# jcribeiro98/V-GAN

Hardware: AMD Instinct MI355X
Metric: V-GAN train steps/sec (batch=1024, d=784) (higher is better)
Workload: dtype f32; MMD contractions of `value`: split-bf16 x3 on the bf16 MFMA with fp32 accumulation (centred operand); the same step with the fp32 MFMA is timed in `fp32_mode`; 1 GPU; configs[2]: MNIST-pixels-as-features stand-in, d=784, batch=1024 (VGAN_no_kl step); global_batch=1024, features=784, latent=49, rows_per_gpu=1024, parallelism=dp1 (row-sharded Gram, replicated front), hip_graph=True, generator=collapsed, chain_association=depth, mmd_precision=bf16x3, gram_tile=64

## Files before the change

include/vgan_hip.h:

```cpp
#ifndef VGAN_HIP_H
#define VGAN_HIP_H

#include <stdint.h>

#ifdef __cplusplus
extern "C" {
#endif

#define VGAN_OK 0
#define VGAN_ERR_ARG 1
#define VGAN_ERR_HIP 2

#define VGAN_ABI_VERSION 11

typedef void* vgan_stream_t;

int vgan_abi_version(void);
const char* vgan_last_error(void);

int vgan_linear_forward(const float* x, int ldx, int x_nslabs, int64_t x_slab_stride, const float* W,
                        int ldw, const float* b, float* y, int ldy, int n, int in, int out,
                        vgan_stream_t stream);
int vgan_linear_backward_input(const float* dy, int lddy, const float* W, int ldw,
                               float* dx, int lddx, int n, int in, int out, vgan_stream_t stream);
int vgan_linear_backward_params(const float* dy, int lddy, const float* x, int ldx, int x_nslabs,
                                int64_t x_slab_stride, float* dW, int lddw, float* db, int n, int in,
                                int out, int splits, int64_t slab_stride, vgan_stream_t stream);
struct vgan_xx_job;
int vgan_linear_backward_params_xx_supported(int n, int in, int out);
int vgan_linear_backward_params_xx(const float* dy, int lddy, const float* x, int ldx, float* dW, int lddw, int n, int in,
                                   int out, const struct vgan_xx_job* xx, vgan_stream_t stream);
int64_t vgan_linear_backward_params_ksplit_ws_bytes(int in, int out, int parts);
int vgan_linear_backward_params_ksplit(const float* dy, int lddy, const float* x, int ldx, float* dW, int lddw, int n, int in,
                                       int out, int parts, void* ws, int64_t ws_bytes, vgan_stream_t stream);
int vgan_reduce_slabs(const float* src, int64_t slab_stride, int nslabs, float* dst, int64_t count,
                      vgan_stream_t stream);

typedef struct vgan_logits_chain {
    const float* za;
    const float* At4;
    int32_t ldza, ldat, e0, pad;
} vgan_logits_chain;
int vgan_mask_project_forward(const float* logits, int ldl, const float* data, int ldd,
                              const int32_t* rows, const uint64_t* row_cursor, int row_batches,
                              int row_stride, int row_offset, float* S, float* U, float* Zx, float* Zy,
                              int ldz, float* sqx, float* sqy, int n, int d, const float* center,
                              int norm_split, const vgan_logits_chain* chain, vgan_stream_t stream);
int vgan_col_mean(const float* data, int ldd, int rows, int d, float* out, vgan_stream_t stream);
int vgan_gather_rows(const float* data, int ldd, const int32_t* rows, const uint64_t* row_cursor,
                     int row_batches, int row_stride, int row_offset, float* out, int ldo,
                     float* sq, int n, int d, vgan_stream_t stream);
int vgan_gather_rows_split(const float* data, int ldd, const int32_t* rows, const uint64_t* row_cursor,
                           int row_batches, int row_stride, int row_offset, const float* center, float* out,
                           int ldo, float* sq, int norm_split, uint16_t* Zh, uint16_t* Zl, int kp, int n, int d,
                           vgan_stream_t stream);
int vgan_mask_backward(const float* gU, int ldg, int nslabs, int64_t slab_stride, const float* S,
                       int lds, const uint64_t* colkey, float pen_weight, int row_offset,
                       float* dlogits, int ldo, int n, int d, vgan_stream_t stream);
int vgan_colmax_chunks(int n);
int vgan_colmax(const float* S, int lds, int from_softmax, int row_offset, uint64_t* part,
                uint64_t* colkey, int n, int d, vgan_stream_t stream);
int vgan_colmax_partial(const float* S, int lds, int from_softmax, int row_offset, uint64_t* part,
                        int n, int d, vgan_stream_t stream);
int vgan_mask_from_softmax(const float* S, int lds, float* U, int ldu, int n, int d, vgan_stream_t stream);
int vgan_upper_softmax_forward(const float* logits, int ldl, float* S, float* U, int n, int d,
                               vgan_stream_t stream);

#define VGAN_TILE 64
#define VGAN_TILE_INTS 8
#define VGAN_TF_SLOT_MASK 3
#define VGAN_TF_TWICE 4
#define VGAN_TF_STORE 8
#define VGAN_TF_MIRROR 16
#define VGAN_TF_NEG 32

int vgan_mmd_build_tiles(int n, int grad_mode, int rank, int world, int tile, int32_t* out, int cap);
int vgan_mmd_order_tiles(int32_t* tiles, int count, int tile);

int vgan_mmd_gram(const float* Z, int ldz, const float* sq, int n, int p, const float* bw,
                  const int32_t* tiles, int ntiles, int calibrate,
                  float* Wg, int ldw, int wrow0, float* partial, vgan_stream_t stream);
#define VGAN_RBF_MAX_KERNELS 8
int vgan_mmd_gram_general(const float* Z, int ldz, const float* sq, int n, int p, const float* bw,
                          const int32_t* tiles, int ntiles, const float* multipliers, int n_kernels,
                          float* Wg, int ldw, int wrow0, float* partial, vgan_stream_t stream);
int vgan_mmd_gram_colmax(const float* Z, int ldz, const float* sq, int n, int p, const float* bw,
                         const int32_t* tiles, int ntiles, float* Wg, int ldw, int wrow0, float* partial,
                         const float* S, int lds, int from_softmax, int row_offset, uint64_t* colpart,
                         int nrows, int d, vgan_stream_t stream);
int vgan_mmd_reduce(const float* partial, const int32_t* tiles, int ntiles, double* stats,
                    int zero_first, vgan_stream_t stream);
int vgan_mmd_set_bandwidth(const double* stats, int n, float* bw, vgan_stream_t stream);
int vgan_mmd_loss(const double* stats, const uint64_t* colkey, int n, int d, float weight,
                  float* loss, float* loss_accum, float accum_scale, uint64_t* step_counter,
                  vgan_stream_t stream);
int vgan_mmd_finalize(const float* partial, const int32_t* tiles, int ntiles, const uint64_t* colpart,
                      int chunks, uint64_t* colkey, int n, int d, float weight, double* stats,
                      float* loss, float* loss_accum, float accum_scale, uint64_t* step_counter,
                      vgan_stream_t stream);
typedef struct vgan_finalize_job {
    const float* partial;
    const int32_t* tiles;
    const uint64_t* colpart;
    uint64_t* colkey;
    double* stats;
    float* loss;
    float* loss_accum;
    uint64_t* step_counter;
    int32_t ntiles, chunks, n, d;
    float weight, accum_scale;
    int32_t mode, ntiles_main;
} vgan_finalize_job;
int vgan_mmd_backward(const float* Wg, int ldw, const float* Z, int ldz, int wrow0, int nr,
                      int ncols, int p, const float* mul, int ldmul, const float* mul_shift, float* out,
                      int ldo, int splits, int64_t slab_stride, const vgan_finalize_job* finalize,
                      vgan_stream_t stream);
int vgan_mmd_bf3_prepare(const float* Z, int ldz, int rows, int p, uint16_t* Zh, uint16_t* Zl, int kp,
                         uint16_t* ZTh, uint16_t* ZTl, int kn, vgan_stream_t stream);
int64_t vgan_mmd_gram_bf3_tail_ws_bytes(void);
int vgan_mmd_gram_bf3(const uint16_t* Zh, const uint16_t* Zl, int kp, const float* sq, int n, const float* bw,
                      const int32_t* tiles, int ntiles, int tile, uint16_t* Wh, uint16_t* Wl, int ldw,
                      int wrow0, float* partial, const float* S, int lds, int from_softmax, int row_offset,
                      uint64_t* colpart, int nrows, int d, void* tail_ws, int64_t tail_ws_bytes,
                      float* rs_part, int ldrs, vgan_stream_t stream);
int vgan_mmd_backward_bf3_tile(int nr, int p, int splits, int tile);
int vgan_mmd_backward_bf3(const uint16_t* Wh, const uint16_t* Wl, int ldw, const uint16_t* ZTh,
                          const uint16_t* ZTl, int kn, int kp, const float* Z, int ldz, int wrow0, int nr,
                          int p, const float* mul, int ldmul, const float* mul_shift, float* out, int ldo,
                          int splits, int64_t slab_stride, int tile, const vgan_finalize_job* finalize,
                          vgan_stream_t stream);
int vgan_mmd_backward_bf3_rm(const uint16_t* Wh, const uint16_t* Wl, int ldw, int kn, const uint16_t* Zh,
                             const uint16_t* Zl, int kp, int zrows, const float* Z, int ldz, int wrow0, int nr,
                             int p, const float* mul, int ldmul, const float* mul_shift, float* out, int ldo,
                             int splits, int64_t slab_stride, int tile, const vgan_finalize_job* finalize,
                             const float* rs_part, int ldrs, vgan_stream_t stream);
int vgan_mmd_backward_bf3_rm_xx(const uint16_t* Wh, const uint16_t* Wl, int ldw, int kn, const uint16_t* Zh,
                                const uint16_t* Zl, int kp, int zrows, const float* Z, int ldz, int wrow0, int nr,
                                int p, const float* mul, int ldmul, const float* mul_shift, float* out, int ldo,
                                int splits, int64_t slab_stride, const vgan_finalize_job* finalize,
                                const struct vgan_xx_job* xx, vgan_stream_t stream);
typedef struct vgan_bwd_rebuild {
    const float* data;
    const int32_t* xrow;
    const float* S;
    const float* center;
    int32_t ldd, lds;
} vgan_bwd_rebuild;
int vgan_mmd_backward_bf3_rm_rebuild(const uint16_t* Wh, const uint16_t* Wl, int ldw, int kn, const uint16_t* Zh,
                                     const uint16_t* Zl, int kp, int zrows, int nr, int p,
                                     const vgan_bwd_rebuild* rebuild, float* out, int ldo, int splits,
                                     int64_t slab_stride, const vgan_finalize_job* finalize,
                                     const struct vgan_xx_job* xx, vgan_stream_t stream);
#define VGAN_GEMM_MAX_GROUP 4
#define VGAN_GEMM_NN 0
#define VGAN_GEMM_NT 1
#define VGAN_GEMM_TN 2
#define VGAN_GEMM_NT_NT 3
typedef struct vgan_gemm_problem {
    const float* a;
    const float* b;
    float* c;
    int32_t kind, m, n, k, lda, ldb, ldc, splitk;
    const float* d;
    float* scratch;
    int32_t ldd, k2;
} vgan_gemm_problem;
int vgan_gemm_grouped(const vgan_gemm_problem* problems, int count, vgan_stream_t stream);
typedef struct vgan_adadelta_layer {
    float* w_packed;
    int64_t off_w, off_b;
    int32_t ldp, out, in, pad;
} vgan_adadelta_layer;
typedef struct vgan_grouped_extras {
    const float* copy_src;
    float* copy_dst;
    int64_t copy_count;
    int32_t adadelta, pad;
    float* p;
    float* sq_avg;
    float* acc_delta;
    float lr, rho, eps, weight_decay, grad_scale;
    int32_t ld_extra;
    vgan_adadelta_layer layer[VGAN_GEMM_MAX_GROUP + 1];
    const float* g_extra;
    float* next_noise;
    int32_t noise_rows, noise_cols, noise_ld, noise_ones_col;
    uint64_t seed;
    const uint64_t* step_counter;
    const vgan_finalize_job* fold;
} vgan_grouped_extras;
int vgan_gemm_grouped_ex(const vgan_gemm_problem* problems, int count, const vgan_grouped_extras* extras,
                         vgan_stream_t stream);
int64_t vgan_gemm_grouped_ksplit_ws_bytes(const vgan_gemm_problem* problems, int count, const int32_t* kparts);
int vgan_gemm_grouped_ksplit(const vgan_gemm_problem* problems, int count, const vgan_grouped_extras* extras,
                             const int32_t* kparts, void* ws, int64_t ws_bytes, vgan_stream_t stream);

typedef struct vgan_xx_job {
    const uint16_t* Dh;
    const uint16_t* Dl;
    const float* dsq;
    const int32_t* tiles;
    const float* bw;
    float* partial;
    int32_t ldd, ntiles;
} vgan_xx_job;
int vgan_mask_project_forward_bf3(const float* logits, int ldl, const float* data, int ldd, const int32_t* rows,
                                  const uint64_t* row_cursor, int row_batches, int row_stride, float* S, float* Z,
                                  int ldz, float* sq, uint16_t* Zh, uint16_t* Zl, int kp, uint16_t* ZTh,
                                  uint16_t* ZTl, int kn, int n, int d, const float* center, int write_x,
                                  const vgan_xx_job* xx, const vgan_logits_chain* chain, vgan_stream_t stream);
int vgan_mask_project_forward_bf3_ex(const float* logits, int ldl, const float* data, int ldd, const int32_t* rows,
                                     const uint64_t* row_cursor, int row_batches, int row_stride, float* S, float* Z,
                                     int ldz, float* sq, uint16_t* Zh, uint16_t* Zl, int kp, uint16_t* ZTh,
                                     uint16_t* ZTl, int kn, int n, int d, const float* center, int write_x,
                                     const vgan_xx_job* xx, const vgan_logits_chain* chain, int write_z, int32_t* xrow,
                                     vgan_stream_t stream);
int vgan_row_sqnorm(const float* Z, int ldz, float* sq, int rows, int p, vgan_stream_t stream);

int vgan_adadelta_step(float* p, const float* g, int nslabs, int64_t slab_stride, float* sq_avg,
                       float* acc_delta, int64_t count, float lr, float rho, float eps,
                       float weight_decay, float grad_scale, vgan_stream_t stream);

int vgan_noise_normal(float* z, int rows, int cols, int ld, int ones_col, uint64_t seed,
                      const uint64_t* step_counter, uint64_t stream_id, vgan_stream_t stream);

int vgan_homogeneous_pack(const int64_t* desc, int count, int max_elems, int unpack, vgan_stream_t stream);
int vgan_adadelta_step_packed(float* p, const int32_t* pmap, const float* g_packed, float* w_packed,
                              float* sq_avg, float* acc_delta, int64_t count, float lr, float rho,
                              float eps, float weight_decay, float grad_scale, float* next_noise,
                              int noise_rows, int noise_cols, int noise_ld, int noise_ones_col,
                              uint64_t seed, const uint64_t* step_counter, vgan_stream_t stream);

int vgan_mse(const float* a, int lda, const float* b, int ldb, int n, int d, float scale,
             float* out, int accumulate, vgan_stream_t stream);

int vgan_mse_grad(const float* target, int ldt, const float* pred, int ldp, int n, int d, float gscale,
                  double* part, float* g, int ldg, vgan_stream_t stream);
int vgan_sum_f64(const double* in, int count, double scale, float* out, int accumulate, vgan_stream_t stream);

#define VGAN_DP_ID_BYTES 128
typedef struct vgan_dp_comm vgan_dp_comm;
int vgan_dp_unique_id(uint8_t* id );
int vgan_dp_comm_create(vgan_dp_comm** comm, int nranks, const uint8_t* id, int rank);
int vgan_dp_allreduce_sum(vgan_dp_comm* comm, float* buf, int64_t count, vgan_stream_t stream);
int vgan_dp_allgather(vgan_dp_comm* comm, void* buf, int64_t bytes_per_rank, vgan_stream_t stream);
int vgan_dp_comm_destroy(vgan_dp_comm* comm);

int vgan_shuffle_epoch(int32_t* perm, int64_t count, int64_t train_size, uint64_t seed, uint64_t epoch,
                       vgan_stream_t stream);
int64_t vgan_shuffle_index(int64_t i, int64_t train_size, uint64_t seed, uint64_t epoch);
int vgan_mask_unique(const uint8_t* masks, int ldm, int n, int d, uint64_t* keys, int32_t* work,
                     int32_t* out_row, int32_t* out_count, vgan_stream_t stream);

int vgan_rbf_kernel_matrix(const float* Z, int ldz, int m, int p, const float* sq, float alpha, float* K, int ldk,
                           vgan_stream_t stream);
int vgan_rbf_multi_kernel_matrix(const float* Z, int ldz, int m, int p, const float* sq, const float* bw,
                                 const float* multipliers, int n_kernels, float* K, int ldk, float* dK, int lddk,
                                 vgan_stream_t stream);
int vgan_rows_dot(const float* A, int lda, const float* B, int ldb, double* out, int rows, int cols,
                  vgan_stream_t stream);

#define VGAN_OUTLIER_MAX_K 32
#define VGAN_OUTLIER_ENGINE_EXACT 0
#define VGAN_OUTLIER_ENGINE_GRAM 1
#define VGAN_OUTLIER_KNN_LARGEST 0
#define VGAN_OUTLIER_KNN_MEAN 1
#define VGAN_OUTLIER_KNN_MEDIAN 2
#define VGAN_OUTLIER_LRD 3
#define VGAN_OUTLIER_LOF 4
#define VGAN_OUTLIER_KDE_MAX_ROWS 8388607
int vgan_outlier_pack(const float* X, int ldx, int n, int d, const float* center, const int32_t* feat,
                      const int32_t* feat_off, const int64_t* col_off, int first, int count, float* packed, float* sq,
                      vgan_stream_t stream);
int vgan_outlier_knn(const float* Pq, const float* sq_q, int nq, const float* Pr, const float* sq_r, int nr,
                     const int32_t* feat_off, const int64_t* col_off, int first, int count, int k, int exclude_self,
                     int engine, int splits, float* part_d, int32_t* part_i, int32_t* nbr, vgan_stream_t stream);
int vgan_outlier_refine(const float* Xq, int ldq, int nq, const float* Xr, int ldr, int nr, int d, const int32_t* feat,
                        const int32_t* feat_off, int first, int count, const int32_t* nbr, int k, int32_t* out_idx,
                        float* out_dist, float* kdist, vgan_stream_t stream);
int vgan_outlier_score(const int32_t* idx, const float* dist, int nq, int k, int count, int method, const float* kdist_ref,
                       const double* lrd_ref, int nr, float* score, const int32_t* score_row, int ld_score, double* lrd_out,
                       vgan_stream_t stream);
int vgan_outlier_kde(const float* Pq, const float* sq_q, int nq, const float* Pr, const float* sq_r, int nr,
                     const int32_t* feat_off, const int64_t* col_off, int first, int count, const double* bandwidth,
                     int exclude_self, int engine, int splits, uint32_t* pivot, uint64_t* acc, float* score,
                     const int32_t* score_row, int ld_score, vgan_stream_t stream);
int vgan_outlier_combine(const float* score, int ld, int S, int n, const double* weights, double* out,
                         vgan_stream_t stream);
int vgan_outlier_abod(const float* Xq, int ldq, int nq, const float* Xr, int ldr, int nr, int d, const int32_t* feat,
                      const int32_t* feat_off, int first, int count, const int32_t* idx, int k, float* score,
                      const int32_t* score_row, int ld_score, vgan_stream_t stream);
int vgan_outlier_abod_floor(float* score, int ld, int S, int n, int fit, double* score_floor, int32_t* n_degenerate,
                            vgan_stream_t stream);
#define VGAN_OUTLIER_NORM_ZSCORE 1
#define VGAN_OUTLIER_NORM_ROBUST 2
#define VGAN_OUTLIER_NORM_MINMAX 3
#define VGAN_OUTLIER_COMBINE_SUM 0
#define VGAN_OUTLIER_COMBINE_MAX 1
int64_t vgan_outlier_score_stats_ws_bytes(int S, int n, int mode);
int vgan_outlier_score_stats(const float* score, int ld, int S, int n, int mode, double* center, double* scale,
                             void* workspace, int64_t workspace_bytes, vgan_stream_t stream);
int vgan_outlier_combine_normalized(const float* score, int ld, int S, int n, const double* center, const double* scale,
                                    const double* weights, int combination, double* out, vgan_stream_t stream);

#define VGAN_CLUSTER_MAX_CLUSTERS 64
// ... 101 lines not shown
```

v-gan_amd/csrc/gemm_bf3.hpp:

```cpp
#pragma once
#include <type_traits>

#include "gemm_core.hpp"

namespace vgan {

typedef __bf16 bf16x8 __attribute__((ext_vector_type(8)));
typedef unsigned u32x4 __attribute__((ext_vector_type(4)));
typedef __attribute__((address_space(3))) u32x4 lds_u4;
typedef __attribute__((address_space(3))) unsigned short lds_u16;
typedef short s16x4 __attribute__((ext_vector_type(4)));
typedef short s16x8 __attribute__((ext_vector_type(8)));
typedef __attribute__((address_space(3))) s16x4 lds_s4;

__device__ __forceinline__ bf16x8 tr_read_k8(const char __attribute__((address_space(3)))* p0, int rows4) {
    const s16x4 a = __builtin_amdgcn_ds_read_tr16_b64_v4i16((lds_s4*)p0);
    const s16x4 b = __builtin_amdgcn_ds_read_tr16_b64_v4i16((lds_s4*)(p0 + rows4));
    const s16x8 v = {a[0], a[1], a[2], a[3], b[0], b[1], b[2], b[3]};
    return __builtin_bit_cast(bf16x8, v);
}


template <int BK_>
struct GemmBF3 {
// ... 130 lines not shown
            for (int r = 0; r < NR; ++r) {
                float s = rsum[r];
#pragma unroll
                for (int o = 1; o < QPR; o <<= 1) s += __shfl_xor(s, o, 64);
                const int f = tid + kBlock * r;
                if (f % QPR == 0) rs_lds[f / QPR] = s;
            }
            __syncthreads();
        }
    }
    __device__ static __forceinline__ int sub_row(int r) {
        const int lane = threadIdx.x & 63, wave = (threadIdx.x >> 6) & 3;
        return (wave >> 1) * 32 + (r & 3) + 8 * (r >> 2) + 4 * (lane >> 5);
    }
    __device__ static __forceinline__ int sub_col() {
        const int lane = threadIdx.x & 63, wave = (threadIdx.x >> 6) & 3;
        return (wave & 1) * 32 + (lane & 31);
    }

    static_assert(BK == 64, "row-major B path: K tile of 64");
    static constexpr int PARTB = 64 * 128;
    static constexpr int BUFT = 2 * PART + 2 * PARTB;
    static constexpr int kLdsBytesT = 2 * BUFT;

    struct StageT {
        u32x4 v[4][NR];
        const char* srcA[2][NR];
        const unsigned short *Bh, *Bl;
        long ldb;
        int lofsA[NR], lofsB[NR], rowB[NR], colB[NR], zrows;
        __device__ __forceinline__ void init(const unsigned short* Ah, const unsigned short* Al, long lda, int m0, int M,
                                             const unsigned short* Bh_, const unsigned short* Bl_, long ldb_, int n0, int zrows_, int tid) {
            Bh = Bh_; Bl = Bl_; ldb = ldb_; zrows = zrows_;
#pragma unroll
            for (int r = 0; r < NR; ++r) {
                const int f = tid + kBlock * r, row = f / QPR, q = f % QPR;
                const long ra = (long)min(m0 + row, M - 1) * lda + 8 * q;
                srcA[0][r] = reinterpret_cast<const char*>(Ah + ra);
                srcA[1][r] = reinterpret_cast<const char*>(Al + ra);
                lofsA[r] = row * ROWB + q * 16;
                rowB[r] = row;
                colB[r] = n0 + 8 * q;
                lofsB[r] = row * 128 + ((q ^ (((row >> 1) & 1) << 2)) << 4);
            }
        }
        __device__ __forceinline__ void load(int k0) {
#pragma unroll
            for (int r = 0; r < NR; ++r) {
                v[0][r] = *reinterpret_cast<const u32x4*>(srcA[0][r] + 2 * (long)k0);
                v[1][r] = *reinterpret_cast<const u32x4*>(srcA[1][r] + 2 * (long)k0);
                const long ob = (long)min(k0 + rowB[r], zrows - 1) * ldb + colB[r];
                v[2][r] = *reinterpret_cast<const u32x4*>(Bh + ob);
                v[3][r] = *reinterpret_cast<const u32x4*>(Bl + ob);
            }
        }
        __device__ __forceinline__ void store(char __attribute__((address_space(3)))* buf) const {
#pragma unroll
            for (int r = 0; r < NR; ++r) {
                *(lds_u4*)(buf + lofsA[r]) = v[0][r];
                *(lds_u4*)(buf + PART + lofsA[r]) = v[1][r];
                *(lds_u4*)(buf + 2 * PART + lofsB[r]) = v[2][r];
                *(lds_u4*)(buf + 2 * PART + PARTB + lofsB[r]) = v[3][r];
            }
        }
        __device__ __forceinline__ float a_rowpart(int r) const {
            float s = 0.f;
            const unsigned* h = reinterpret_cast<const unsigned*>(&v[0][r]);
            const unsigned* l = reinterpret_cast<const unsigned*>(&v[1][r]);
#pragma unroll
            for (int e = 0; e < 4; ++e) {
                s += __uint_as_float(h[e] << 16) + __uint_as_float(h[e] & 0xFFFF0000u);
                s += __uint_as_float(l[e] << 16) + __uint_as_float(l[e] & 0xFFFF0000u);
            }
            return s;
        }
    };

    template <bool SIDE_A>
    __device__ static __forceinline__ void run_bt(const unsigned short* Ah, const unsigned short* Al, long lda, const unsigned short* Bh,
                                                  const unsigned short* Bl, long ldb, int zrows, int m0, int n0, int M, int K,
                                                  char* lds_generic, float* rs_generic, f32x16& acc) {
        typedef char __attribute__((address_space(3))) lds_c;
        lds_c* lds = (lds_c*)lds_generic;
        lds_f* rs_lds = (lds_f*)rs_generic;
        const int tid = threadIdx.x, lane = tid & 63, wave = tid >> 6;
        const int wm0 = (wave >> 1) * 32, wn0 = (wave & 1) * 32;
        const int fi = lane & 31, fh = lane >> 5;
        const int g = lane >> 4, li = lane & 15, qq = li >> 2, pp = li & 3;
        const int chunk = (wn0 >> 3) + 2 * (g & 1) + (pp >> 1);
        const int offB0 = (8 * (g >> 1) + qq) * 128 + ((chunk ^ (((qq >> 1) & 1) << 2)) << 4) + (pp & 1) * 8;
        StageT st;
        st.init(Ah, Al, lda, m0, M, Bh, Bl, ldb, n0, zrows, tid);
        float rsum[NR];
#pragma unroll
        for (int r = 0; r < NR; ++r) rsum[r] = 0.f;
        auto side = [&]() {
#pragma unroll
            for (int r = 0; r < NR; ++r) rsum[r] += st.a_rowpart(r);
        };
        const int nk = K / BK;
        st.load(0);
        st.store(lds);
        if constexpr (SIDE_A) side();
        if (nk > 1) st.load(BK);
        __syncthreads();
        auto body = [&](int kt, auto store_next, auto load_next2) {
            const lds_c* buf = lds + (kt & 1) * BUFT;
            const lds_c* pa = buf + (wm0 + fi) * ROWB + fh * 16;
            const lds_c* pb = buf + 2 * PART + offB0;
            u32x4 ah[KS], al[KS];
            bf16x8 yh[KS], yl[KS];
#pragma unroll
            for (int s = 0; s < KS; ++s) {
                ah[s] = *(const lds_u4*)(pa + s * 32);
                al[s] = *(const lds_u4*)(pa + PART + s * 32);
                yh[s] = tr_read_k8(pb + s * 2048, 512);
                yl[s] = tr_read_k8(pb + PARTB + s * 2048, 512);
            }
            if constexpr (decltype(store_next)::value) {
                st.store(lds + ((kt & 1) ^ 1) * BUFT);
                if constexpr (SIDE_A) side();
            }
            if constexpr (decltype(load_next2)::value) st.load((kt + 2) * BK);
#pragma unroll
            for (int s = 0; s < KS; ++s) {
                const bf16x8 xh = __builtin_bit_cast(bf16x8, ah[s]), xl = __builtin_bit_cast(bf16x8, al[s]);
                acc = __builtin_amdgcn_mfma_f32_32x32x16_bf16(xl, yh[s], acc, 0, 0, 0);
                acc = __builtin_amdgcn_mfma_f32_32x32x16_bf16(xh, yl[s], acc, 0, 0, 0);
                acc = __builtin_amdgcn_mfma_f32_32x32x16_bf16(xh, yh[s], acc, 0, 0, 0);
            }
            __builtin_amdgcn_iglp_opt(0);
            __syncthreads();
        };
        using T = std::true_type;
        using F = std::false_type;
        int kt = 0;
        for (; kt + 2 < nk; ++kt) body(kt, T{}, T{});
        if (kt + 1 < nk) {
            body(kt, T{}, F{});
            ++kt;
        }
        body(kt, F{}, F{});
        if constexpr (SIDE_A) {
#pragma unroll
            for (int r = 0; r < NR; ++r) {
                float s = rsum[r];
#pragma unroll
                for (int o = 1; o < QPR; o <<= 1) s += __shfl_xor(s, o, 64);
                const int f = tid + kBlock * r;
                if (f % QPR == 0) rs_lds[f / QPR] = s;
            }
            __syncthreads();
        }
    }
};


struct GemmBF3Big {
    static constexpr int BM = 128, BN = 128, BK = 64, NTH = 512;
    static constexpr int PART = 128 * 128;
    static constexpr int PARTB = 64 * 256;
    static constexpr int BUF = 4 * PART;
    static constexpr int BUFT = 2 * PART + 2 * PARTB;
    static constexpr int kLdsBytes = 2 * BUF;
    static constexpr int kLdsBytesT = 2 * BUFT;
    typedef char __attribute__((address_space(3))) lds_c;

    struct Quad {
        f32x16 a[2][2];
        __device__ __forceinline__ void zero() {
#pragma unroll
            for (int i = 0; i < 2; ++i)
#pragma unroll
                for (int j = 0; j < 2; ++j)
#pragma unroll
                    for (int r = 0; r < 16; ++r) a[i][j][r] = 0.f;
        }
        __device__ __forceinline__ void mac(const bf16x8 (&xh)[2], const bf16x8 (&xl)[2], const bf16x8 (&yh)[2], const bf16x8 (&yl)[2]) {
#pragma unroll
            for (int i = 0; i < 2; ++i)
#pragma unroll
                for (int j = 0; j < 2; ++j) a[i][j] = __builtin_amdgcn_mfma_f32_32x32x16_bf16(xl[i], yh[j], a[i][j], 0, 0, 0);
#pragma unroll
            for (int i = 0; i < 2; ++i)
#pragma unroll
                for (int j = 0; j < 2; ++j) a[i][j] = __builtin_amdgcn_mfma_f32_32x32x16_bf16(xh[i], yl[j], a[i][j], 0, 0, 0);
#pragma unroll
            for (int i = 0; i < 2; ++i)
#pragma unroll
                for (int j = 0; j < 2; ++j) a[i][j] = __builtin_amdgcn_mfma_f32_32x32x16_bf16(xh[i], yh[j], a[i][j], 0, 0, 0);
        }
        __device__ __forceinline__ void exchange(lds_c* lds, f32x16 (&acc)[2]) const {
            lds_f* xch = (lds_f*)lds;
            const int lane = threadIdx.x & 63, wave = threadIdx.x >> 6, grp = wave >> 2;
#pragma unroll
            for (int i = 0; i < 2; ++i)
#pragma unroll
                for (int r = 0; r < 16; ++r) xch[((wave * 2 + i) * 16 + r) * 64 + lane] = grp ? a[i][0][r] : a[i][1][r];
            __syncthreads();
            const int partner = wave ^ 4;
#pragma unroll
            for (int i = 0; i < 2; ++i)
#pragma unroll
                for (int r = 0; r < 16; ++r) acc[i][r] += (grp ? a[i][1][r] : a[i][0][r]) + xch[((partner * 2 + i) * 16 + r) * 64 + lane];
            __syncthreads();
        }
    };

    struct FillRows {
        const char* src[8];
        int dst0;
        __device__ __forceinline__ void init(const unsigned short* base, long ld, int r0, int lim, int part, int half, int lane) {
#pragma unroll
            for (int e = 0; e < 8; ++e) {
                const int row = half * 64 + 8 * e + (lane >> 3);
                const int c = (lane & 7) ^ ((row >> 1) & 7);
                src[e] = reinterpret_cast<const char*>(base + (long)min(r0 + row, lim - 1) * ld) + 16 * c;
            }
            dst0 = part * PART + half * 8192;
        }
        __device__ __forceinline__ void issue(lds_c* buf, int kt) const {
#pragma unroll
            for (int e = 0; e < 8; ++e)
                __builtin_amdgcn_global_load_lds((const void __attribute__((address_space(1)))*)(src[e] + 2 * (long)kt * BK),
                                                 (void __attribute__((address_space(3)))*)(buf + dst0 + e * 1024), 16, 0, 0);
        }
    };
    struct FillRM {
        const char* src[8];
        long ldb2;
        int krow0, zrows, dst0;
        __device__ __forceinline__ void init(const unsigned short* base, long ld, int n0, int ncols, int zrows_, int bpart, int half, int lane) {
            ldb2 = 2 * ld;
            zrows = zrows_;
            krow0 = half * 32 + (lane >> 4);
#pragma unroll
            for (int e = 0; e < 8; ++e) {
                const int row = krow0 + 4 * e;
                const int c = (lane & 15) ^ ((row & 3) << 2);
                src[e] = reinterpret_cast<const char*>(base + min(n0 + 8 * c, ncols - 8));
            }
            dst0 = 2 * PART + bpart * PARTB + half * 8192;
        }
        __device__ __forceinline__ void issue(lds_c* buf, int kt) const {
#pragma unroll
            for (int e = 0; e < 8; ++e) {
                const char* g = src[e] + (long)min(kt * BK + krow0 + 4 * e, zrows - 1) * ldb2;
                __builtin_amdgcn_global_load_lds((const void __attribute__((address_space(1)))*)g,
                                                 (void __attribute__((address_space(3)))*)(buf + dst0 + e * 1024), 16, 0, 0);
            }
        }
    };

    template <class Fill0, class Fill1, class FragF, class MfmaF>
    __device__ static __forceinline__ void pingpong(int grp, int nk, Fill0 fill0, Fill1 fill1, FragF frags, MfmaF mfmas) {
        auto bar = [&]() {
            __builtin_amdgcn_sched_barrier(0);
            __builtin_amdgcn_s_barrier();
            __builtin_amdgcn_sched_barrier(0);
        };
        auto drain = [&]() { __builtin_amdgcn_s_waitcnt(0x0070); };
        if (grp == 0) {
            for (int kt = 0; kt < nk; ++kt) {
                if (kt + 1 < nk) fill0(kt + 1);
                frags(kt);
                bar();
                mfmas();
                drain();
                bar();
            }
            bar();
        } else {
            if (1 < nk) fill1(1);
            bar();
            for (int kt = 0; kt < nk; ++kt) {
                frags(kt);
                drain();
                bar();
                if (kt + 2 < nk) fill1(kt + 2);
                mfmas();
                bar();
            }
        }
        __syncthreads();
    }

    __device__ static __forceinline__ float frag_sum(const u32x4& h, const u32x4& l, float s) {
#pragma unroll
        for (int e = 0; e < 4; ++e) {
            s += __uint_as_float(h[e] << 16) + __uint_as_float(h[e] & 0xFFFF0000u);
            s += __uint_as_float(l[e] << 16) + __uint_as_float(l[e] & 0xFFFF0000u);
        }
        return s;
    }
    template <class Frag>
    __device__ static __forceinline__ void rowsum_step(const Frag (&ah)[2][2], const Frag (&al)[2][2], int C, float (&rsum)[2]) {
        if (C == 0) {
            rsum[0] = frag_sum(ah[0][0], al[0][0], rsum[0]);
            rsum[1] = frag_sum(ah[0][1], al[0][1], rsum[1]);
        } else {
            rsum[0] = frag_sum(ah[1][0], al[1][0], rsum[0]);
            rsum[1] = frag_sum(ah[1][1], al[1][1], rsum[1]);
        }
    }
    __device__ static __forceinline__ void rowsum_publish(const float (&rsum)[2], lds_f* tmp, int grp, int R, int C, int fi, int fh) {
#pragma unroll
// ... 146 lines not shown
```

v-gan_amd/csrc/mmd_bf16.hip:

```cpp
#include "gemm_bf3.hpp"
#include "gemm_bf3w.hpp"
#include "mmd_common.hpp"
#include "mmd_xx.hpp"

namespace vgan {


__global__ __launch_bounds__(kBlock) void bf3_prepare_kernel(const float* __restrict__ Z, int ldz, int rows, int p,
                                                            unsigned short* __restrict__ Zh, unsigned short* __restrict__ Zl, int kp,
                                                            unsigned short* __restrict__ ZTh, unsigned short* __restrict__ ZTl, int kn,
                                                            int vec) {
    __shared__ unsigned short th[64][68], tl[64][68];
    const int j0 = blockIdx.x * 64, k0 = blockIdx.y * 64;
    const int tj = 4 * (threadIdx.x & 15), tk = 4 * (threadIdx.x >> 4);
    unsigned short hi[4][4], lo[4][4];
#pragma unroll
    for (int a = 0; a < 4; ++a) {
        const int k = k0 + tk + a;
        float v[4] = {0.f, 0.f, 0.f, 0.f};
        if (k < rows) {
            if (vec && j0 + tj + 3 < p) {
                const float4 q = *reinterpret_cast<const float4*>(Z + (long)k * ldz + j0 + tj);
                v[0] = q.x; v[1] = q.y; v[2] = q.z; v[3] = q.w;
            } else {
// ... 385 lines not shown
        };
        float w[16];
        if (cons) {
#pragma unroll
            for (int i = 0; i < 4; ++i)
#pragma unroll
                for (int j = 0; j < 4; ++j)
#pragma unroll
                    for (int r = 0; r < 4; ++r) Wt[G::sub_row(i, r) * LDT + G::sub_col(j)] = acc[i][j][r];
        }
        __syncthreads();
        for (int t = threadIdx.x; t < 256 * 8; t += G::NTH) {
            const int line = t >> 3, q16 = 16 * (t & 7);
            float cs = 0.f;
            if (td.r0 + line < td.rlim && td.c0 + q16 < td.clim) {
#pragma unroll
                for (int e = 0; e < 4; ++e) {
                    const f32x4 v = *(const lds_f4*)(Wt + line * LDT + q16 + 4 * e);
                    w[4 * e] = v[0]; w[4 * e + 1] = v[1]; w[4 * e + 2] = v[2]; w[4 * e + 3] = v[3];
                }
                cs = emit(w, (long)(td.r0 + line - wrow0) * ldw, td.c0 + q16, td.clim);
            }
            if (rs_part != nullptr) {
                cs = slot_sum(cs);
                if ((t & 7) == 0 && td.r0 + line < td.rlim) rs_part[(long)(td.c0 >> 7) * ldrs + (td.r0 + line - wrow0)] = cs;
            }
        }
        if (mirror) {
            __syncthreads();
            if (cons) {
#pragma unroll
                for (int i = 0; i < 4; ++i)
#pragma unroll
                    for (int j = 0; j < 4; ++j)
                        *(lds_f4*)(Wt + G::sub_col(j) * LDM + G::sub_row(i, 0)) = f32x4{acc[i][j][0], acc[i][j][1], acc[i][j][2], acc[i][j][3]};
            }
            __syncthreads();
            for (int t = threadIdx.x; t < 128 * 16; t += G::NTH) {
                const int line = t >> 4, q16 = 16 * (t & 15);
                float cs = 0.f;
                if (td.c0 + line < td.clim && td.r0 + q16 < td.rlim) {
#pragma unroll
                    for (int e = 0; e < 4; ++e) {
                        const f32x4 v = *(const lds_f4*)(Wt + line * LDM + q16 + 4 * e);
                        w[4 * e] = v[0]; w[4 * e + 1] = v[1]; w[4 * e + 2] = v[2]; w[4 * e + 3] = v[3];
                    }
                    cs = emit(w, (long)(td.c0 + line - wrow0) * ldw, td.r0 + q16, td.rlim);
                }
                if (rs_part != nullptr) {
                    cs = slot_sum(cs);
                    if ((t & 7) == 0 && td.c0 + line < td.clim && td.r0 + q16 < td.rlim)
                        rs_part[(long)((td.r0 + q16) >> 7) * ldrs + (td.c0 + line - wrow0)] = cs;
                }
            }
        }
    }
    ksum = wave_sum(ksum);
    if (lane == 0) red[wave] = ksum;
    __syncthreads();
    if (threadIdx.x == 0)
        reinterpret_cast<float4*>(partial)[ti] =
            make_float4(((red[0] + red[1]) + (red[2] + red[3])) + ((red[4] + red[5]) + (red[6] + red[7])), 0.f, 0.f, 0.f);
}

struct BwdRebuild {
    const float* data;
    const int* xrow;
    const float* S;
    const float* center;
    int ldd, lds;
};

template <int BK, bool RM, bool REBUILD>
__global__ __launch_bounds__(kBlock, BK == 64 ? 2 : 3) void mmd_backward_bf3_kernel(const unsigned short* __restrict__ Wh, const unsigned short* __restrict__ Wl,
                                                                    int ldw, const unsigned short* __restrict__ ZTh,
                                                                    const unsigned short* __restrict__ ZTl, int kn, int ldb, int brows,
                                                                    const float* __restrict__ Z, int ldz, int wrow0, int nr, int p,
                                                                    int ptiles, const float* __restrict__ mul, int ldmul,
                                                                    const float* __restrict__ mul_shift, float* __restrict__ out, int ldo,
                                                                    int kchunk, long slab_stride, vgan_finalize_job job, int nfin,
                                                                    XXJob xx, BwdRebuild rb) {
    using G = GemmBF3<BK>;
    constexpr int kBytes = (RM ? G::kLdsBytesT : G::kLdsBytes) > G::kLdsBytes ? (RM ? G::kLdsBytesT : G::kLdsBytes) : G::kLdsBytes;
    __shared__ __attribute__((aligned(16))) char lds[kBytes];
    __shared__ float rs[64];
    const int gx = ptiles, gy = (nr + 63) / 64, total = gx * gy;
    if ((int)blockIdx.x >= total) {
        if (blockIdx.y != 0) return;
        const int extra = (int)blockIdx.x - total;
        if (extra < nfin)
            finalize_body(job);
        else if constexpr (BK == 64)
            xx_tile_body(xx, extra - nfin, lds, rs);
        return;
    }
    const int xcd = blockIdx.x % 8, kidx = blockIdx.x / 8;
    const int q = total / 8, r8 = total % 8;
    const int t = (xcd < r8 ? xcd * (q + 1) : r8 * (q + 1) + (xcd - r8) * q) + kidx;
    const int band = t / (4 * gx), rem = t - band * 4 * gx;
    const int rows_in_band = min(4, gy - band * 4);
    const int m0 = (band * 4 + rem % rows_in_band) * 64, n0 = (rem / rows_in_band) * 64;
    f32x16 acc;
#pragma unroll
    for (int r = 0; r < 16; ++r) acc[r] = 0.f;
    const int k0 = blockIdx.y * kchunk, klen = min(kchunk, kn - k0);
    out += blockIdx.y * slab_stride;
    const int col = n0 + G::sub_col(), colc = min(col, p - 1);
    float z_pre[16], m_pre[16];
    float mshift;
    if constexpr (REBUILD) {
        mshift = rb.center[colc];
#pragma unroll
        for (int r = 0; r < 16; ++r) {
            const int rowc = min(m0 + G::sub_row(r), nr - 1);
            z_pre[r] = rb.S[(long)rowc * rb.lds + colc];
            m_pre[r] = rb.data[(long)rb.xrow[rowc] * rb.ldd + colc];
        }
    } else {
        mshift = mul_shift != nullptr ? mul_shift[colc] : 0.f;
#pragma unroll
        for (int r = 0; r < 16; ++r) {
            const int rowc = min(m0 + G::sub_row(r), nr - 1);
            z_pre[r] = Z[(long)(wrow0 + rowc) * ldz + colc];
            m_pre[r] = mul != nullptr ? mul[(long)rowc * ldmul + colc] + mshift : 1.f;
        }
    }
    if (klen > 0) {
        if constexpr (RM)
            G::template run_bt<true>(Wh + k0, Wl + k0, ldw, ZTh + (long)k0 * ldb, ZTl + (long)k0 * ldb, ldb, brows - k0, m0, n0, nr, klen, lds,
                                     rs, acc);
        else
            G::template run<true>(Wh + k0, Wl + k0, ldw, ZTh + k0, ZTl + k0, ldb, m0, n0, nr, gx * 64, klen, lds, rs, acc);
    }
    if (col >= p) return;
    if constexpr (REBUILD) {
        const float tau = 1.0f / (float)p;
#pragma unroll
        for (int r = 0; r < 16; ++r) {
            const float x = m_pre[r];
            z_pre[r] = project_centred(upper_mask(z_pre[r], tau), x, mshift);
            m_pre[r] = uncentred_x(centred_x(x, mshift), mshift);
        }
    }
#pragma unroll
    for (int r = 0; r < 16; ++r) {
        const int lrow = G::sub_row(r), row = m0 + lrow;
        if (row < nr) {
            const float v = klen > 0 ? 2.f * (rs[lrow] * z_pre[r] - acc[r]) : 0.f;
            out[(long)row * ldo + col] = v * m_pre[r];
        }
    }
}

template <bool RM>
__global__ __launch_bounds__(512, 2) void mmd_backward_bf3_big_kernel(const unsigned short* __restrict__ Wh, const unsigned short* __restrict__ Wl,
                                                                      int ldw, const unsigned short* __restrict__ ZTh,
                                                                      const unsigned short* __restrict__ ZTl, int kn, int ldb, int brows,
                                                                      const float* __restrict__ Z, int ldz, int wrow0, int nr, int p,
                                                                      int ptiles, const float* __restrict__ mul, int ldmul,
                                                                      const float* __restrict__ mul_shift, float* __restrict__ out, int ldo,
                                                                      int kchunk, long slab_stride, int nb_rows, vgan_finalize_job job) {
    using G = GemmBF3Big;
    __shared__ __attribute__((aligned(16))) char lds[RM ? G::kLdsBytesT : G::kLdsBytes];
    __shared__ float rs[128];
    const int gx = ptiles, gy = (nr + 127) / 128, total = gx * gy;
    if ((int)blockIdx.x >= total) {
        if (blockIdx.y == 0) finalize_body(job);
        return;
    }
    const int xcd = blockIdx.x % 8, kidx = blockIdx.x / 8;
    const int q = total / 8, r8 = total % 8;
    const int t = (xcd < r8 ? xcd * (q + 1) : r8 * (q + 1) + (xcd - r8) * q) + kidx;
    const int band = t / (4 * gx), rem = t - band * 4 * gx;
    const int rows_in_band = min(4, gy - band * 4);
    const int m0 = (band * 4 + rem % rows_in_band) * 128, n0 = (rem / rows_in_band) * 128;
    const int k0 = blockIdx.y * kchunk, klen = min(kchunk, kn - k0);
    out += blockIdx.y * slab_stride;
    const int col = n0 + G::sub_col(), colc = min(col, p - 1);
    const float mshift = mul_shift != nullptr ? mul_shift[colc] : 0.f;
    f32x16 acc[2];
#pragma unroll
    for (int i2 = 0; i2 < 2; ++i2)
#pragma unroll
        for (int r = 0; r < 16; ++r) acc[i2][r] = 0.f;
    if (klen > 0) {
        if constexpr (RM)
            G::template run_bt<true>(Wh + k0, Wl + k0, ldw, ZTh + (long)k0 * ldb, ZTl + (long)k0 * ldb, ldb, nb_rows, brows - k0, m0, n0, nr, klen,
                                     lds, acc, rs);
        else
            G::template run<true>(Wh + k0, Wl + k0, ldw, ZTh + k0, ZTl + k0, ldb, m0, n0, nr, nb_rows, klen, lds, acc, rs);
    }
    if (col >= p) return;
#pragma unroll
    for (int i2 = 0; i2 < 2; ++i2) {
        float z_pre[16], m_pre[16];
#pragma unroll
        for (int r = 0; r < 16; ++r) {
            const int rowc = min(m0 + G::sub_row(i2, r), nr - 1);
            z_pre[r] = Z[(long)(wrow0 + rowc) * ldz + colc];
            m_pre[r] = mul != nullptr ? mul[(long)rowc * ldmul + colc] + mshift : 1.f;
        }
#pragma unroll
        for (int r = 0; r < 16; ++r) {
            const int lrow = G::sub_row(i2, r), row = m0 + lrow;
            if (row < nr) {
                const float v = klen > 0 ? 2.f * (rs[lrow] * z_pre[r] - acc[i2][r]) : 0.f;
                out[(long)row * ldo + col] = v * m_pre[r];
            }
        }
    }
}


__global__ __launch_bounds__(768, 3) void mmd_backward_bf3_wide_kernel(const unsigned short* __restrict__ Wh, const unsigned short* __restrict__ Wl,
                                                                       int ldw, const unsigned short* __restrict__ Bh,
                                                                       const unsigned short* __restrict__ Bl, int kn, int ldb, int brows,
                                                                       const float* __restrict__ Z, int ldz, int wrow0, int nr, int p,
                                                                       int ptiles, const float* __restrict__ mul, int ldmul,
                                                                       const float* __restrict__ mul_shift, float* __restrict__ out, int ldo,
                                                                       int kchunk, long slab_stride, int nb_cols, vgan_finalize_job job,
                                                                       const float* __restrict__ rs_part, int ldrs) {
    using G = GemmBF3Wide;
    extern __shared__ __attribute__((aligned(16))) char lds[];
    __shared__ float rs[256];
    const int gx = ptiles, gy = (nr + 255) / 256, total = gx * gy;
    if ((int)blockIdx.x >= total) {
        if (blockIdx.y == 0) finalize_body(job);
        return;
    }
    const int xcd = blockIdx.x % 8, kidx = blockIdx.x / 8;
    const int q = total / 8, r8 = total % 8;
    const int t = (xcd < r8 ? xcd * (q + 1) : r8 * (q + 1) + (xcd - r8) * q) + kidx;
    const int band = t / (4 * gx), rem = t - band * 4 * gx;
    const int rows_in_band = min(4, gy - band * 4);
    const int m0 = (band * 4 + rem % rows_in_band) * 256, n0 = (rem / rows_in_band) * 128;
    const int k0 = blockIdx.y * kchunk, klen = min(kchunk, kn - k0);
    out += blockIdx.y * slab_stride;
    f32x4w acc[4][4];
#pragma unroll
    for (int i = 0; i < 4; ++i)
#pragma unroll
        for (int j = 0; j < 4; ++j) acc[i][j] = f32x4w{0.f, 0.f, 0.f, 0.f};
    if (klen > 0 && rs_part != nullptr) {
        if (threadIdx.x < 256) {
            const float* src = rs_part + min(m0 + (int)threadIdx.x, nr - 1);
            const int s0 = k0 >> 7, s1 = (k0 + klen + 127) >> 7;
            float a0 = 0.f, a1 = 0.f, a2 = 0.f, a3 = 0.f;
            int sl = s0;
            for (; sl + 4 <= s1; sl += 4) {
                a0 += src[(long)sl * ldrs];
                a1 += src[(long)(sl + 1) * ldrs];
                a2 += src[(long)(sl + 2) * ldrs];
                a3 += src[(long)(sl + 3) * ldrs];
            }
            for (; sl < s1; ++sl) a0 += src[(long)sl * ldrs];
            rs[threadIdx.x] = (a0 + a1) + (a2 + a3);
        }
        G::run_bt<false>(Wh + k0, Wl + k0, ldw, Bh + (long)k0 * ldb, Bl + (long)k0 * ldb, ldb, nb_cols, brows - k0, m0, n0, nr, klen, lds, acc);
    } else if (klen > 0)
        G::run_bt<true>(Wh + k0, Wl + k0, ldw, Bh + (long)k0 * ldb, Bl + (long)k0 * ldb, ldb, nb_cols, brows - k0, m0, n0, nr, klen, lds, acc, rs);
    if (G::is_loader()) return;
#pragma unroll
    for (int j = 0; j < 4; ++j) {
        const int col = n0 + G::sub_col(j);
        if (col >= p) continue;
        const float mshift = mul_shift != nullptr ? mul_shift[col] : 0.f;
#pragma unroll
        for (int i = 0; i < 4; ++i) {
            float z_pre[4], m_pre[4];
#pragma unroll
            for (int r = 0; r < 4; ++r) {
                const int rowc = min(m0 + G::sub_row(i, r), nr - 1);
                z_pre[r] = Z[(long)(wrow0 + rowc) * ldz + col];
                m_pre[r] = mul != nullptr ? mul[(long)rowc * ldmul + col] + mshift : 1.f;
            }
#pragma unroll
            for (int r = 0; r < 4; ++r) {
                const int lrow = G::sub_row(i, r), row = m0 + lrow;
                if (row < nr) {
                    const float v = klen > 0 ? 2.f * (rs[lrow] * z_pre[r] - acc[i][j][r]) : 0.f;
                    out[(long)row * ldo + col] = v * m_pre[r];
                }
            }
        }
    }
}

}

using namespace vgan;

extern "C" int vgan_mmd_bf3_prepare(const float* Z, int ldz, int rows, int p, uint16_t* Zh, uint16_t* Zl, int kp, uint16_t* ZTh,
                                    uint16_t* ZTl, int kn, vgan_stream_t stream) {
    VGAN_CHECK_ARG(Z && Zh && Zl && rows > 0 && p > 0 && ldz >= p && kp >= p && kp % 64 == 0 && aligned16(Zh) && aligned16(Zl));
    VGAN_CHECK_ARG((ZTh == nullptr) == (ZTl == nullptr) && (ZTh == nullptr || (kn >= rows && kn % 64 == 0)));
    dim3 grid(kp / 64, (rows + 63) / 64);
    if (ZTh != nullptr) grid.y = kn / 64;
    const int vec = (ldz % 4 == 0) && aligned16(Z);
    hipLaunchKernelGGL(bf3_prepare_kernel, grid, dim3(kBlock), 0, (hipStream_t)stream, Z, ldz, rows, p, Zh, Zl, kp, ZTh, ZTl, kn, vec);
    VGAN_CHECK_LAUNCH();
    return VGAN_OK;
}

#ifndef VGAN_TAIL_MAX_PARTS
#define VGAN_TAIL_MAX_PARTS 4
#endif
extern "C" int64_t vgan_mmd_gram_bf3_tail_ws_bytes(void) { return kTailSlabs * kTailSlabBytes + kTailTicketBytes; }

extern "C" int vgan_mmd_gram_bf3(const uint16_t* Zh, const uint16_t* Zl, int kp, const float* sq, int n, const float* bw,
                                 const int32_t* tiles, int ntiles, int tile, uint16_t* Wh, uint16_t* Wl, int ldw, int wrow0,
                                 float* partial, const float* S, int lds, int from_softmax, int row_offset, uint64_t* colpart,
                                 int nrows, int d, void* tail_ws, int64_t tail_ws_bytes, float* rs_part, int ldrs,
                                 vgan_stream_t stream) {
    VGAN_CHECK_ARG(Zh && Zl && sq && bw && tiles && partial && n > 0 && ntiles > 0 && kp > 0 && kp % 64 == 0);
    VGAN_CHECK_ARG((Wh == nullptr) == (Wl == nullptr) && (reinterpret_cast<uintptr_t>(partial) & 15) == 0);
    VGAN_CHECK_ARG(aligned16(Zh) && aligned16(Zl) && (Wh == nullptr || (aligned16(Wh) && aligned16(Wl) && ldw % 8 == 0)));
    ColmaxJob cj{};
    int extra = 0;
    if (S != nullptr) {
        VGAN_CHECK_ARG(colpart && nrows > 0 && d > 0 && lds >= d);
        cj = ColmaxJob{S, reinterpret_cast<unsigned long long*>(colpart), lds, row_offset, nrows, d, from_softmax, (d + 63) / 64};
        extra = cj.nbx * ((nrows + kColChunkRows - 1) / kColChunkRows);
    }
    VGAN_CHECK_ARG(tile == 64 || tile == 128 || tile == 256);
    VGAN_CHECK_ARG(rs_part == nullptr || (tile == 256 && Wh != nullptr && ldrs > 0 && wrow0 >= 0 && n % 128 == 0));
    if (tile == 256) {
        static const hipError_t attr = hipFuncSetAttribute(reinterpret_cast<const void*>(&mmd_gram_bf3_wide_kernel),
                                                           hipFuncAttributeMaxDynamicSharedMemorySize, GemmBF3Wide::kLdsBytes);
        VGAN_CHECK_ARG(attr == hipSuccess);
        TailSplit ts{nullptr, nullptr, ntiles, 1, kp};
        if (tail_ws != nullptr) {
            VGAN_CHECK_ARG(tail_ws_bytes >= vgan_mmd_gram_bf3_tail_ws_bytes() && aligned16(tail_ws));
            static const int cus = [] {
                int dev = 0, v = 0;
                if (hipGetDevice(&dev) != hipSuccess || hipDeviceGetAttribute(&v, hipDeviceAttributeMultiprocessorCount, dev) != hipSuccess) v = 0;
                return v;
            }();
            const int slots = cus < kTailSlabs ? cus : kTailSlabs;
            const int r = slots > 0 ? ntiles % slots : 0, nst = kp / GemmBF3Wide::BK;
            int parts = 1;
            while (r > 0 && parts < VGAN_TAIL_MAX_PARTS && 2 * parts * r <= slots && nst / (2 * parts) >= 8) parts *= 2;
            if (parts > 1) {
                const int kchunk = ((nst + parts - 1) / parts) * GemmBF3Wide::BK;
                ts = TailSplit{static_cast<float*>(tail_ws), reinterpret_cast<int*>(static_cast<char*>(tail_ws) + kTailSlabs * kTailSlabBytes),
                               ntiles - r, (kp + kchunk - 1) / kchunk, kchunk};
            }
        }
        const int nblk = ts.first + (ntiles - ts.first) * ts.parts;
        hipLaunchKernelGGL(mmd_gram_bf3_wide_kernel, dim3(nblk + extra), dim3(GemmBF3Wide::NTH), GemmBF3Wide::kLdsBytes, (hipStream_t)stream, Zh,
                           Zl, kp, sq, n, bw, reinterpret_cast<const TileDesc*>(tiles), ntiles, Wh, Wl, ldw, wrow0, partial, cj, ts, rs_part, ldrs);
    } else if (tile == 128)
        hipLaunchKernelGGL(mmd_gram_bf3_big_kernel, dim3(ntiles + extra), dim3(512), 0, (hipStream_t)stream, Zh, Zl, kp, sq, n, bw,
                           reinterpret_cast<const TileDesc*>(tiles), ntiles, Wh, Wl, ldw, wrow0, partial, cj);
    else
        hipLaunchKernelGGL(mmd_gram_bf3_kernel<64>, dim3(ntiles + extra), dim3(kBlock), 0, (hipStream_t)stream, Zh, Zl, kp, sq, n, bw,
                           reinterpret_cast<const TileDesc*>(tiles), ntiles, Wh, Wl, ldw, wrow0, partial, cj);
    VGAN_CHECK_LAUNCH();
    return VGAN_OK;
}

extern "C" int vgan_mmd_backward_bf3_tile(int nr, int p, int splits, int tile) {
    if (tile == 64 || tile == 128 || tile == 256) return tile;
    const int wide_tiles = ((p + 127) / 128) * ((nr + 255) / 256);
    if (nr >= 256 && wide_tiles * splits >= 256) return 256;
    const int big_tiles = ((p + 127) / 128) * ((nr + 127) / 128);
    return big_tiles * splits >= 512 ? 128 : 64;
}

static int launch_backward_bf3(int rm, const uint16_t* Wh, const uint16_t* Wl, int ldw, const uint16_t* Bh, const uint16_t* Bl, int kn, int kp,
                               int zrows, const float* Z, int ldz, int wrow0, int nr, int p, const float* mul, int ldmul,
                               const float* mul_shift, float* out, int ldo, int splits, int64_t slab_stride, int tile,
                               const vgan_finalize_job* finalize, vgan_stream_t stream, const vgan_xx_job* xxjob = nullptr,
                               const float* rs_part = nullptr, int ldrs = 0, const vgan_bwd_rebuild* rebuild = nullptr) {
    VGAN_CHECK_ARG(Wh && Wl && Bh && Bl && (Z || rebuild) && out && nr > 0 && p > 0 && kn > 0 && kn % 64 == 0 && kp >= p && kp % 64 == 0);
    VGAN_CHECK_ARG(ldw >= kn && (rebuild || ldz >= p) && ldo >= p && (mul == nullptr || ldmul >= p) && wrow0 >= 0);
    BwdRebuild rb{};
    if (rebuild != nullptr) {
        const vgan_bwd_rebuild& q = *rebuild;
        VGAN_CHECK_ARG(rm && tile == 64 && q.data && q.xrow && q.S && q.center && q.ldd >= p && q.lds >= p && Z == nullptr && mul == nullptr &&
                       mul_shift == nullptr);
        rb = BwdRebuild{q.data, q.xrow, q.S, q.center, q.ldd, q.lds};
    }
    VGAN_CHECK_ARG(aligned16(Wh) && aligned16(Wl) && aligned16(Bh) && aligned16(Bl) && ldw % 8 == 0);
    VGAN_CHECK_ARG(splits >= 1 && splits <= 64 && (splits == 1 || slab_stride >= (int64_t)nr * ldo));
    VGAN_CHECK_ARG((tile == 0 || tile == 64 || tile == 128 || tile == 256) && (mul_shift == nullptr || mul != nullptr) && (!rm || zrows > 0));
    const int kchunk = ((kn / 64 + splits - 1) / splits) * 64;
    const int ldb = rm ? kp : kn;
    vgan_finalize_job job{};
    if (finalize != nullptr) {
        VGAN_CHECK_ARG(finalize_job_ok(*finalize));
        job = *finalize;
    }
    hipStream_t st = (hipStream_t)stream;
    XXJob xx{};
    if (xxjob != nullptr) {
        const vgan_xx_job& j = *xxjob;
        VGAN_CHECK_ARG(rm && tile == 64 && j.Dh && j.Dl && j.dsq && j.tiles && j.bw && j.partial && j.ntiles > 0 && j.ldd % 64 == 0 &&
                       aligned16(j.Dh) && aligned16(j.Dl) && (reinterpret_cast<uintptr_t>(j.partial) & 15) == 0);
        xx = XXJob{j.Dh, j.Dl, j.dsq, nullptr, nullptr, reinterpret_cast<const TileDesc*>(j.tiles), j.bw, j.partial, j.ldd, 1, 0, j.ntiles, 0};
    }
    const int nfin = finalize != nullptr ? 1 : 0;
    int edge = vgan_mmd_backward_bf3_tile(nr, p, splits, tile);
    if (edge == 256 && !rm) edge = 128;
    if (edge == 256) {
        static const hipError_t attr = hipFuncSetAttribute(reinterpret_cast<const void*>(&mmd_backward_bf3_wide_kernel),
                                                           hipFuncAttributeMaxDynamicSharedMemorySize, GemmBF3Wide::kLdsBytes);
        VGAN_CHECK_ARG(attr == hipSuccess);
        const int pt = (p + 127) / 128;
        dim3 grid(pt * ((nr + 255) / 256) + nfin, splits);
        if (rs_part != nullptr && !(ldrs >= nr && (splits == 1 || kchunk % 128 == 0))) rs_part = nullptr;
        hipLaunchKernelGGL(mmd_backward_bf3_wide_kernel, grid, dim3(GemmBF3Wide::NTH), GemmBF3Wide::kLdsBytes, st, Wh, Wl, ldw, Bh, Bl, kn, ldb,
                           zrows, Z, ldz, wrow0, nr, p, pt, mul, ldmul, mul_shift, out, ldo, kchunk, (long)slab_stride, kp, job, rs_part, ldrs);
        VGAN_CHECK_LAUNCH();
        return VGAN_OK;
    }
    if (edge == 128) {
        const int pt = (p + 127) / 128;
        dim3 grid(pt * ((nr + 127) / 128) + (finalize != nullptr ? 1 : 0), splits);
        if (rm)
            hipLaunchKernelGGL(mmd_backward_bf3_big_kernel<true>, grid, dim3(512), 0, st, Wh, Wl, ldw, Bh, Bl, kn, ldb, zrows, Z, ldz, wrow0, nr,
                               p, pt, mul, ldmul, mul_shift, out, ldo, kchunk, (long)slab_stride, kp, job);
        else
            hipLaunchKernelGGL(mmd_backward_bf3_big_kernel<false>, grid, dim3(512), 0, st, Wh, Wl, ldw, Bh, Bl, kn, ldb, 0, Z, ldz, wrow0, nr, p,
                               pt, mul, ldmul, mul_shift, out, ldo, kchunk, (long)slab_stride, kp, job);
        VGAN_CHECK_LAUNCH();
        return VGAN_OK;
    }
    const int ptiles = (p + 63) / 64;
    dim3 grid(ptiles * ((nr + 63) / 64) + nfin + xx.ntiles, splits);
    if (rebuild != nullptr)
        hipLaunchKernelGGL((mmd_backward_bf3_kernel<64, true, true>), grid, dim3(kBlock), 0, st, Wh, Wl, ldw, Bh, Bl, kn, ldb, zrows, Z, ldz, wrow0,
                           nr, p, ptiles, mul, ldmul, mul_shift, out, ldo, kchunk, (long)slab_stride, job, nfin, xx, rb);
    else if (rm)
        hipLaunchKernelGGL((mmd_backward_bf3_kernel<64, true, false>), grid, dim3(kBlock), 0, st, Wh, Wl, ldw, Bh, Bl, kn, ldb, zrows, Z, ldz, wrow0,
                           nr, p, ptiles, mul, ldmul, mul_shift, out, ldo, kchunk, (long)slab_stride, job, nfin, xx, rb);
    else
        hipLaunchKernelGGL((mmd_backward_bf3_kernel<64, false, false>), grid, dim3(kBlock), 0, st, Wh, Wl, ldw, Bh, Bl, kn, ldb, 0, Z, ldz, wrow0, nr,
                           p, ptiles, mul, ldmul, mul_shift, out, ldo, kchunk, (long)slab_stride, job, nfin, xx, rb);
    VGAN_CHECK_LAUNCH();
    return VGAN_OK;
}

extern "C" int vgan_mmd_backward_bf3(const uint16_t* Wh, const uint16_t* Wl, int ldw, const uint16_t* ZTh, const uint16_t* ZTl, int kn,
                                     int kp, const float* Z, int ldz, int wrow0, int nr, int p, const float* mul, int ldmul,
                                     const float* mul_shift, float* out, int ldo, int splits, int64_t slab_stride, int tile,
                                     const vgan_finalize_job* finalize, vgan_stream_t stream) {
    return launch_backward_bf3(0, Wh, Wl, ldw, ZTh, ZTl, kn, kp, 0, Z, ldz, wrow0, nr, p, mul, ldmul, mul_shift, out, ldo, splits, slab_stride,
                               tile, finalize, stream);
}

extern "C" int vgan_mmd_backward_bf3_rm_xx(const uint16_t* Wh, const uint16_t* Wl, int ldw, int kn, const uint16_t* Zh, const uint16_t* Zl,
                                           int kp, int zrows, const float* Z, int ldz, int wrow0, int nr, int p, const float* mul, int ldmul,
                                           const float* mul_shift, float* out, int ldo, int splits, int64_t slab_stride,
                                           const vgan_finalize_job* finalize, const vgan_xx_job* xx, vgan_stream_t stream) {
    VGAN_CHECK_ARG(xx != nullptr);
    return launch_backward_bf3(1, Wh, Wl, ldw, Zh, Zl, kn, kp, zrows, Z, ldz, wrow0, nr, p, mul, ldmul, mul_shift, out, ldo, splits,
                               slab_stride, 64, finalize, stream, xx);
}

extern "C" int vgan_mmd_backward_bf3_rm(const uint16_t* Wh, const uint16_t* Wl, int ldw, int kn, const uint16_t* Zh, const uint16_t* Zl,
                                        int kp, int zrows, const float* Z, int ldz, int wrow0, int nr, int p, const float* mul, int ldmul,
                                        const float* mul_shift, float* out, int ldo, int splits, int64_t slab_stride, int tile,
                                        const vgan_finalize_job* finalize, const float* rs_part, int ldrs, vgan_stream_t stream) {
    return launch_backward_bf3(1, Wh, Wl, ldw, Zh, Zl, kn, kp, zrows, Z, ldz, wrow0, nr, p, mul, ldmul, mul_shift, out, ldo, splits,
                               slab_stride, tile, finalize, stream, nullptr, rs_part, ldrs);
}

extern "C" int vgan_mmd_backward_bf3_rm_rebuild(const uint16_t* Wh, const uint16_t* Wl, int ldw, int kn, const uint16_t* Zh, const uint16_t* Zl,
                                                int kp, int zrows, int nr, int p, const vgan_bwd_rebuild* rebuild, float* out, int ldo,
                                                int splits, int64_t slab_stride, const vgan_finalize_job* finalize, const vgan_xx_job* xx,
                                                vgan_stream_t stream) {
    VGAN_CHECK_ARG(rebuild != nullptr);
    return launch_backward_bf3(1, Wh, Wl, ldw, Zh, Zl, kn, kp, zrows, nullptr, 0, 0, nr, p, nullptr, 0, nullptr, out, ldo, splits, slab_stride, 64,
                               finalize, stream, xx, nullptr, 0, rebuild);
}
```

v-gan_amd/lib.py:

```python
import ctypes
import os

_HERE = os.path.dirname(os.path.abspath(__file__))
LIB_PATH = os.path.join(_HERE, "libvgan_hip.so")

_p = ctypes.c_void_p
_i = ctypes.c_int
_f = ctypes.c_float
_i64 = ctypes.c_int64
_u64 = ctypes.c_uint64

class FinalizeJob(ctypes.Structure):
    _fields_ = [("partial", _p), ("tiles", _p), ("colpart", _p), ("colkey", _p), ("stats", _p), ("loss", _p), ("loss_accum", _p),
                ("step_counter", _p), ("ntiles", ctypes.c_int32), ("chunks", ctypes.c_int32), ("n", ctypes.c_int32),
                ("d", ctypes.c_int32), ("weight", _f), ("accum_scale", _f), ("mode", ctypes.c_int32), ("ntiles_main", ctypes.c_int32)]


class GemmProblem(ctypes.Structure):
    _fields_ = [("a", _p), ("b", _p), ("c", _p), ("kind", ctypes.c_int32), ("m", ctypes.c_int32), ("n", ctypes.c_int32),
                ("k", ctypes.c_int32), ("lda", ctypes.c_int32), ("ldb", ctypes.c_int32), ("ldc", ctypes.c_int32), ("splitk", ctypes.c_int32),
                ("d", _p), ("scratch", _p), ("ldd", ctypes.c_int32), ("k2", ctypes.c_int32)]


class LogitsChain(ctypes.Structure):
    _fields_ = [("za", _p), ("At4", _p), ("ldza", ctypes.c_int32), ("ldat", ctypes.c_int32), ("e0", ctypes.c_int32), ("pad", ctypes.c_int32)]


class XXJob(ctypes.Structure):
    _fields_ = [("Dh", _p), ("Dl", _p), ("dsq", _p), ("tiles", _p), ("bw", _p), ("partial", _p), ("ldd", ctypes.c_int32),
                ("ntiles", ctypes.c_int32)]


class BwdRebuild(ctypes.Structure):
    _fields_ = [("data", _p), ("xrow", _p), ("S", _p), ("center", _p), ("ldd", ctypes.c_int32), ("lds", ctypes.c_int32)]


class AdadeltaLayer(ctypes.Structure):
    _fields_ = [("w_packed", _p), ("off_w", _i64), ("off_b", _i64), ("ldp", ctypes.c_int32), ("out", ctypes.c_int32),
                ("inp", ctypes.c_int32), ("pad", ctypes.c_int32)]


class GroupedExtras(ctypes.Structure):
    _fields_ = [("copy_src", _p), ("copy_dst", _p), ("copy_count", _i64), ("adadelta", ctypes.c_int32), ("pad", ctypes.c_int32),
                ("p", _p), ("sq_avg", _p), ("acc_delta", _p), ("lr", _f), ("rho", _f), ("eps", _f), ("weight_decay", _f),
                ("grad_scale", _f), ("ld_extra", ctypes.c_int32), ("layer", AdadeltaLayer * 5), ("g_extra", _p), ("next_noise", _p),
                ("noise_rows", ctypes.c_int32), ("noise_cols", ctypes.c_int32), ("noise_ld", ctypes.c_int32),
                ("noise_ones_col", ctypes.c_int32), ("seed", _u64), ("step_counter", _p), ("fold", _p)]


GEMM_NN, GEMM_NT, GEMM_TN, GEMM_NT_NT = 0, 1, 2, 3
GEMM_MAX_GROUP = 4

SIGNATURES = {
    "vgan_abi_version": (_i, []),
    "vgan_last_error": (ctypes.c_char_p, []),
    "vgan_linear_forward": (_i, [_p, _i, _i, _i64, _p, _i, _p, _p, _i, _i, _i, _i, _p]),
    "vgan_linear_backward_input": (_i, [_p, _i, _p, _i, _p, _i, _i, _i, _i, _p]),
    "vgan_linear_backward_params": (_i, [_p, _i, _p, _i, _i, _i64, _p, _i, _p, _i, _i, _i, _i, _i64, _p]),
    "vgan_linear_backward_params_ksplit_ws_bytes": (_i64, [_i, _i, _i]),
    "vgan_linear_backward_params_ksplit": (_i, [_p, _i, _p, _i, _p, _i, _i, _i, _i, _i, _p, _i64, _p]),
    "vgan_linear_backward_params_xx_supported": (_i, [_i, _i, _i]),
    "vgan_linear_backward_params_xx": (_i, [_p, _i, _p, _i, _p, _i, _i, _i, _i, _p, _p]),
    "vgan_reduce_slabs": (_i, [_p, _i64, _i, _p, _i64, _p]),
    "vgan_mask_project_forward": (_i, [_p, _i, _p, _i, _p, _p, _i, _i, _i, _p, _p, _p, _p, _i, _p, _p, _i, _i, _p, _i, _p, _p]),
    "vgan_col_mean": (_i, [_p, _i, _i, _i, _p, _p]),
    "vgan_gather_rows": (_i, [_p, _i, _p, _p, _i, _i, _i, _p, _i, _p, _i, _i, _p]),
    "vgan_gather_rows_split": (_i, [_p, _i, _p, _p, _i, _i, _i, _p, _p, _i, _p, _i, _p, _p, _i, _i, _i, _p]),
    "vgan_mask_backward": (_i, [_p, _i, _i, _i64, _p, _i, _p, _f, _i, _p, _i, _i, _i, _p]),
    "vgan_colmax_partial": (_i, [_p, _i, _i, _i, _p, _i, _i, _p]),
    "vgan_mmd_finalize": (_i, [_p, _p, _i, _p, _i, _p, _i, _i, _f, _p, _p, _p, _f, _p, _p]),
    "vgan_colmax_chunks": (_i, [_i]),
    "vgan_colmax": (_i, [_p, _i, _i, _i, _p, _p, _i, _i, _p]),
    "vgan_mask_from_softmax": (_i, [_p, _i, _p, _i, _i, _i, _p]),
    "vgan_upper_softmax_forward": (_i, [_p, _i, _p, _p, _i, _i, _p]),
    "vgan_mmd_build_tiles": (_i, [_i, _i, _i, _i, _i, _p, _i]),
    "vgan_mmd_order_tiles": (_i, [_p, _i, _i]),
    "vgan_mmd_gram": (_i, [_p, _i, _p, _i, _i, _p, _p, _i, _i, _p, _i, _i, _p, _p]),
    "vgan_mmd_gram_general": (_i, [_p, _i, _p, _i, _i, _p, _p, _i, _p, _i, _p, _i, _i, _p, _p]),
    "vgan_mmd_gram_colmax": (_i, [_p, _i, _p, _i, _i, _p, _p, _i, _p, _i, _i, _p, _p, _i, _i, _i, _p, _i, _i, _p]),
    "vgan_mmd_reduce": (_i, [_p, _p, _i, _p, _i, _p]),
    "vgan_mmd_set_bandwidth": (_i, [_p, _i, _p, _p]),
    "vgan_mmd_loss": (_i, [_p, _p, _i, _i, _f, _p, _p, _f, _p, _p]),
    "vgan_mmd_backward": (_i, [_p, _i, _p, _i, _i, _i, _i, _i, _p, _i, _p, _p, _i, _i, _i64, _p, _p]),
    "vgan_mmd_bf3_prepare": (_i, [_p, _i, _i, _i, _p, _p, _i, _p, _p, _i, _p]),
    "vgan_mmd_gram_bf3": (_i, [_p, _p, _i, _p, _i, _p, _p, _i, _i, _p, _p, _i, _i, _p, _p, _i, _i, _i, _p, _i, _i, _p, _i64, _p, _i, _p]),
    "vgan_mmd_gram_bf3_tail_ws_bytes": (_i64, []),
    "vgan_mmd_backward_bf3": (_i, [_p, _p, _i, _p, _p, _i, _i, _p, _i, _i, _i, _i, _p, _i, _p, _p, _i, _i, _i64, _i, _p, _p]),
    "vgan_mmd_backward_bf3_tile": (_i, [_i, _i, _i, _i]),
    "vgan_mmd_backward_bf3_rm": (_i, [_p, _p, _i, _i, _p, _p, _i, _i, _p, _i, _i, _i, _i, _p, _i, _p, _p, _i, _i, _i64, _i, _p, _p, _i, _p]),
    "vgan_mmd_backward_bf3_rm_xx": (_i, [_p, _p, _i, _i, _p, _p, _i, _i, _p, _i, _i, _i, _i, _p, _i, _p, _p, _i, _i, _i64, _p, _p, _p]),
    "vgan_mmd_backward_bf3_rm_rebuild": (_i, [_p, _p, _i, _i, _p, _p, _i, _i, _i, _i, _p, _p, _i, _i, _i64, _p, _p, _p]),
    "vgan_row_sqnorm": (_i, [_p, _i, _p, _i, _i, _p]),
    "vgan_adadelta_step": (_i, [_p, _p, _i, _i64, _p, _p, _i64, _f, _f, _f, _f, _f, _p]),
    "vgan_noise_normal": (_i, [_p, _i, _i, _i, _i, _u64, _p, _u64, _p]),
    "vgan_homogeneous_pack": (_i, [_p, _i, _i, _i, _p]),
    "vgan_adadelta_step_packed": (_i, [_p, _p, _p, _p, _p, _p, _i64, _f, _f, _f, _f, _f, _p, _i, _i, _i, _i, _u64, _p, _p]),
    "vgan_gemm_grouped": (_i, [_p, _i, _p]),
    "vgan_gemm_grouped_ex": (_i, [_p, _i, _p, _p]),
    "vgan_gemm_grouped_ksplit_ws_bytes": (_i64, [_p, _i, _p]),
    "vgan_gemm_grouped_ksplit": (_i, [_p, _i, _p, _p, _p, _i64, _p]),
    "vgan_mask_project_forward_bf3": (_i, [_p, _i, _p, _i, _p, _p, _i, _i, _p, _p, _i, _p, _p, _p, _i, _p, _p, _i, _i, _i, _p, _i, _p, _p, _p]),
    "vgan_mask_project_forward_bf3_ex": (_i, [_p, _i, _p, _i, _p, _p, _i, _i, _p, _p, _i, _p, _p, _p, _i, _p, _p, _i, _i, _i, _p, _i, _p, _p, _i, _p,
                                              _p]),
    "vgan_mse_grad": (_i, [_p, _i, _p, _i, _i, _i, _f, _p, _p, _i, _p]),
    "vgan_sum_f64": (_i, [_p, _i, ctypes.c_double, _p, _i, _p]),
    "vgan_rbf_kernel_matrix": (_i, [_p, _i, _i, _i, _p, _f, _p, _i, _p]),
    "vgan_rbf_multi_kernel_matrix": (_i, [_p, _i, _i, _i, _p, _p, _p, _i, _p, _i, _p, _i, _p]),
    "vgan_rows_dot": (_i, [_p, _i, _p, _i, _p, _i, _i, _p]),
    "vgan_shuffle_epoch": (_i, [_p, _i64, _i64, _u64, _u64, _p]),
    "vgan_shuffle_index": (_i64, [_i64, _i64, _u64, _u64]),
    "vgan_mask_unique": (_i, [_p, _i, _i, _i, _p, _p, _p, _p, _p]),
    "vgan_dp_unique_id": (_i, [_p]),
    "vgan_dp_comm_create": (_i, [_p, _i, _p, _i]),
    "vgan_dp_allreduce_sum": (_i, [_p, _p, _i64, _p]),
    "vgan_dp_allgather": (_i, [_p, _p, _i64, _p]),
    "vgan_dp_comm_destroy": (_i, [_p]),
    "vgan_mse": (_i, [_p, _i, _p, _i, _i, _i, _f, _p, _i, _p]),
    "vgan_outlier_pack": (_i, [_p, _i, _i, _i, _p, _p, _p, _p, _i, _i, _p, _p, _p]),
    "vgan_outlier_knn": (_i, [_p, _p, _i, _p, _p, _i, _p, _p, _i, _i, _i, _i, _i, _i, _p, _p, _p, _p]),
    "vgan_outlier_refine": (_i, [_p, _i, _i, _p, _i, _i, _i, _p, _p, _i, _i, _p, _i, _p, _p, _p, _p]),
    "vgan_outlier_score": (_i, [_p, _p, _i, _i, _i, _i, _p, _p, _i, _p, _p, _i, _p, _p]),
    "vgan_outlier_kde": (_i, [_p, _p, _i, _p, _p, _i, _p, _p, _i, _i, _p, _i, _i, _i, _p, _p, _p, _p, _i, _p]),
    "vgan_outlier_combine": (_i, [_p, _i, _i, _i, _p, _p, _p]),
    "vgan_outlier_abod": (_i, [_p, _i, _i, _p, _i, _i, _i, _p, _p, _i, _i, _p, _i, _p, _p, _i, _p]),
    "vgan_outlier_abod_floor": (_i, [_p, _i, _i, _i, _i, _p, _p, _p]),
    "vgan_outlier_score_stats_ws_bytes": (_i64, [_i, _i, _i]),
    "vgan_outlier_score_stats": (_i, [_p, _i, _i, _i, _i, _p, _p, _p, _i64, _p]),
    "vgan_outlier_combine_normalized": (_i, [_p, _i, _i, _i, _p, _p, _p, _i, _p, _p]),
    "vgan_cluster_lloyd_ws_bytes": (_i64, [_i, _i, _i, _i]),
    "vgan_cluster_image": (_i, [_p, _i, _p, _p, _p, _i, _i, _p, _p, _p, _p]),
    "vgan_cluster_lloyd": (_i, [_p, _p, _p, _i, _i, _i, _p, _p, _p, _i, _i, _i, _i, _i, _i, _p, _p, _p, _p, _p, _p, _p, _p, _p,
                                _p, _i64, _i, _p]),
    "vgan_cluster_final": (_i, [_p, _i, _i, _i, _p, _p, _i, _i, _p, _p, _p, _i, _p, _p, _p, _p, _p, _i, _p]),
    "vgan_ecod_sort_columns": (_i, [_p, _i, _i, _i, _p, _i64, _p]),
    "vgan_ecod_skew_sign": (_i, [_p, _i64, _i, _i, _p, _p]),
    "vgan_ecod_tail_counts": (_i, [_p, _i, _i, _i, _p, _i64, _i, _p, _p, _p]),
    "vgan_ecod_scores": (_i, [_p, _p, _i, _i, _p, _i, _i, _i, _p, _i, _i, _p, _p, _i64, _p]),
    "vgan_hist_column_range": (_i, [_p, _i, _i, _i, _p, _p]),
    "vgan_hist_edges": (_i, [_p, _i64, _i, _p, _p]),
    "vgan_hist_column_counts": (_i, [_p, _i, _i, _i, _p, _i, _p, _p]),
    "vgan_hbos_scores": (_i, [_p, _i, _i, _i, _p, _i, _p, _p, _p, _i, _i, _p, _p, _i64, _p]),
    "vgan_hist_reset": (_i, [_p, _i64, _p, _i64, _p]),
    "vgan_loda_range": (_i, [_p, _i, _p, _p, _i, _i, _i, _p, _p, _p, _i, _p, _p]),
    "vgan_loda_counts": (_i, [_p, _i, _p, _p, _i, _i, _i, _p, _p, _p, _i, _p, _i, _p, _p]),
    "vgan_loda_scores": (_i, [_p, _i, _p, _p, _i, _i, _i, _p, _p, _p, _i, _p, _i, _p, _p, _i64, _p]),
    "vgan_iforest_build": (_i, [_p, _i, _i64, _i, _p, _p, _i, _i, _i, _i, _i, _i, _u64, _p, _p]),
    "vgan_iforest_path_sums": (_i, [_p, _i, _i, _i, _p, _i, _i, _i, _i, _i, _p, _p, _i64, _p]),
    "vgan_iforest_scores": (_i, [_p, _i64, _i, _i, _i64, _p, _i64, _p]),
    "vgan_maha_moments": (_i, [_p, _i, _i, _i, _p, _p, _p, _i, _i, _i, _i, _p, _i, _p, _i64, _p, _p, _p, _p, _i64, _p]),
    "vgan_maha_factor": (_i, [_p, _p, _p, _i, _i, _i, _p, ctypes.c_double, _p, _p, _p, _p, _p]),
    "vgan_maha_scores": (_i, [_p, _i, _i, _i, _p, _p, _p, _i, _i, _i, _p, _p, _p, _i64, _p]),
    "vgan_maha_select": (_i, [_p, _i64, _i, _i, _i, _p, _p, _i64, _p, _p]),
    "vgan_gmm_moments": (_i, [_p, _i, _i, _i, _p, _p, _p, _i, _i, _i, _i, _i, _p, _i, _p, _p, ctypes.c_double, _p, _p, _p, _p, _p, _p,
                              _i64, _p]),
    "vgan_gmm_logdet": (_i, [_p, _p, _p, _i, _i, _i, _p, _p]),
    "vgan_gmm_estep": (_i, [_p, _i, _i, _i, _p, _p, _p, _i, _i, _i, _i, _p, _p, _p, _p, _p, _p, _p, _p, _i64, _p]),
    "vgan_gmm_converge": (_i, [_p, _i, _i, _i, _i, _p, ctypes.c_double, _i, _p, _p, _p, _p, _p]),
}

ABI_VERSION = 11
_lib = None


class VganHipError(RuntimeError):
    pass


def load():
    global _lib
    if _lib is not None:
        return _lib
    if not os.path.exists(LIB_PATH):
        raise VganHipError(
            f"{LIB_PATH} is missing: build it with `python -c 'import __graft_entry__ as g; g.build()'` "
            "(or `make -C v-gan_amd/csrc`).  vgan_amd has no CPU fallback.")
    lib = ctypes.CDLL(LIB_PATH)
    for name, (res, args) in SIGNATURES.items():
        fn = getattr(lib, name)
        fn.restype = res
        fn.argtypes = args
    if lib.vgan_abi_version() != ABI_VERSION:
        raise VganHipError(f"ABI mismatch: library {lib.vgan_abi_version()} vs binding {ABI_VERSION}")
    _lib = lib
    return lib


def check(rc, what=""):
    if rc != 0:
        msg = load().vgan_last_error().decode(errors="replace")
        raise VganHipError(f"{what} failed (code {rc}): {msg}")


def build_tiles(n, grad_mode, rank=0, world=1, tile=64):
    lib = load()
    cnt = lib.vgan_mmd_build_tiles(n, grad_mode, rank, world, tile, None, 0)
    if cnt < 0:
        raise VganHipError("vgan_mmd_build_tiles: " + lib.vgan_last_error().decode())
    buf = (ctypes.c_int32 * (cnt * 8))()
    got = lib.vgan_mmd_build_tiles(n, grad_mode, rank, world, tile, ctypes.cast(buf, ctypes.c_void_p), cnt)
    if got != cnt:
        raise VganHipError("vgan_mmd_build_tiles: inconsistent tile count")
    return list(buf), cnt


def split_tiles(table, tile=64, yy_last=False):
    import torch
    lib = load()
    slot = table[:, 4] & 3
    first = (slot != 2) if yy_last else (slot != 0)
    parts = []
    for keep in (first, ~first):
        sub = table[keep].contiguous()
        if sub.shape[0] > 1:
            buf = (ctypes.c_int32 * sub.numel())(*sub.reshape(-1).tolist())
            if lib.vgan_mmd_order_tiles(ctypes.cast(buf, ctypes.c_void_p), sub.shape[0], tile) != 0:
                raise VganHipError("vgan_mmd_order_tiles: " + lib.vgan_last_error().decode())
            sub = torch.tensor(list(buf), dtype=torch.int32).view(-1, 8)
        parts.append(sub)
    return parts
```

v-gan_amd/ops.py:

```python
import ctypes

import torch

from . import lib as _lib

_f32 = torch.float32


def _round4(v):
    return (int(v) + 3) // 4 * 4


def _ptr(t):
    return ctypes.c_void_p(t.data_ptr()) if t is not None else None


def _mat(t, name):
    if not (t.is_cuda and t.dtype == _f32 and t.dim() == 2 and t.stride(1) == 1):
        raise ValueError(f"{name}: need a float32 HIP matrix with unit inner stride, got "
                         f"{t.dtype} {tuple(t.shape)} strides {t.stride()} on {t.device}")
    return t


def _vec(t, name, dtype=_f32):
    if not (t.is_cuda and t.dtype == dtype and t.is_contiguous()):
        raise ValueError(f"{name}: need a contiguous {dtype} HIP tensor, got {t.dtype} on {t.device}")
    return t


class HipOps:

    name = "hip"

    def __init__(self):
        self.lib = _lib.load()
        if not torch.cuda.is_available():
            raise _lib.VganHipError("vgan_amd needs a HIP device (torch.cuda.is_available() is False); "
                                    "there is no CPU fallback")

    @staticmethod
    def _stream():
        return ctypes.c_void_p(torch.cuda.current_stream().cuda_stream)

    def build_tiles(self, n, grad_mode, rank=0, world=1, device=None, tile=64, split_xx=False, split=None):
        flat, cnt = _lib.build_tiles(n, grad_mode, rank, world, tile)
        table = torch.tensor(flat, dtype=torch.int32).view(cnt, 8)
        if split_xx or split:
            first, second = _lib.split_tiles(table, tile, yy_last=(split == "yy_last"))
            return torch.cat([first, second]).to(device or "cuda"), first.shape[0]
        return table.to(device or "cuda")

    def colmax_chunks(self, n):
        return self.lib.vgan_colmax_chunks(n)

    def linear_forward(self, x, W, b, y, x_nslabs=1, x_slab_stride=0):
        _mat(x, "x"), _mat(W, "W"), _mat(y, "y")
        n, kin = x.shape
        out = W.shape[0]
        assert W.shape[1] == kin and y.shape == (n, out)
        _lib.check(self.lib.vgan_linear_forward(_ptr(x), x.stride(0), int(x_nslabs), int(x_slab_stride), _ptr(W), W.stride(0),
                                                _ptr(b), _ptr(y), y.stride(0), n, kin, out, self._stream()), "vgan_linear_forward")

    def linear_backward_input(self, dy, W, dx):
        _mat(dy, "dy"), _mat(W, "W"), _mat(dx, "dx")
        n, out = dy.shape
        kin = W.shape[1]
        assert W.shape[0] == out and dx.shape == (n, kin)
        _lib.check(self.lib.vgan_linear_backward_input(_ptr(dy), dy.stride(0), _ptr(W), W.stride(0), _ptr(dx), dx.stride(0),
                                                       n, kin, out, self._stream()), "vgan_linear_backward_input")

    def linear_backward_params(self, dy, x, dW, db, splits=1, slab_stride=0, x_nslabs=1, x_slab_stride=0):
        _mat(dy, "dy"), _mat(x, "x"), _mat(dW, "dW")
        n, out = dy.shape
        kin = x.shape[1]
        assert x.shape[0] == n and dW.shape == (out, kin)
        _lib.check(self.lib.vgan_linear_backward_params(_ptr(dy), dy.stride(0), _ptr(x), x.stride(0), int(x_nslabs), int(x_slab_stride),
                                                        _ptr(dW), dW.stride(0), _ptr(db), n, kin, out, int(splits), int(slab_stride),
                                                        self._stream()), "vgan_linear_backward_params")

    def linear_backward_params_ksplit_ws_bytes(self, kin, out, parts):
        return int(self.lib.vgan_linear_backward_params_ksplit_ws_bytes(int(kin), int(out), int(parts)))

    def ksplit_workspace(self, nbytes, device=None):
        return torch.zeros(max(int(nbytes), 16) // 4 + 4, dtype=torch.int32, device=device or "cuda")

    def linear_backward_params_ksplit(self, dy, x, dW, parts, ws):
        _mat(dy, "dy"), _mat(x, "x"), _mat(dW, "dW")
        n, out = dy.shape
        kin = x.shape[1]
        assert x.shape[0] == n and dW.shape == (out, kin)
        _lib.check(self.lib.vgan_linear_backward_params_ksplit(_ptr(dy), dy.stride(0), _ptr(x), x.stride(0), _ptr(dW), dW.stride(0), n, kin, out,
                                                               int(parts), _ptr(ws), 0 if ws is None else ws.numel() * ws.element_size(),
                                                               self._stream()), "vgan_linear_backward_params_ksplit")

    def linear_backward_params_xx_supported(self, n, kin, out):
        return bool(self.lib.vgan_linear_backward_params_xx_supported(int(n), int(kin), int(out)))

    def linear_backward_params_xx(self, dy, x, dW, xx):
        _mat(dy, "dy"), _mat(x, "x"), _mat(dW, "dW")
        n, out = dy.shape
        kin = x.shape[1]
        assert x.shape[0] == n and dW.shape == (out, kin)
        _lib.check(self.lib.vgan_linear_backward_params_xx(_ptr(dy), dy.stride(0), _ptr(x), x.stride(0), _ptr(dW), dW.stride(0), n, kin, out,
                                                           ctypes.byref(xx), self._stream()), "vgan_linear_backward_params_xx")

    def reduce_slabs(self, src, slab_stride, nslabs, dst):
        _vec(dst, "dst")
        _lib.check(self.lib.vgan_reduce_slabs(_ptr(src), int(slab_stride), int(nslabs), _ptr(dst), dst.numel(), self._stream()),
                   "vgan_reduce_slabs")

    def col_mean(self, data, out):
        _mat(data, "data"), _vec(out, "out")
        rows, d = data.shape
        assert out.numel() >= d
        _lib.check(self.lib.vgan_col_mean(_ptr(data), data.stride(0), rows, d, _ptr(out), self._stream()), "vgan_col_mean")

    @staticmethod
    def logits_chain(za, At4):
        _mat(za, "za"), _mat(At4, "At4")
        assert za.shape[1] == At4.shape[1]
        return _lib.LogitsChain(_ptr(za), _ptr(At4), za.stride(0), At4.stride(0), za.shape[1], 0)

    @staticmethod
    def chain_fusable(n, d, *lds):
        return d % 4 == 0 and d <= 1024 and all(int(v) % 4 == 0 for v in lds)

    def mask_project_forward(self, logits, data, rows, S, U, Zx, Zy, sqx, sqy, row_cursor=None, row_batches=1, row_stride=0,
                             row_offset=0, center=None, norm_split=False, chain=None):
        _mat(data, "data"), _mat(Zy, "Zy"), _mat(S, "S")
        n, d = S.shape
        if logits is not None:
            _mat(logits, "logits")
            assert tuple(logits.shape) == (n, d)
        assert S.is_contiguous() and S.shape == (n, d) and (U is None or (U.is_contiguous() and U.shape == (n, d)))
        assert Zx is None or Zx.stride(0) == Zy.stride(0)
        if rows is not None:
            _vec(rows, "rows", torch.int32)
        _lib.check(self.lib.vgan_mask_project_forward(_ptr(logits), logits.stride(0) if logits is not None else 0, _ptr(data), data.stride(0), _ptr(rows),
                                                      _ptr(row_cursor), int(row_batches), int(row_stride), int(row_offset), _ptr(S), _ptr(U), _ptr(Zx), _ptr(Zy), Zy.stride(0), _ptr(sqx), _ptr(sqy),
                                                      n, d, _ptr(center), int(bool(norm_split)),
                                                      ctypes.byref(chain) if chain is not None else None, self._stream()), "vgan_mask_project_forward")

    bf3_rebuild = True
    chain_ksplit = True

    def xx_job(self, Dh, Dl, dsq, tiles, bw, partial):
        assert tiles.is_contiguous() and partial.is_contiguous() and Dh.stride(0) == Dl.stride(0)
        return _lib.XXJob(_ptr(Dh), _ptr(Dl), _ptr(dsq), _ptr(tiles), _ptr(bw), _ptr(partial), Dh.stride(0), tiles.shape[0])

    def bwd_rebuild(self, data, xrow, S, center):
        _mat(data, "data"), _mat(S, "S")
        assert xrow.dtype == torch.int32 and xrow.is_contiguous() and center.is_contiguous()
        return _lib.BwdRebuild(_ptr(data), _ptr(xrow), _ptr(S), _ptr(center), data.stride(0), S.stride(0))

    def mask_project_forward_bf3(self, logits, data, rows, S, Z, sq, Zh, Zl, ZTh, ZTl, row_cursor=None, row_batches=1, row_stride=0,
                                 center=None, write_x=True, xx=None, chain=None, write_z=True, xrow=None):
        _mat(data, "data"), _mat(Z, "Z"), _mat(S, "S")
# ... 45 lines not shown
        _mat(logits, "logits")
        n, d = logits.shape
        assert S.is_contiguous() and (U is None or U.is_contiguous())
        _lib.check(self.lib.vgan_upper_softmax_forward(_ptr(logits), logits.stride(0), _ptr(S), _ptr(U), n, d, self._stream()),
                   "vgan_upper_softmax_forward")

    def mask_backward(self, gU, S, colkey, pen_weight, row_offset, dlogits, nslabs=1, slab_stride=0):
        _mat(gU, "gU"), _mat(S, "S"), _mat(dlogits, "dlogits")
        n, d = S.shape
        _lib.check(self.lib.vgan_mask_backward(_ptr(gU), gU.stride(0), int(nslabs), int(slab_stride), _ptr(S), S.stride(0),
                                               _ptr(colkey), float(pen_weight),
                                               int(row_offset), _ptr(dlogits), dlogits.stride(0), n, d, self._stream()),
                   "vgan_mask_backward")

    def colmax(self, S, row_offset, part, colkey, from_softmax=True):
        _mat(S, "S")
        n, d = S.shape
        assert part.dtype == torch.int64 and colkey.dtype == torch.int64 and part.numel() >= self.colmax_chunks(n) * d
        _lib.check(self.lib.vgan_colmax(_ptr(S), S.stride(0), int(bool(from_softmax)), int(row_offset), _ptr(part), _ptr(colkey), n, d, self._stream()),
                   "vgan_colmax")

    def colmax_partial(self, S, row_offset, part, from_softmax=True):
        _mat(S, "S")
        n, d = S.shape
        assert part.dtype == torch.int64 and part.numel() >= self.colmax_chunks(n) * d
        _lib.check(self.lib.vgan_colmax_partial(_ptr(S), S.stride(0), int(bool(from_softmax)), int(row_offset), _ptr(part), n, d,
                                                self._stream()), "vgan_colmax_partial")

    def mmd_finalize(self, partial, tiles, colpart, chunks, colkey, n, d, weight, stats, loss, loss_accum=None, accum_scale=1.0,
                     step_counter=None):
        _lib.check(self.lib.vgan_mmd_finalize(_ptr(partial), _ptr(tiles), tiles.shape[0], _ptr(colpart), int(chunks), _ptr(colkey),
                                              int(n), int(d), float(weight), _ptr(stats), _ptr(loss), _ptr(loss_accum),
                                              float(accum_scale), _ptr(step_counter), self._stream()), "vgan_mmd_finalize")

    def finalize_job(self, partial, tiles, colpart, chunks, colkey, n, d, weight, stats, loss, loss_accum=None, accum_scale=1.0,
                     step_counter=None, mode=0, ntiles_main=0):
        return _lib.FinalizeJob(_ptr(partial), _ptr(tiles), _ptr(colpart), _ptr(colkey), _ptr(stats), _ptr(loss), _ptr(loss_accum),
                                _ptr(step_counter), tiles.shape[0], int(chunks), int(n), int(d), float(weight), float(accum_scale),
                                int(mode), int(ntiles_main))

    def mask_from_softmax(self, S, U):
        _mat(S, "S"), _mat(U, "U")
        n, d = S.shape
        _lib.check(self.lib.vgan_mask_from_softmax(_ptr(S), S.stride(0), _ptr(U), U.stride(0), n, d, self._stream()),
                   "vgan_mask_from_softmax")

    def row_sqnorm(self, Z, sq, p):
        _mat(Z, "Z")
        _lib.check(self.lib.vgan_row_sqnorm(_ptr(Z), Z.stride(0), _ptr(sq), Z.shape[0], int(p), self._stream()), "vgan_row_sqnorm")

    def mmd_gram(self, Z, sq, n, p, bw, tiles, calibrate, Wg, wrow0, partial):
        _mat(Z, "Z")
        assert (calibrate or Z.shape[0] >= 2 * n) and tiles.dtype == torch.int32 and tiles.is_contiguous()
        ntiles = tiles.shape[0]
        assert partial.numel() >= 4 * ntiles
        ldw = Wg.stride(0) if Wg is not None else 0
        _lib.check(self.lib.vgan_mmd_gram(_ptr(Z), Z.stride(0), _ptr(sq), int(n), int(p), _ptr(bw), _ptr(tiles), ntiles,
                                          int(bool(calibrate)), _ptr(Wg), ldw, int(wrow0), _ptr(partial), self._stream()),
                   "vgan_mmd_gram")

    @staticmethod
    def _mults(multipliers):
        vals = [float(v) for v in multipliers]
        return (ctypes.c_float * len(vals))(*vals), len(vals)

    def mmd_gram_general(self, Z, sq, n, p, bw, tiles, multipliers, Wg, wrow0, partial):
        _mat(Z, "Z")
        ntiles = tiles.shape[0]
        assert partial.numel() >= 4 * ntiles
        arr, nk = self._mults(multipliers)
        ldw = Wg.stride(0) if Wg is not None else 0
        _lib.check(self.lib.vgan_mmd_gram_general(_ptr(Z), Z.stride(0), _ptr(sq), int(n), int(p), _ptr(bw), _ptr(tiles), ntiles, arr, nk,
                                                  _ptr(Wg), ldw, int(wrow0), _ptr(partial), self._stream()), "vgan_mmd_gram_general")

    def rbf_multi_kernel_matrix(self, Z, sq, bw, multipliers, K, dK=None):
        _mat(Z, "Z"), _mat(K, "K")
        m, p = Z.shape
        arr, nk = self._mults(multipliers)
        _lib.check(self.lib.vgan_rbf_multi_kernel_matrix(_ptr(Z), Z.stride(0), m, p, _ptr(sq), _ptr(bw), arr, nk, _ptr(K), K.stride(0),
                                                         _ptr(dK), dK.stride(0) if dK is not None else 0, self._stream()),
                   "vgan_rbf_multi_kernel_matrix")

    def mmd_gram_colmax(self, Z, sq, n, p, bw, tiles, Wg, wrow0, partial, S, row_offset, colpart, from_softmax=True):
        _mat(Z, "Z"), _mat(S, "S")
        ntiles = tiles.shape[0]
        nrows, d = S.shape
        assert partial.numel() >= 4 * ntiles and colpart.dtype == torch.int64 and colpart.numel() >= self.colmax_chunks(nrows) * d
        ldw = Wg.stride(0) if Wg is not None else 0
        _lib.check(self.lib.vgan_mmd_gram_colmax(_ptr(Z), Z.stride(0), _ptr(sq), int(n), int(p), _ptr(bw), _ptr(tiles), ntiles,
                                                 _ptr(Wg), ldw, int(wrow0), _ptr(partial), _ptr(S), S.stride(0),
                                                 int(bool(from_softmax)), int(row_offset), _ptr(colpart), nrows, d, self._stream()),
                   "vgan_mmd_gram_colmax")

    def mmd_reduce(self, partial, tiles, stats, zero_first=True):
        assert stats.dtype == torch.float64 and stats.numel() >= 4
        _lib.check(self.lib.vgan_mmd_reduce(_ptr(partial), _ptr(tiles), tiles.shape[0], _ptr(stats), int(bool(zero_first)),
                                            self._stream()), "vgan_mmd_reduce")

    def mmd_set_bandwidth(self, stats, n, bw):
        _lib.check(self.lib.vgan_mmd_set_bandwidth(_ptr(stats), int(n), _ptr(bw), self._stream()), "vgan_mmd_set_bandwidth")

    def mmd_loss(self, stats, colkey, n, d, weight, loss, loss_accum=None, accum_scale=1.0, step_counter=None):
        _lib.check(self.lib.vgan_mmd_loss(_ptr(stats), _ptr(colkey), int(n), int(d), float(weight), _ptr(loss), _ptr(loss_accum),
                                          float(accum_scale), _ptr(step_counter), self._stream()), "vgan_mmd_loss")

    def mmd_backward(self, Wg, Z, wrow0, nr, ncols, p, mul, out, splits=1, slab_stride=0, finalize=None, mul_shift=None):
        _mat(Wg, "Wg"), _mat(Z, "Z"), _mat(out, "out")
        ldmul = mul.stride(0) if mul is not None else 0
        _lib.check(self.lib.vgan_mmd_backward(_ptr(Wg), Wg.stride(0), _ptr(Z), Z.stride(0), int(wrow0), int(nr), int(ncols), int(p),
                                              _ptr(mul), ldmul, _ptr(mul_shift), _ptr(out), out.stride(0), int(splits), int(slab_stride),
                                              ctypes.byref(finalize) if finalize is not None else None, self._stream()),
                   "vgan_mmd_backward")

    def mmd_bf3_prepare(self, Z, rows, p, Zh, Zl, ZTh=None, ZTl=None):
        _mat(Z, "Z")
        for t in (Zh, Zl, ZTh, ZTl):
            assert t is None or (t.dtype == torch.int16 and t.is_cuda and t.stride(1) == 1)
        kn = ZTh.stride(0) if ZTh is not None else 0
        _lib.check(self.lib.vgan_mmd_bf3_prepare(_ptr(Z), Z.stride(0), int(rows), int(p), _ptr(Zh), _ptr(Zl), Zh.stride(0),
                                                 _ptr(ZTh), _ptr(ZTl), kn, self._stream()), "vgan_mmd_bf3_prepare")

    def gram_tail_workspace(self, device):
        return torch.zeros(int(self.lib.vgan_mmd_gram_bf3_tail_ws_bytes()) // 4, dtype=torch.int32, device=device)

    def mmd_gram_bf3(self, Zh, Zl, sq, n, bw, tiles, Wh, Wl, wrow0, partial, S=None, row_offset=0, colpart=None, from_softmax=True,
                     tile=64, tail_ws=None, rs_part=None):
        ntiles = tiles.shape[0]
        nrows, d = (S.shape if S is not None else (0, 0))
        ldw = Wh.stride(0) if Wh is not None else 0
        _lib.check(self.lib.vgan_mmd_gram_bf3(_ptr(Zh), _ptr(Zl), Zh.stride(0), _ptr(sq), int(n), _ptr(bw), _ptr(tiles), ntiles,
                                              int(tile), _ptr(Wh), _ptr(Wl), ldw, int(wrow0), _ptr(partial), _ptr(S),
                                              S.stride(0) if S is not None else 0, int(bool(from_softmax)), int(row_offset),
                                              _ptr(colpart), nrows, d, _ptr(tail_ws), tail_ws.numel() * 4 if tail_ws is not None else 0,
                                              _ptr(rs_part), rs_part.stride(0) if rs_part is not None else 0, self._stream()),
                   "vgan_mmd_gram_bf3")

    def mmd_backward_bf3(self, Wh, Wl, ZTh, ZTl, Z, wrow0, nr, p, mul, out, splits=1, slab_stride=0, finalize=None, mul_shift=None,
                         tile=0):
        _mat(Z, "Z"), _mat(out, "out")
        ldmul = mul.stride(0) if mul is not None else 0
        _lib.check(self.lib.vgan_mmd_backward_bf3(_ptr(Wh), _ptr(Wl), Wh.stride(0), _ptr(ZTh), _ptr(ZTl), ZTh.stride(0),
                                                  ZTh.shape[0], _ptr(Z), Z.stride(0), int(wrow0), int(nr), int(p), _ptr(mul), ldmul,
                                                  _ptr(mul_shift), _ptr(out), out.stride(0), int(splits), int(slab_stride), int(tile),
                                                  ctypes.byref(finalize) if finalize is not None else None, self._stream()),
                   "vgan_mmd_backward_bf3")

    def mmd_backward_bf3_rm(self, Wh, Wl, Zh, Zl, zrows, Z, wrow0, nr, p, mul, out, splits=1, slab_stride=0, finalize=None, mul_shift=None,
                            tile=0, xx=None, rs_part=None):
        _mat(Z, "Z"), _mat(out, "out")
        ldmul = mul.stride(0) if mul is not None else 0
        kn = (int(zrows) + 63) // 64 * 64
        assert Wh.stride(0) >= kn and Zh.shape[0] >= zrows
        if xx is not None:
            assert tile in (0, 64)
            _lib.check(self.lib.vgan_mmd_backward_bf3_rm_xx(_ptr(Wh), _ptr(Wl), Wh.stride(0), kn, _ptr(Zh), _ptr(Zl), Zh.stride(0), int(zrows),
                                                            _ptr(Z), Z.stride(0), int(wrow0), int(nr), int(p), _ptr(mul), ldmul, _ptr(mul_shift),
                                                            _ptr(out), out.stride(0), int(splits), int(slab_stride),
                                                            ctypes.byref(finalize) if finalize is not None else None, ctypes.byref(xx),
                                                            self._stream()), "vgan_mmd_backward_bf3_rm_xx")
            return
        _lib.check(self.lib.vgan_mmd_backward_bf3_rm(_ptr(Wh), _ptr(Wl), Wh.stride(0), kn, _ptr(Zh), _ptr(Zl), Zh.stride(0), int(zrows),
                                                     _ptr(Z), Z.stride(0), int(wrow0), int(nr), int(p), _ptr(mul), ldmul, _ptr(mul_shift),
                                                     _ptr(out), out.stride(0), int(splits), int(slab_stride), int(tile),
                                                     ctypes.byref(finalize) if finalize is not None else None, _ptr(rs_part),
                                                     rs_part.stride(0) if rs_part is not None else 0, self._stream()),
                   "vgan_mmd_backward_bf3_rm")

    def mmd_backward_bf3_rm_rebuild(self, Wh, Wl, Zh, Zl, zrows, nr, p, rebuild, out, splits=1, slab_stride=0, finalize=None, xx=None):
        _mat(out, "out")
        kn = (int(zrows) + 63) // 64 * 64
        assert Wh.stride(0) >= kn and Zh.shape[0] >= zrows
        _lib.check(self.lib.vgan_mmd_backward_bf3_rm_rebuild(_ptr(Wh), _ptr(Wl), Wh.stride(0), kn, _ptr(Zh), _ptr(Zl), Zh.stride(0), int(zrows),
                                                             int(nr), int(p), ctypes.byref(rebuild), _ptr(out), out.stride(0), int(splits),
                                                             int(slab_stride), ctypes.byref(finalize) if finalize is not None else None,
                                                             ctypes.byref(xx) if xx is not None else None, self._stream()),
                   "vgan_mmd_backward_bf3_rm_rebuild")

    def mmd_backward_bf3_tile(self, nr, p, splits=1, tile=0):
        return int(self.lib.vgan_mmd_backward_bf3_tile(int(nr), int(p), int(splits), int(tile)))

    def gemm_grouped(self, problems, copy=None, adadelta=None, noise=None, fold=None, kparts=None, ksplit_ws=None):
        assert 1 <= len(problems) <= _lib.GEMM_MAX_GROUP
        if kparts is not None and all(int(v) == 1 for v in kparts):
            kparts = None
        arr = self._gemm_problems(problems)
        if kparts is None and copy is None and adadelta is None and noise is None and fold is None:
            _lib.check(self.lib.vgan_gemm_grouped(arr, len(problems), self._stream()), "vgan_gemm_grouped")
            return
        x = self._grouped_extras(len(problems), copy, adadelta, noise, fold)
        if kparts is not None:
            assert len(kparts) == len(problems)
            kp = (ctypes.c_int32 * len(problems))(*[int(v) for v in kparts])
            _lib.check(self.lib.vgan_gemm_grouped_ksplit(arr, len(problems), ctypes.byref(x), kp, _ptr(ksplit_ws),
                                                         0 if ksplit_ws is None else ksplit_ws.numel() * ksplit_ws.element_size(),
                                                         self._stream()), "vgan_gemm_grouped_ksplit")
            return
        _lib.check(self.lib.vgan_gemm_grouped_ex(arr, len(problems), ctypes.byref(x), self._stream()), "vgan_gemm_grouped_ex")

    def gemm_grouped_ksplit_ws_bytes(self, problems, kparts):
        kp = (ctypes.c_int32 * len(problems))(*[int(v) for v in kparts])
        return int(self.lib.vgan_gemm_grouped_ksplit_ws_bytes(self._gemm_problems(problems), len(problems), kp))

    def _gemm_problems(self, problems):
        arr = (_lib.GemmProblem * len(problems))()
        for q, (kind, A, B, C, *rest) in zip(arr, problems):
            if kind == "NT2":
                D, scratch = rest
                _mat(A, "A"), _mat(B, "B"), _mat(C, "C"), _mat(D, "D")
                (m, k), (k2, kb), (n, k2d) = A.shape, B.shape, D.shape
                assert k == kb and k2 == k2d and tuple(C.shape) == (m, n)
                tiles = ((m + 63) // 64) * ((n + 63) // 64)
                assert scratch.is_cuda and scratch.dtype == _f32 and scratch.is_contiguous() and scratch.numel() >= tiles * 64 * _round4(k2)
                q.a, q.b, q.c, q.d, q.scratch = A.data_ptr(), B.data_ptr(), C.data_ptr(), D.data_ptr(), scratch.data_ptr()
                q.kind, q.m, q.n, q.k, q.k2, q.splitk = _lib.GEMM_NT_NT, m, n, k, k2, 1
                q.lda, q.ldb, q.ldc, q.ldd = A.stride(0), B.stride(0), C.stride(0), D.stride(0)
                continue
            q.splitk = int(rest[0]) if rest else 1
            if q.splitk > 1:
                assert C.dim() == 3 and C.shape[0] == q.splitk and C.is_contiguous()
                C = C[0]
            _mat(A, "A"), _mat(B, "B"), _mat(C, "C")
            if kind == "NN":
                (m, k), (k2, n), code = A.shape, B.shape, _lib.GEMM_NN
            elif kind == "NT":
                (m, k), (n, k2), code = A.shape, B.shape, _lib.GEMM_NT
            elif kind == "TN":
                (k, m), (k2, n), code = A.shape, B.shape, _lib.GEMM_TN
            else:
                raise ValueError(kind)
            assert k == k2 and tuple(C.shape) == (m, n), (kind, tuple(A.shape), tuple(B.shape), tuple(C.shape))
            q.a, q.b, q.c, q.kind, q.m, q.n, q.k = A.data_ptr(), B.data_ptr(), C.data_ptr(), code, m, n, k
            q.lda, q.ldb, q.ldc = A.stride(0), B.stride(0), C.stride(0)
        return arr

    def _grouped_extras(self, nproblems, copy, adadelta, noise, fold):
        x = _lib.GroupedExtras()
        if copy is not None:
            src, dst = copy
            _vec(src, "copy src"), _vec(dst, "copy dst")
            assert src.numel() == dst.numel()
            x.copy_src, x.copy_dst, x.copy_count = src.data_ptr(), dst.data_ptr(), src.numel()
        if adadelta is not None:
            a = adadelta
            for nm in ("p", "sq", "acc"):
                _vec(a[nm], nm)
            x.adadelta, x.p, x.sq_avg, x.acc_delta = 1, a["p"].data_ptr(), a["sq"].data_ptr(), a["acc"].data_ptr()
            x.lr, x.rho, x.eps, x.weight_decay, x.grad_scale = (float(a["lr"]), float(a.get("rho", 0.9)), float(a.get("eps", 1e-6)),
                                                                float(a.get("weight_decay", 0.0)), float(a.get("grad_scale", 1.0)))
            extra = a.get("extra_grad")
            assert len(a["layers"]) == nproblems + (1 if extra is not None else 0)
            for L, (w, off_w, off_b, out, inp) in zip(x.layer, a["layers"]):
                _mat(w, "w_packed")
                L.w_packed, L.off_w, L.off_b, L.ldp, L.out, L.inp = w.data_ptr(), int(off_w), int(off_b), w.stride(0), int(out), int(inp)
            if extra is not None:
                _mat(extra, "extra_grad")
                x.g_extra, x.ld_extra = extra.data_ptr(), extra.stride(0)
        if noise is not None:
            z = noise["next_noise"]
            x.next_noise, x.noise_rows, x.noise_ld = z.data_ptr(), z.shape[0], z.stride(0)
            x.noise_cols, x.noise_ones_col = int(noise["noise_cols"]), int(noise["noise_ones_col"])
            x.seed, x.step_counter = int(noise["seed"]) & 0xFFFFFFFFFFFFFFFF, noise["step_counter"].data_ptr()
        if fold is not None:
            x.fold = ctypes.addressof(fold)
        return x

    def mse_grad(self, target, pred, gscale, part, g):
        _mat(target, "target"), _mat(pred, "pred"), _mat(g, "g")
        n, d = pred.shape
        assert part.dtype == torch.float64 and part.numel() >= (n + 3) // 4
        _lib.check(self.lib.vgan_mse_grad(_ptr(target), target.stride(0), _ptr(pred), pred.stride(0), n, d, float(gscale), _ptr(part),
                                          _ptr(g), g.stride(0), self._stream()), "vgan_mse_grad")

    def sum_f64(self, src, count, scale, out, accumulate=False):
        assert src.dtype == torch.float64
        _lib.check(self.lib.vgan_sum_f64(_ptr(src), int(count), float(scale), _ptr(out), int(bool(accumulate)), self._stream()),
                   "vgan_sum_f64")

    def rbf_kernel_matrix(self, Z, sq, alpha, K):
        _mat(Z, "Z"), _mat(K, "K")
        m, p = Z.shape
        _lib.check(self.lib.vgan_rbf_kernel_matrix(_ptr(Z), Z.stride(0), m, p, _ptr(sq), float(alpha), _ptr(K), K.stride(0),
                                                   self._stream()), "vgan_rbf_kernel_matrix")

    def rows_dot(self, A, B, out, broadcast_b=False):
        _mat(A, "A")
        rows, cols = A.shape
        assert out.dtype == torch.float64 and out.numel() >= rows
        ldb = 0 if broadcast_b else B.stride(0)
        _lib.check(self.lib.vgan_rows_dot(_ptr(A), A.stride(0), _ptr(B), ldb, _ptr(out), rows, cols, self._stream()), "vgan_rows_dot")

    def dp_unique_id(self):
        buf = (ctypes.c_uint8 * 128)()
        _lib.check(self.lib.vgan_dp_unique_id(ctypes.cast(buf, ctypes.c_void_p)), "vgan_dp_unique_id")
        return bytes(buf)

    def dp_comm_create(self, nranks, unique_id, rank):
        comm = ctypes.c_void_p()
        buf = (ctypes.c_uint8 * 128).from_buffer_copy(unique_id)
        _lib.check(self.lib.vgan_dp_comm_create(ctypes.byref(comm), int(nranks), ctypes.cast(buf, ctypes.c_void_p), int(rank)),
                   "vgan_dp_comm_create")
        return comm

    def dp_allreduce_sum(self, comm, t):
        _vec(t, "t")
        _lib.check(self.lib.vgan_dp_allreduce_sum(comm, _ptr(t), t.numel(), self._stream()), "vgan_dp_allreduce_sum")

    def dp_allgather(self, comm, t, nranks):
        assert t.is_cuda and t.is_contiguous() and t.shape[0] % nranks == 0
        _lib.check(self.lib.vgan_dp_allgather(comm, _ptr(t), t.numel() * t.element_size() // nranks, self._stream()), "vgan_dp_allgather")

    def dp_comm_destroy(self, comm):
        _lib.check(self.lib.vgan_dp_comm_destroy(comm), "vgan_dp_comm_destroy")

    def shuffle_epoch(self, perm, train_size, seed, epoch):
        _vec(perm, "perm", torch.int32)
        _lib.check(self.lib.vgan_shuffle_epoch(_ptr(perm), perm.numel(), int(train_size), int(seed) & 0xFFFFFFFFFFFFFFFF,
                                               int(epoch) & 0xFFFFFFFFFFFFFFFF, self._stream()), "vgan_shuffle_epoch")

    def shuffle_index(self, i, train_size, seed, epoch):
        return int(self.lib.vgan_shuffle_index(int(i), int(train_size), int(seed) & 0xFFFFFFFFFFFFFFFF, int(epoch) & 0xFFFFFFFFFFFFFFFF))

    def mask_unique(self, masks):
        assert masks.is_cuda and masks.dtype == torch.bool and masks.dim() == 2
        m8 = masks.contiguous().view(torch.uint8)
        n, d = m8.shape
        dev = masks.device
        keys = torch.empty(n * ((d + 63) // 64), dtype=torch.int64, device=dev)
        work = torch.empty(2 * n, dtype=torch.int32, device=dev)
        out_row = torch.zeros(n, dtype=torch.int32, device=dev)
# ... 428 lines not shown
```

v-gan_amd/trainer.py:

```python
import contextlib
import gc
import os

import torch

ADADELTA_RHO = 0.9
ADADELTA_EPS = 1e-6


@contextlib.contextmanager
def no_gc_while_capturing():
    was_enabled = gc.isenabled()
    gc.collect()
    gc.disable()
    try:
        yield
    finally:
        if was_enabled:
            gc.enable()


def _round4(v):
    return (v + 3) // 4 * 4


def _launch_rounds(tiles, slots, can_split):
    if tiles <= 0:
        return 0.0
    full, r = divmod(tiles, slots)
    if r == 0:
        return float(full)
    x = r / slots
    last = 0.55 if x <= 0.5 else 0.55 + 0.9 * (x - 0.5)
    if can_split and x <= 0.125:
        last = 0.25
    elif can_split and x <= 0.25:
        last = 0.4
    elif can_split and x <= 0.5:
        last = 0.5
    return full + last


def _best_boundary(n_main, total, slots, can_split):
    cost = lambda k: _launch_rounds(k, slots, can_split) + _launch_rounds(total - k, slots, can_split)
    best, best_cost = n_main, cost(n_main)
    for k in range(n_main - 1, max(n_main - slots, 0), -1):
        c = cost(k)
        if c < best_cost - 1e-9 and c <= cost(n_main) - 0.15:
            best, best_cost = k, c
    return best


CHAIN_KPARTS_AUTO = 4


def chain_kparts(want, tiles, k, chain_flops=False):
    if want != "auto":
        parts = int(want)
        if parts not in (1, 2, 4, 8):
            raise ValueError(f"VGAN_CHAIN_KPARTS must be auto, 1, 2, 4 or 8, got {want!r}")
        return parts
    if chain_flops or not (32 <= tiles <= 64 and k >= 768):
        return 1
    return CHAIN_KPARTS_AUTO


class FlatParams:

    def __init__(self, params, device):
        self.shapes = [tuple(p.shape) for p in params]
        self.offsets = []
        off = 0
        for p in params:
            self.offsets.append(off)
            off += _round4(p.numel())
        self.total = off
        self.flat = torch.zeros(off, dtype=torch.float32, device=device)
        self.grad = torch.zeros_like(self.flat)
        self.sq = torch.zeros_like(self.flat)
        self.acc = torch.zeros_like(self.flat)
        for k, (p, o) in enumerate(zip(params, self.offsets)):
            self.flat[o:o + p.numel()].copy_(p.detach().reshape(-1).to(device=device, dtype=torch.float32))
            p.data = self.view(self.flat, k)

    def view(self, buf, k):
        o, shp = self.offsets[k], self.shapes[k]
        numel = 1
        for s in shp:
            numel *= s
        return buf[o:o + numel].view(shp)


class NoKLStepEngine:
    def __init__(self, ops, generator, data, batch_size, batches_per_epoch, lr=0.007, weight_decay=0.04, penalty_weight=10.0,
                 seed=777, noise="device", rank=0, world=1, group=None, use_graph=True, loss_accum_scale=None,
                 generator_mode=None, force_exchange=False, mmd_precision=None, center_operand=True, overlap_exchange=None,
                 fuse_update=None, front=None, chain_assoc=None):
        self.ops = ops
        self.dev = data.device
        self.rank, self.world, self.group = rank, world, group
        self.exchange = world > 1 or bool(force_exchange)
        n = self.n = int(batch_size)
        if n % world != 0:
            raise ValueError(f"global batch {n} must be divisible by the number of ranks {world}")
        nl = self.nl = n // world
        self.lo = rank * nl
        self.data = data
        d = self.d = data.shape[1]
        dp = self.dp = _round4(d)
        self.nb = int(batches_per_epoch)
        self.lr, self.wd, self.pen = float(lr), float(weight_decay), float(penalty_weight)
        self.seed = int(seed)
        self.noise_mode = noise
        self.use_graph = bool(use_graph) and data.is_cuda
        self.graph = None
        self.graph_multi = None
        self.graph_blocks = {}
        self.steps_per_graph = max(1, min(16, int(batches_per_epoch)))
        self.steps_done = 0
        self._xx_primed = False
        self._coalesce = None
        self.mode = generator_mode or os.environ.get("VGAN_GENERATOR", "collapsed")
        if self.mode not in ("collapsed", "layered"):
            raise ValueError(f"generator_mode must be 'collapsed' or 'layered', got {self.mode!r}")
        self.fuse_update = (os.environ.get("VGAN_FUSE_UPDATE", "0") == "1") if fuse_update is None else bool(fuse_update)
        want_front = front or os.environ.get("VGAN_DP_FRONT", "auto")
        if want_front not in ("auto", "replicated", "sharded"):
            raise ValueError(f"front must be 'auto', 'replicated' or 'sharded', got {want_front!r}")
        if want_front == "sharded" and not (self.exchange and self.mode == "collapsed"):
            raise ValueError("front='sharded' needs a data-parallel engine (world > 1 or force_exchange) with the collapsed generator")
        self.front_sharded = (self.exchange and self.mode == "collapsed" and
                              (want_front == "sharded" or (want_front == "auto" and n * data.shape[1] >= (1 << 22))))

        lin = [m for m in generator.main if isinstance(m, torch.nn.Linear)]
        assert len(lin) == 4
        L = self.L = lin[0].in_features
        self.widths = [L] + [m.out_features for m in lin]
        params = [q for m in lin for q in (m.weight, m.bias)]
        self.fp = FlatParams(params, self.dev)
        self.W = [self.fp.view(self.fp.flat, 2 * k) for k in range(4)]
        self.b = [self.fp.view(self.fp.flat, 2 * k + 1) for k in range(4)]

        f32 = dict(dtype=torch.float32, device=self.dev)
        self.splits = max(1, min(8, nl // 128))
        self.e = [_round4(w + 1) for w in self.widths]
        self.za = torch.zeros(n, self.e[0], **f32)
        self.za[:, L] = 1.0
        self.z_own = self.za[self.lo:self.lo + nl]
        self.logits = torch.zeros(n, d, **f32)
        self.chain_flops = False
        if self.mode == "layered":
            self.gslab = torch.zeros(self.splits, self.fp.total, **f32) if self.splits > 1 else None
            gbase = self.gslab[0] if self.splits > 1 else self.fp.grad
            self.dW = [self.fp.view(gbase, 2 * k) for k in range(4)]
            self.db = [self.fp.view(gbase, 2 * k + 1) for k in range(4)]
            self.acts = [self.za[:, :L]] + [torch.zeros(n, w, **f32) for w in self.widths[1:4]] + [self.logits]
            self.acts_own = [a[self.lo:self.lo + nl] for a in self.acts]
            self.dacts = [None] + [torch.zeros(nl, w, **f32) for w in self.widths[1:4]]
        else:
            e = self.e
            poff = [0]
            for k in range(1, 5):
                poff.append(poff[-1] + e[k] * e[k - 1])
            self.Wt_all = torch.zeros(poff[-1], **f32)
            self.Gt_all = torch.zeros(poff[-1], **f32)
            self.Wt = [None] + [self.Wt_all[poff[k - 1]:poff[k]].view(e[k], e[k - 1]) for k in range(1, 5)]
            self.Gt = [None] + [self.Gt_all[poff[k - 1]:poff[k]].view(e[k], e[k - 1]) for k in range(1, 5)]
            self.At = [None, self.Wt[1]] + [torch.zeros(e[k], e[0], **f32) for k in range(2, 5)]
            self.M = [None, self.Gt[1]] + [torch.zeros(e[k], e[0], **f32) for k in range(2, 5)]
            self.B3 = torch.zeros(e[4], e[2], **f32)
            self.B2 = torch.zeros(e[4], e[1], **f32)
            self.At1s = torch.zeros(e[1], e[0], **f32)
            want_assoc = chain_assoc or os.environ.get("VGAN_CHAIN_ASSOC", "auto")
            if want_assoc not in ("auto", "depth", "flops"):
                raise ValueError(f"chain_assoc must be 'auto', 'depth' or 'flops', got {want_assoc!r}")
            self.chain_flops = want_assoc == "flops" or (want_assoc == "auto" and 2.0 * e[4] * e[3] * e[2] >= 1e9)
            if self.chain_flops:
                self.fuse_update = False
                def split_of(m, n_, k):
                    t64 = ((m + 63) // 64) * ((n_ + 63) // 64)
                    return 1 if 2.0 * m * n_ * k < 2.5e8 else max(1, min(8, 1024 // t64, k // 256))
                self.fwd_split = {k: split_of(e[k], e[0], e[k - 1]) for k in (2, 3, 4)}
                self.bwd_split = {k: split_of(e[k - 1], e[0], e[k]) for k in (4, 3, 2)}
                if os.environ.get("VGAN_CHAIN_SPLITK", "1") != "1":
                    self.fwd_split, self.bwd_split = {k: 1 for k in (2, 3, 4)}, {k: 1 for k in (4, 3, 2)}
                need = max([self.fwd_split[k] * e[k] * e[0] for k in (2, 3, 4)] + [self.bwd_split[k] * e[k - 1] * e[0] for k in (4, 3, 2)])
                self.chain_ws = torch.zeros(need, **f32)
            pmap = torch.full((self.fp.total,), -1, dtype=torch.int32)
            for k in range(1, 5):
                wk, wk1 = self.widths[k], self.widths[k - 1]
                r = torch.arange(wk, dtype=torch.int32)[:, None] * e[k - 1]
                ow, ob = self.fp.offsets[2 * (k - 1)], self.fp.offsets[2 * (k - 1) + 1]
                pmap[ow:ow + wk * wk1] = (poff[k - 1] + r + torch.arange(wk1, dtype=torch.int32)[None, :]).reshape(-1)
                pmap[ob:ob + wk] = (poff[k - 1] + r + wk1).reshape(-1)
            self.pmap = pmap.to(self.dev)
            self.pack_layers = [(self.W[k - 1], self.b[k - 1], self.Wt[k]) for k in range(1, 5)]
            self.unpack_layers = [(self.fp.view(self.fp.grad, 2 * (k - 1)), self.fp.view(self.fp.grad, 2 * (k - 1) + 1), self.Gt[k])
                                  for k in range(1, 5)]
            ops.homogeneous_pack(self.pack_layers, unpack=False)

        self.precision = mmd_precision or os.environ.get("VGAN_MMD_PRECISION", "auto")
        if self.precision not in ("auto", "fp32", "bf16x3"):
            raise ValueError(f"mmd_precision must be 'auto', 'fp32' or 'bf16x3', got {self.precision!r}")
        if self.precision == "auto":
            self.precision = "bf16x3" if 2 * n * d >= (1 << 20) else "fp32"
        self.bf3 = self.precision == "bf16x3"
        self.center = torch.zeros(dp, **f32)
        if center_operand:
            ops.col_mean(data, self.center)
        self.bwd_tile = int(os.environ.get("VGAN_BWD_TILE", "0"))
        self._fin = None
        self.S = torch.zeros(n, d, **f32)
        self.S_own = self.S[self.lo:self.lo + nl]
        self.Z = torch.zeros(2 * n, dp, **f32)
        self.sqn = torch.zeros(2 * n, **f32)
        self.sq_cal = torch.zeros(2 * n, **f32) if self.bf3 else self.sqn
        self.Wg = torch.zeros(nl, 2 * n, **f32)
        out_tiles = ((nl + 63) // 64) * ((d + 63) // 64)
        auto_splits = max(2 if self.bf3 else 1, min(4, 256 // max(out_tiles, 1), max(1, (2 * n) // 64)))
        rm = self.front_sharded or os.environ.get("VGAN_BWD_OPERAND", "rowmajor") != "transposed"
        if self.bf3 and rm and self.bwd_tile in (0, 256) and ops.mmd_backward_bf3_tile(nl, d, 1, self.bwd_tile) == 256:
            auto_splits = 1
        self.bsplits = max(1, int(os.environ.get("VGAN_BWD_SPLITS", str(auto_splits))))
        self.gU_slabs = torch.zeros(self.bsplits, nl, dp, **f32)
        self.gU = self.gU_slabs[0]
        self.dlogits_pad = torch.zeros(nl, dp, **f32)
        self.dlogits = self.dlogits_pad[:, :d]
        self.rm_backward = True
        if self.precision == "bf16x3":
            i16 = dict(dtype=torch.int16, device=self.dev)
            self.kp, self.kn = (d + 63) // 64 * 64, (2 * n + 63) // 64 * 64
            self.Zh, self.Zl = torch.zeros(2 * n, self.kp, **i16), torch.zeros(2 * n, self.kp, **i16)
            self.rm_backward = self.front_sharded or os.environ.get("VGAN_BWD_OPERAND", "rowmajor") != "transposed"
            if self.rm_backward:
                self.ZTh = self.ZTl = None
            else:
                self.ZTh, self.ZTl = torch.zeros(self.kp, self.kn, **i16), torch.zeros(self.kp, self.kn, **i16)
            self.Wh, self.Wl = torch.zeros(nl, self.kn, **i16), torch.zeros(nl, self.kn, **i16)
        self.fused_prepare = (self.bf3 and not self.front_sharded and ops.bf3_fusable(n, d, self.logits.stride(0), data.stride(0), dp) and
                              os.environ.get("VGAN_FUSED_PREPARE", "1") == "1")
        self.chain_in_mask = (self.mode == "collapsed" and not self.front_sharded and ops.chain_fusable(n, d, data.stride(0), dp) and
                              (not self.bf3 or self.fused_prepare) and os.environ.get("VGAN_CHAIN_IN_MASK", "0") == "1")
        self._chain = None
        self.two_stage_logits = (self.mode == "collapsed" and not self.chain_flops and not self.chain_in_mask and not self.front_sharded and
                                 os.environ.get("VGAN_LOGITS_2STAGE", "0") == "1")
        if self.two_stage_logits:
            e2 = self.e[2]
            self.T = torch.zeros(n, e2, **f32)
            self.T_ws = torch.zeros(((n + 63) // 64) * ((e2 + 63) // 64) * 64 * _round4(self.e[1]), **f32)
        self.perm = torch.zeros(self.nb, n, dtype=torch.int32, device=self.dev)
        self.perm_next = torch.zeros_like(self.perm)
        self.epoch_staged = False
        self.gram_tile = 64
        want = os.environ.get("VGAN_GRAM_TILE", "auto")
        if self.bf3 and nl % 128 == 0 and want in ("auto", "128"):
            if want == "128" or len(ops.build_tiles(n, 1, rank, world, device=self.dev, tile=128)) >= 512:
                self.gram_tile = 128
        if self.bf3 and nl % 256 == 0 and want in ("auto", "256"):
            if want == "256" or len(ops.build_tiles(n, 1, rank, world, device=self.dev, tile=256)) >= 512:
                self.gram_tile = 256
        self.gram_tail_ws = (ops.gram_tail_workspace(self.dev)
                             if self.gram_tile == 256 and os.environ.get("VGAN_GRAM_TAIL", "1") != "0" else None)
        self.rs_part = None
        if (self.gram_tile == 256 and self.rm_backward and n % 128 == 0 and os.environ.get("VGAN_RS_FROM_GRAM", "1") != "0"
                and ops.mmd_backward_bf3_tile(nl, d, self.bsplits, self.bwd_tile) == 256):
            self.rs_part = torch.zeros((2 * n + 127) // 128, nl, **f32)
        if overlap_exchange is None and os.environ.get("VGAN_OVERLAP") is not None:
            overlap_exchange = {"1": True, "0": False}.get(os.environ["VGAN_OVERLAP"], os.environ["VGAN_OVERLAP"])
        self.overlap = False if overlap_exchange is None else bool(overlap_exchange)
        if self.front_sharded and self.overlap:
            raise ValueError("overlap_exchange and front='sharded' are two schedules of the same exchange: choose one")
        self._side = torch.cuda.Stream(device=self.dev) if (self.overlap and data.is_cuda and overlap_exchange != "serial") else None
        self.x_ahead = self.overlap and (not self.bf3 or self.rm_backward)
        self.xx_ride = False
        self._xx = None
        if (self.fused_prepare and self.gram_tile == 64 and not self.overlap and self.rm_backward and
                os.environ.get("VGAN_XX_RIDE", "0") == "1"):
            split, n_main = ops.build_tiles(n, 1, rank, world, device=self.dev, tile=64, split_xx=True)
            xx_tiles = split.shape[0] - n_main
            self.xx_ride = xx_tiles > 0 and 8 * ((n // 8 + 7) // 8) + xx_tiles <= 512
        if self.xx_ride:
            i16 = dict(dtype=torch.int16, device=self.dev)
            rows_total = data.shape[0]
            self.Dh, self.Dl = torch.zeros(rows_total, self.kp, **i16), torch.zeros(rows_total, self.kp, **i16)
            self.dsq = torch.zeros(rows_total, **f32)
            ops.gather_rows_split(data, None, self.center, None, self.dsq, True, self.Dh, self.Dl, n=rows_total)
        self.xx_in_m4 = (self.bf3 and self.mode == "collapsed" and self.gram_tile == 64 and not self.overlap and not self.xx_ride and
                         not self.front_sharded and
                         ops.linear_backward_params_xx_supported(nl, self.e[0], dp) and os.environ.get("VGAN_XX_IN_M4", "1") == "1")
        self._xx_m4 = self._fold = None
        if self.front_sharded:
            self.tiles, self.n_main = ops.build_tiles(n, 1, rank, world, device=self.dev, tile=self.gram_tile, split="yy_last")
            slots = 256 if self.gram_tile >= 128 else (512 if self.bf3 else 1024)
            self.n_main = _best_boundary(self.n_main, self.tiles.shape[0], slots, self.gram_tail_ws is not None)
        elif self.overlap or self.xx_ride or self.xx_in_m4:
            self.tiles, self.n_main = ops.build_tiles(n, 1, rank, world, device=self.dev, tile=self.gram_tile, split_xx=True)
            if self.xx_in_m4:
                slots = int(os.environ.get("VGAN_GRAM_SLOTS", "512"))
                self.n_main = min(self.tiles.shape[0], max(self.n_main, slots))
                if self.n_main == self.tiles.shape[0]:
                    self.xx_in_m4 = False
        else:
            self.tiles = ops.build_tiles(n, 1, rank, world, device=self.dev, tile=self.gram_tile)
            self.n_main = self.tiles.shape[0]
        self.xx_late_in_backward = False
        if self.xx_in_m4 and self.rm_backward and os.environ.get("VGAN_XX_LATE", "backward") == "backward":
            late = self.tiles.shape[0] - self.n_main
            bwd_wgs = ((d + 63) // 64) * ((nl + 63) // 64) * self.bsplits + 1
            self.xx_late_in_backward = (ops.mmd_backward_bf3_tile(nl, d, self.bsplits, self.bwd_tile) == 64 and late <= 512 - bwd_wgs)
        self.m4_kparts = self.tn_kparts = 1
        self.m4_ws = self.tn_ws = None
        if self.mode == "collapsed" and getattr(ops, "chain_ksplit", False):
            want_kp = os.environ.get("VGAN_CHAIN_KPARTS", "auto")
            e = self.e
            t32 = lambda rows, cols: ((rows + 31) // 32) * ((cols + 31) // 32)
            if not (self.xx_in_m4 and not self.xx_late_in_backward):
                self.m4_kparts = chain_kparts(want_kp, t32(dp, e[0]), nl, self.chain_flops)
            tn_tiles = sum(t32(e[k], e[0]) for k in (3, 2, 1))
            if not self.chain_flops and e[4] >= 96 and tn_tiles <= 256:
                self.tn_kparts = chain_kparts(want_kp, tn_tiles, e[4])
            if self.m4_kparts > 1:
                self.m4_ws = ops.ksplit_workspace(ops.linear_backward_params_ksplit_ws_bytes(e[0], dp, self.m4_kparts), self.dev)
            if self.tn_kparts > 1:
                tn = [("TN", self.Wt[4], self.M[4], self.M[3]), ("TN", self.B3, self.M[4], self.M[2]), ("TN", self.B2, self.M[4], self.M[1])]
                self.tn_ws = ops.ksplit_workspace(ops.gemm_grouped_ksplit_ws_bytes(tn, [self.tn_kparts] * 3), self.dev)
        plain_bf3 = (getattr(ops, "bf3_rebuild", False) and self.bf3 and self.fused_prepare and self.gram_tile == 64 and
                     self.rm_backward and world == 1 and not self.overlap and not self.front_sharded and
                     ops.mmd_backward_bf3_tile(nl, d, self.bsplits, self.bwd_tile) == 64)
        self.lean = plain_bf3 and os.environ.get("VGAN_Z_FP32", "0") != "1"
        self.xrow = torch.zeros(n, dtype=torch.int32, device=self.dev) if self.lean else None
        self._rebuild = None
        self.tiles_cal = self.tiles if (world == 1 and self.gram_tile == 64 and not (self.overlap or self.xx_ride or self.xx_in_m4 or self.front_sharded)) else ops.build_tiles(n, 0, 0, 1, device=self.dev)
        self.partial = torch.zeros(max(self.tiles.shape[0], self.tiles_cal.shape[0]), 4, **f32)
        self.stats = torch.zeros(4, dtype=torch.float64, device=self.dev)
        self.bw = torch.zeros(1, **f32)
        self.has_bw = False
        self.loss = torch.zeros(1, **f32)
        self.loss_accum = torch.zeros(1, **f32)
        self._hist, self._hist_n, self._hist_events = None, 0, []
        self._read_stream, self._loss_host = None, None
        self.accum_scale = (1.0 / self.nb) if loss_accum_scale is None else float(loss_accum_scale)
        self.step_counter = torch.zeros(1, dtype=torch.int64, device=self.dev)
        self.col_chunks = (world * ops.colmax_chunks(nl)) if self.front_sharded else ops.colmax_chunks(n)
        self.colpart = torch.zeros(self.col_chunks * d, dtype=torch.int64, device=self.dev)
        own = ops.colmax_chunks(nl) * d
        self.colpart_own = self.colpart[rank * own:(rank + 1) * own] if self.front_sharded else self.colpart
        self.colkey = torch.zeros(d, dtype=torch.int64, device=self.dev)
        if self.front_sharded and data.is_cuda and self._collect().is_initialized():
            self._coalesce = self._probe_coalescing(self._collect())

    def set_epoch_batches(self, idx):
        if os.environ.get("VGAN_FEED_DIRECT") == "1":
            self.perm.copy_(idx.to(dtype=torch.int32), non_blocking=True)
            self._after_new_epoch_table()
            return
        self.stage_epoch_batches(idx)
        self.begin_epoch()

    def stage_epoch_batches(self, idx):
        self.perm_next.copy_(idx.to(dtype=torch.int32).view(self.nb, self.n), non_blocking=True)
        self.epoch_staged = True

    def begin_epoch(self):
        if not self.epoch_staged:
            raise RuntimeError("begin_epoch without a staged table (stage_epoch_batches)")
        self.perm.copy_(self.perm_next)
        self.epoch_staged = False
        self._after_new_epoch_table()

    def _after_new_epoch_table(self):
        if self.overlap and self.has_bw:
            self._prefetch_xx()

    def _prefetch_xx(self):
        self._prefetch_x_operand()
        self._xx_tiles()
        self._xx_primed = True

    def _prefetch_x_operand(self):
        ops, n = self.ops, self.n
        rowsel = dict(row_cursor=self.step_counter, row_batches=self.nb, row_stride=n)
        if self.bf3:
            ops.gather_rows_split(self.data, self.perm, self.center, self.Z[:n], self.sqn[:n], True, self.Zh[:n], self.Zl[:n], **rowsel)
        else:
            ops.gather_rows_split(self.data, self.perm, self.center, self.Z[:n], self.sqn[:n], False, **rowsel)

    def _xx_tiles(self):
        ops, n = self.ops, self.n
        ntx = self.tiles.shape[0] - self.n_main
        if ntx == 0:
            return
        tx, px = self.tiles[self.n_main:], self.partial[self.n_main:self.n_main + ntx]
        if self.bf3:
            ops.mmd_gram_bf3(self.Zh, self.Zl, self.sqn, n, self.bw, tx, None, None, 0, px, tile=self.gram_tile)
        else:
            ops.mmd_gram(self.Z, self.sqn, n, self.dp, self.bw, tx, False, None, 0, px)

    def _fork_prefetch(self):
        if not self.overlap:
            return
        if self._side is None:
            self._prefetch_xx()
            return
        self._side.wait_stream(torch.cuda.current_stream())
        with torch.cuda.stream(self._side):
            self._prefetch_xx()

    def _join_prefetch(self):
        if self.overlap and self._side is not None:
            torch.cuda.current_stream().wait_stream(self._side)

    def shuffle_epoch(self, epoch):
        self.ops.shuffle_epoch(self.perm, self.data.shape[0], self.seed, int(epoch))
        self._after_new_epoch_table()

    def set_bandwidth(self, value):
        self.bw.fill_(float(value))
        self.has_bw = True

    def set_noise(self, z):
        self.za[:, :self.L].copy_(z.to(dtype=torch.float32), non_blocking=True)

    def epoch_loss(self):
        v = float(self._sum_over_ranks(self.loss_accum).item())
        self.loss_accum.zero_()
        return v

    def close_epoch(self):
        if self._hist is None or self._hist_n == self._hist.numel():
            grown = torch.zeros(max(64, 2 * self._hist_n), dtype=torch.float32, device=self.dev)
            if self._hist is not None:
                grown[:self._hist_n].copy_(self._hist)
            self._hist = grown
        slot = self._hist_n
        cell = self._hist[slot:slot + 1]
        cell.copy_(self.loss_accum)
        self.loss_accum.zero_()
        if self.exchange:
            self._collect().all_reduce(cell, group=self.group)
        ev = None
        if self.data.is_cuda:
            ev = torch.cuda.Event()
            ev.record()
        self._hist_events.append(ev)
        self._hist_n += 1
        return slot

    def read_epoch_loss(self, slot):
        ev = self._hist_events[slot]
        if ev is None:
            return float(self._hist[slot])
        if self._read_stream is None:
            self._read_stream = torch.cuda.Stream(self.dev)
            self._loss_host = torch.zeros(1, dtype=torch.float32).pin_memory()
        self._read_stream.wait_event(ev)
        with torch.cuda.stream(self._read_stream):
            self._loss_host.copy_(self._hist[slot:slot + 1], non_blocking=True)
        self._read_stream.synchronize()
        return float(self._loss_host[0])

    def step_loss(self):
        return float(self._sum_over_ranks(self.loss).item())

    def _sum_over_ranks(self, t):
        if not self.exchange:
            return t
        t = t.clone()
        self._collect().all_reduce(t, group=self.group)
        return t

    def grad_view(self, k):
        if self.mode == "collapsed":
            self.ops.homogeneous_pack(self.unpack_layers, unpack=True)
        elif not self.exchange and self.splits > 1:
            return sum(self.fp.view(self.gslab[sl], k) for sl in range(self.splits))
        return self.fp.view(self.fp.grad, k)

    def _generator_forward(self, own_rows=False):
        ops = self.ops
        if self.mode == "layered":
            for k in range(4):
# ... 10 lines not shown
                    ops.gemm_grouped([("NN", Wt[k], At[k - 1], At[k])])
        elif self.two_stage_logits:
            ops.gemm_grouped([("NN", Wt[2], At[1], At[2]), ("NN", Wt[4], Wt[3], self.B3), ("NT2", self.za, Wt[1], self.T, Wt[2], self.T_ws)])
            ops.gemm_grouped([("NN", Wt[3], At[2], At[3]), ("NN", self.B3, Wt[2], self.B2), ("NT", self.T, self.B3[:self.d], self.logits)])
            return
        else:
            ops.gemm_grouped([("NN", Wt[2], At[1], At[2]), ("NN", Wt[4], Wt[3], self.B3)])
            ops.gemm_grouped([("NN", Wt[3], At[2], At[3]), ("NN", self.B3, At[2], At[4]), ("NN", self.B3, Wt[2], self.B2)])
        if own_rows:
            ops.linear_forward(self.z_own, At[4][:self.d], None, self.logits[self.lo:self.lo + self.nl])
        elif not self.chain_in_mask:
            ops.linear_forward(self.za, At[4][:self.d], None, self.logits)

    def _slabs(self, splits, like):
        return self.chain_ws[:splits * like.numel()].view(splits, like.shape[0], like.shape[1])

    def _generator_backward_update(self, dist):
        ops = self.ops
        adadelta = dict(lr=self.lr, rho=ADADELTA_RHO, eps=ADADELTA_EPS, weight_decay=self.wd, grad_scale=1.0)
        if self.mode == "layered":
            g = self.dlogits
            for k in (3, 2, 1, 0):
                ops.linear_backward_params(g, self.acts_own[k], self.dW[k], self.db[k], self.splits, self.fp.total)
                if k:
                    ops.linear_backward_input(g, self.W[k], self.dacts[k])
                    g = self.dacts[k]
            if dist:
                if self.splits > 1:
                    ops.reduce_slabs(self.gslab, self.fp.total, self.splits, self.fp.grad)
                dist.all_reduce(self.fp.grad, group=self.group)
                ops.adadelta_step(self.fp.flat, self.fp.grad, self.fp.sq, self.fp.acc, **adadelta)
            elif self.splits > 1:
                ops.adadelta_step(self.fp.flat, self.gslab[0], self.fp.sq, self.fp.acc, nslabs=self.splits, slab_stride=self.fp.total,
                                  **adadelta)
            else:
                ops.adadelta_step(self.fp.flat, self.fp.grad, self.fp.sq, self.fp.acc, **adadelta)
            return
        e, d = self.e, self.d
        if self.xx_in_m4 and not self.xx_late_in_backward:
            ops.linear_backward_params_xx(self.dlogits_pad, self.z_own, self.M[4][:self.dp], self._late_xx_job())
        elif self.m4_kparts > 1:
            ops.linear_backward_params_ksplit(self.dlogits_pad, self.z_own, self.M[4][:self.dp], self.m4_kparts, self.m4_ws)
        else:
            ops.linear_backward_params(self.dlogits_pad, self.z_own, self.M[4][:self.dp], None)
        if dist:
            dist.all_reduce(self.M[4], group=self.group)
        M, Gt, At = self.M, self.Gt, self.At
        fused_noise = dict(next_noise=self.za, noise_cols=self.L, noise_ones_col=self.L, seed=self.seed,
                           step_counter=self.step_counter) if self.noise_mode == "device" else {}
        if self.chain_flops:
            Wt = self.Wt
            for k in (4, 3, 2):
                sp = self.bwd_split[k]
                probs = [("TN", Wt[k], M[k], self._slabs(sp, M[k - 1]), sp) if sp > 1 else ("TN", Wt[k], M[k], M[k - 1])]
                if k < 4:
                    probs.append(("NT", M[k + 1], At[k], Gt[k + 1]))
                ops.gemm_grouped(probs, fold=self._fold if (self.xx_in_m4 and k == 4) else None)
                if sp > 1:
                    ops.reduce_slabs(self.chain_ws, M[k - 1].numel(), sp, M[k - 1])
            ops.gemm_grouped([("NT", M[2], At[1], Gt[2])])
            ops.adadelta_step_packed(self.fp.flat, self.pmap, self.Gt_all, self.Wt_all, self.fp.sq, self.fp.acc, **adadelta, **fused_noise)
            return
        tn_split = dict(kparts=[self.tn_kparts] * 3, ksplit_ws=self.tn_ws) if self.tn_kparts > 1 else {}
        if not self.fuse_update:
            ops.gemm_grouped([("TN", self.Wt[4], M[4], M[3]), ("TN", self.B3, M[4], M[2]), ("TN", self.B2, M[4], M[1])],
                             fold=self._fold if self.xx_in_m4 else None, **tn_split)
            ops.gemm_grouped([("NT", M[4], At[3], Gt[4]), ("NT", M[3], At[2], Gt[3]), ("NT", M[2], At[1], Gt[2])])
            ops.adadelta_step_packed(self.fp.flat, self.pmap, self.Gt_all, self.Wt_all, self.fp.sq, self.fp.acc, **adadelta, **fused_noise)
            return
        ops.gemm_grouped([("TN", self.Wt[4], M[4], M[3]), ("TN", self.B3, M[4], M[2]), ("TN", self.B2, M[4], M[1])],
                         copy=(self.Wt[1], self.At1s), fold=self._fold if self.xx_in_m4 else None, **tn_split)
        w, off = self.widths, self.fp.offsets
        layers = [(self.Wt[k], off[2 * (k - 1)], off[2 * (k - 1) + 1], w[k], w[k - 1]) for k in (4, 3, 2, 1)]
        ops.gemm_grouped([("NT", M[4], At[3], Gt[4]), ("NT", M[3], At[2], Gt[3]), ("NT", M[2], self.At1s, Gt[2])],
                         adadelta=dict(p=self.fp.flat, sq=self.fp.sq, acc=self.fp.acc, layers=layers, extra_grad=Gt[1], **adadelta),
                         noise=fused_noise or None)

    def _collect(self):
        import torch.distributed as dist
        return dist

    def _forward(self):
        ops, n, nl, lo = self.ops, self.n, self.nl, self.lo
        if self.noise_mode == "device" and (self.mode == "layered" or self.steps_done == 0):
            ops.noise_normal(self.za, self.seed, self.step_counter, 0, cols=self.L, ones_col=self.L)
        self._generator_forward()
        rowsel = dict(row_cursor=self.step_counter, row_batches=self.nb, row_stride=n)
        logits = self.logits
        if self.chain_in_mask:
            if self._chain is None:
                self._chain = ops.logits_chain(self.za, self.At[4][:self.d])
            rowsel["chain"] = self._chain
            logits = None
        if self.fused_prepare:
            xx = None
            if self.xx_ride and self.has_bw:
                if self._xx is None:
                    ntx = self.tiles.shape[0] - self.n_main
                    self._xx = ops.xx_job(self.Dh, self.Dl, self.dsq, self.tiles[self.n_main:], self.bw, self.partial[self.n_main:self.n_main + ntx])
                xx = self._xx
            if self.lean:
                ops.mask_project_forward_bf3(logits, self.data, self.perm, self.S, self.Z, self.sqn, self.Zh, self.Zl, None, None,
                                             center=self.center, xx=xx, write_z=not self.has_bw, xrow=self.xrow, **rowsel)
            else:
                ops.mask_project_forward_bf3(logits, self.data, self.perm, self.S, self.Z, self.sqn, self.Zh, self.Zl, self.ZTh, self.ZTl,
                                             center=self.center, write_x=not self.x_ahead, xx=xx, **rowsel)
            return
        if self.x_ahead:
            ops.mask_project_forward(logits, self.data, self.perm, self.S, None, None, self.Z[n:], None, self.sqn[n:],
                                     row_offset=0, center=self.center, norm_split=self.bf3, **rowsel)
        else:
            ops.mask_project_forward(logits, self.data, self.perm, self.S, None, self.Z[:n], self.Z[n:], self.sqn[:n], self.sqn[n:],
                                     row_offset=0, center=self.center, norm_split=self.bf3, **rowsel)

    def _calibrate(self):
        ops = self.ops
        if self.bf3:
            ops.row_sqnorm(self.Z, self.sq_cal, self.dp)
        ops.mmd_gram(self.Z, self.sq_cal, self.n, self.dp, None, self.tiles_cal, True, None, 0, self.partial)
        ops.mmd_reduce(self.partial, self.tiles_cal, self.stats, True)
        ops.mmd_set_bandwidth(self.stats, self.n, self.bw)
        self.has_bw = True

    def _loss_backward_update(self):
        ops, n, nl, lo, d = self.ops, self.n, self.nl, self.lo, self.d
        dist = self._collect() if self.exchange else None
        gstride = nl * self.dp
        bf3 = self.precision == "bf16x3"
        if bf3 and not self.fused_prepare:
            if self.x_ahead:
                ops.mmd_bf3_prepare(self.Z[n:], n, d, self.Zh[n:], self.Zl[n:])
            else:
                ops.mmd_bf3_prepare(self.Z, 2 * n, d, self.Zh, self.Zl, self.ZTh, self.ZTl)
        if bf3:
            ops.mmd_gram_bf3(self.Zh, self.Zl, self.sqn, n, self.bw, self.tiles[:self.n_main], self.Wh, self.Wl, n + lo, self.partial, self.S, 0,
                             self.colpart, True, tile=self.gram_tile, tail_ws=self.gram_tail_ws, rs_part=self.rs_part)
        else:
            ops.mmd_gram_colmax(self.Z, self.sqn, n, self.dp, self.bw, self.tiles[:self.n_main], self.Wg, n + lo, self.partial, self.S, 0,
                                self.colpart, True)
        if self._fin is None:
            fin_args = (self.partial, self.tiles, self.colpart, ops.colmax_chunks(n), self.colkey, n, d, self.pen if self.rank == 0 else 0.0,
                        self.stats, self.loss, self.loss_accum, self.accum_scale, self.step_counter)
            if self.xx_in_m4:
                self._fin = ops.finalize_job(*fin_args, mode=1, ntiles_main=self.n_main)
                self._fold = ops.finalize_job(*fin_args, mode=2, ntiles_main=self.n_main)
            else:
                self._fin = ops.finalize_job(*fin_args)
        fin = self._fin
        if bf3:
            if self.lean:
                if self._rebuild is None:
                    self._rebuild = ops.bwd_rebuild(self.data, self.xrow, self.S, self.center)
                ops.mmd_backward_bf3_rm_rebuild(self.Wh, self.Wl, self.Zh, self.Zl, 2 * n, nl, d, self._rebuild, self.gU, self.bsplits, gstride,
                                                fin, xx=self._late_xx_job() if self.xx_late_in_backward else None)
            elif self.rm_backward:
                ops.mmd_backward_bf3_rm(self.Wh, self.Wl, self.Zh, self.Zl, 2 * n, self.Z, n + lo, nl, d, self.Z[lo:lo + nl], self.gU,
                                        self.bsplits, gstride, fin, mul_shift=self.center, tile=self.bwd_tile,
                                        xx=self._late_xx_job() if self.xx_late_in_backward else None, rs_part=self.rs_part)
            else:
                ops.mmd_backward_bf3(self.Wh, self.Wl, self.ZTh, self.ZTl, self.Z, n + lo, nl, d, self.Z[lo:lo + nl], self.gU, self.bsplits,
                                     gstride, fin, mul_shift=self.center, tile=self.bwd_tile)
        else:
            ops.mmd_backward(self.Wg, self.Z, n + lo, nl, 2 * n, self.dp, self.Z[lo:lo + nl], self.gU, self.bsplits, gstride, fin,
                             mul_shift=self.center)
        self._fork_prefetch()
        ops.mask_backward(self.gU, self.S_own, self.colkey, self.pen, lo, self.dlogits, self.bsplits, gstride)
        self._generator_backward_update(dist)
        self._join_prefetch()

    def _forward_sharded(self):
        ops, n, nl, lo, d = self.ops, self.n, self.nl, self.lo, self.d
        if self.noise_mode == "device" and self.steps_done == 0:
            ops.noise_normal(self.za, self.seed, self.step_counter, 0, cols=self.L, ones_col=self.L)
        self._generator_forward(own_rows=True)
        rowsel = dict(row_cursor=self.step_counter, row_batches=self.nb, row_stride=n)
        own, yown = slice(lo, lo + nl), slice(n + lo, n + lo + nl)
        if self.bf3:
            ops.gather_rows_split(self.data, self.perm, self.center, None, self.sqn[:n], True, self.Zh[:n], self.Zl[:n], **rowsel)
        else:
            ops.gather_rows_split(self.data, self.perm, self.center, self.Z[:n], self.sqn[:n], False, **rowsel)
        ops.mask_project_forward(self.logits[own], self.data, self.perm, self.S_own, None, self.Z[own] if self.bf3 else None, self.Z[yown],
                                 None, self.sqn[yown], row_offset=lo, center=self.center, norm_split=self.bf3, **rowsel)
        if self.bf3:
            ops.mmd_bf3_prepare(self.Z[yown], nl, d, self.Zh[yown], self.Zl[yown])
        ops.colmax_partial(self.S_own, lo, self.colpart_own)

    def _all_gather(self, dist, out, own):
        size = dist.get_world_size(self.group) if dist.is_initialized() else 1
        if size != self.world:
            out = own
        if own.is_cuda and dist.get_backend(self.group) == "gloo":
            host = out.cpu()
            dist.all_gather_into_tensor(host, own.cpu(), group=self.group)
            out.copy_(host)
            return None
        return dist.all_gather_into_tensor(out, own, group=self.group, async_op=True)

    def _exchange_front(self, dist):
        n, nl, lo = self.n, self.nl, self.lo
        yown = slice(n + lo, n + lo + nl)
        pairs = []
        if self.bf3:
            pairs += [(img[n:2 * n].view(torch.int32), img[yown].view(torch.int32)) for img in (self.Zh, self.Zl)]
        else:
            pairs.append((self.Z[n:], self.Z[yown]))
        pairs += [(self.sqn[n:], self.sqn[yown]), (self.colpart, self.colpart_own)]
        if self._coalesce is None:
            self._coalesce = self._probe_coalescing(dist)
        if self._coalesce:
            emulated = dist.get_world_size(self.group) != self.world
            with dist._coalescing_manager(group=self.group, device=self.dev, async_ops=True) as cm:
                for out, own in pairs:
                    dist.all_gather_into_tensor(own if emulated else out, own, group=self.group)
            return [cm]
        return [self._all_gather(dist, out, own) for out, own in pairs]

    def _probe_coalescing(self, dist):
        if os.environ.get("VGAN_DP_COALESCE", "0") != "1" or not self.data.is_cuda or torch.cuda.is_current_stream_capturing():
            return False
        try:
            if dist.get_backend(self.group) != "nccl" or not hasattr(dist, "_coalescing_manager"):
                return False
            size = dist.get_world_size(self.group)
            a, b = torch.zeros(size * 4, device=self.dev), torch.zeros(size * 2, dtype=torch.int64, device=self.dev)
            r = dist.get_rank(self.group)
            with dist._coalescing_manager(group=self.group, device=self.dev, async_ops=True) as cm:
                dist.all_gather_into_tensor(a, a[4 * r:4 * r + 4], group=self.group)
                dist.all_gather_into_tensor(b, b[2 * r:2 * r + 2], group=self.group)
            cm.wait()
            torch.cuda.synchronize()
            return True
        except Exception as e:
            import warnings
            warnings.warn(f"vgan_amd: coalesced all-gather is not available on this stack ({type(e).__name__}: {e}); one launch per gather")
            return False

    def _loss_backward_update_sharded(self, all_rows_here=False):
        ops, n, nl, lo, d = self.ops, self.n, self.nl, self.lo, self.d
        dist = self._collect()
        works = []
        if all_rows_here:
            if self.bf3:
                ops.mmd_bf3_prepare(self.Z, 2 * n, d, self.Zh, self.Zl)
            self.colpart.zero_()
            ops.colmax_partial(self.S, 0, self.colpart[:ops.colmax_chunks(n) * d])
        else:
            works = self._exchange_front(dist)
        na = self.n_main

        def gram(t0, t1):
            if t1 <= t0:
                return
            if self.bf3:
                ops.mmd_gram_bf3(self.Zh, self.Zl, self.sqn, n, self.bw, self.tiles[t0:t1], self.Wh, self.Wl, n + lo, self.partial[t0:t1],
                                 tile=self.gram_tile, tail_ws=self.gram_tail_ws, rs_part=self.rs_part)
            else:
                ops.mmd_gram(self.Z, self.sqn, n, self.dp, self.bw, self.tiles[t0:t1], False, self.Wg, n + lo, self.partial[t0:t1])

        gram(0, na)
        for w in works:
            if w is not None:
                w.wait()
        gram(na, self.tiles.shape[0])
        if self._fin is None:
            self._fin = ops.finalize_job(self.partial, self.tiles, self.colpart, self.col_chunks, self.colkey, n, d,
                                         self.pen if self.rank == 0 else 0.0, self.stats, self.loss, self.loss_accum, self.accum_scale,
                                         self.step_counter)
        gstride = nl * self.dp
        if self.bf3:
            ops.mmd_backward_bf3_rm(self.Wh, self.Wl, self.Zh, self.Zl, 2 * n, self.Z, n + lo, nl, d, self.Z[lo:lo + nl], self.gU,
                                    self.bsplits, gstride, self._fin, mul_shift=self.center, tile=self.bwd_tile, rs_part=self.rs_part)
        else:
            ops.mmd_backward(self.Wg, self.Z, n + lo, nl, 2 * n, self.dp, self.Z[lo:lo + nl], self.gU, self.bsplits, gstride, self._fin,
                             mul_shift=self.center)
        ops.mask_backward(self.gU, self.S_own, self.colkey, self.pen, lo, self.dlogits, self.bsplits, gstride)
        self._generator_backward_update(dist)

    def _late_xx_job(self):
        if self._xx_m4 is None:
            ntx = self.tiles.shape[0] - self.n_main
            self._xx_m4 = self.ops.xx_job(self.Zh, self.Zl, self.sqn, self.tiles[self.n_main:], self.bw,
                                          self.partial[self.n_main:self.n_main + ntx])
        return self._xx_m4

    def _step_body(self):
        if self.front_sharded:
            self._forward_sharded()
            self._loss_backward_update_sharded()
        else:
            self._forward()
            self._loss_backward_update()

    def step(self):
        if not self.has_bw:
            if self.overlap:
                self._prefetch_x_operand()
            self._forward()
            self._calibrate()
            if self.overlap or self.xx_ride:
                self._xx_tiles()
                self._xx_primed = True
            if self.front_sharded:
                self._loss_backward_update_sharded(all_rows_here=True)
            else:
                self._loss_backward_update()
        elif self.use_graph and self.steps_done > 0:
            if self.graph is None:
# ... 71 lines not shown
```

Measured before the change: 9297 steps/s.

## Add tall 128x64 bf16x3 backward tile for mid-sized grids

Adds a GemmBF3Tall loop: 8-wave workgroups computing 128x64 output tiles with a register prefetch ring. The tile heuristic picks it when the 64-tile grid would exceed 256 workgroups and the tall grid fits within 256. The intent is to fit the backward MMD contraction into a single wave of workgroups with more reuse per tile. The lean rebuild and X-X-late paths are plumbed to accept the new tile. In exchange, each workgroup does more work, fewer workgroups run at once, and the slot budget for X-X tiles shrinks.

After: 9455 steps/s, median of 6. About the same (+1.7%).

```diff
diff --git a/include/vgan_hip.h b/include/vgan_hip.h
--- a/include/vgan_hip.h
+++ b/include/vgan_hip.h
@@ -123,6 +123,7 @@
                       int wrow0, float* partial, const float* S, int lds, int from_softmax, int row_offset,
                       uint64_t* colpart, int nrows, int d, void* tail_ws, int64_t tail_ws_bytes,
                       float* rs_part, int ldrs, vgan_stream_t stream);
+#define VGAN_BWD_TILE_TALL 192
 int vgan_mmd_backward_bf3_tile(int nr, int p, int splits, int tile);
 int vgan_mmd_backward_bf3(const uint16_t* Wh, const uint16_t* Wl, int ldw, const uint16_t* ZTh,
                           const uint16_t* ZTl, int kn, int kp, const float* Z, int ldz, int wrow0, int nr,
@@ -139,6 +140,11 @@
                                 int p, const float* mul, int ldmul, const float* mul_shift, float* out, int ldo,
                                 int splits, int64_t slab_stride, const vgan_finalize_job* finalize,
                                 const struct vgan_xx_job* xx, vgan_stream_t stream);
+int vgan_mmd_backward_bf3_rm_xx_tile(const uint16_t* Wh, const uint16_t* Wl, int ldw, int kn, const uint16_t* Zh,
+                                     const uint16_t* Zl, int kp, int zrows, const float* Z, int ldz, int wrow0, int nr,
+                                     int p, const float* mul, int ldmul, const float* mul_shift, float* out, int ldo,
+                                     int splits, int64_t slab_stride, int tile, const vgan_finalize_job* finalize,
+                                     const struct vgan_xx_job* xx, vgan_stream_t stream);
 typedef struct vgan_bwd_rebuild {
     const float* data;
     const int32_t* xrow;
@@ -151,6 +157,11 @@
                                      const vgan_bwd_rebuild* rebuild, float* out, int ldo, int splits,
                                      int64_t slab_stride, const vgan_finalize_job* finalize,
                                      const struct vgan_xx_job* xx, vgan_stream_t stream);
+int vgan_mmd_backward_bf3_rm_rebuild_tile(const uint16_t* Wh, const uint16_t* Wl, int ldw, int kn, const uint16_t* Zh,
+                                          const uint16_t* Zl, int kp, int zrows, int nr, int p,
+                                          const vgan_bwd_rebuild* rebuild, float* out, int ldo, int splits,
+                                          int64_t slab_stride, int tile, const vgan_finalize_job* finalize,
+                                          const struct vgan_xx_job* xx, vgan_stream_t stream);
 #define VGAN_GEMM_MAX_GROUP 4
 #define VGAN_GEMM_NN 0
 #define VGAN_GEMM_NT 1
diff --git a/v-gan_amd/csrc/gemm_bf3.hpp b/v-gan_amd/csrc/gemm_bf3.hpp
--- a/v-gan_amd/csrc/gemm_bf3.hpp
+++ b/v-gan_amd/csrc/gemm_bf3.hpp
@@ -306,6 +306,187 @@
             }
             __syncthreads();
         }
+    }
+};
+
+
+template <int WAVES, int AHEAD>
+struct GemmBF3Tall {
+    static_assert((WAVES == 4 || WAVES == 8) && AHEAD >= 1 && AHEAD <= 4, "");
+    static constexpr int BM = 128, BN = 64, BK = 64, NTH = 64 * WAVES;
+    static constexpr int MI = 8 / WAVES;
+    static constexpr int NRA = 128 * 8 / NTH;
+    static constexpr int NRB = 64 * 8 / NTH;
+    static constexpr int QPR = BK / 8;
+    static constexpr int KS = BK / 16;
+    static constexpr int ROWB = (BK + 8) * 2;
+    static constexpr int PARTA = BM * ROWB;
+    static constexpr int PARTB = 64 * 128;
+    static constexpr int BUF = 2 * PARTA + 2 * PARTB;
+    static constexpr int kLdsBytes = 2 * BUF;
+    typedef char __attribute__((address_space(3))) lds_c;
+
+    struct Vals {
+        u32x4 va[2][NRA], vb[2][NRB];
+        __device__ __forceinline__ float a_rowpart(int r) const {
+            float s = 0.f;
+            const unsigned* h = reinterpret_cast<const unsigned*>(&va[0][r]);
+            const unsigned* l = reinterpret_cast<const unsigned*>(&va[1][r]);
+#pragma unroll
+            for (int e = 0; e < 4; ++e) {
+                s += __uint_as_float(h[e] << 16) + __uint_as_float(h[e] & 0xFFFF0000u);
+                s += __uint_as_float(l[e] << 16) + __uint_as_float(l[e] & 0xFFFF0000u);
+            }
+            return s;
+        }
+    };
+    struct Stage {
+        const char* srcA[2][NRA];
+        const unsigned short *Bh, *Bl;
+        long ldb;
+        int lofsA[NRA], lofsB[NRB], rowB[NRB], colB[NRB], zrows;
+        __device__ __forceinline__ void init(const unsigned short* Ah, const unsigned short* Al, long lda, int m0, int M,
+                                             const unsigned short* Bh_, const unsigned short* Bl_, long ldb_, int n0, int zrows_, int tid) {
+            Bh = Bh_; Bl = Bl_; ldb = ldb_; zrows = zrows_;
+#pragma unroll
+            for (int r = 0; r < NRA; ++r) {
+                const int f = tid + NTH * r, row = f / QPR, q = f % QPR;
+                const long ra = (long)min(m0 + row, M - 1) * lda + 8 * q;
+                srcA[0][r] = reinterpret_cast<const char*>(Ah + ra);
+                srcA[1][r] = reinterpret_cast<const char*>(Al + ra);
+                lofsA[r] = row * ROWB + q * 16;
+            }
+#pragma unroll
+            for (int r = 0; r < NRB; ++r) {
+                const int f = tid + NTH * r, row = f / QPR, q = f % QPR;
+                rowB[r] = row;
+                colB[r] = n0 + 8 * q;
+                lofsB[r] = row * 128 + ((q ^ (((row >> 1) & 1) << 2)) << 4);
+            }
+        }
+        __device__ __forceinline__ void load(Vals& v, int k0) const {
+#pragma unroll
+            for (int r = 0; r < NRA; ++r) {
+                v.va[0][r] = *reinterpret_cast<const u32x4*>(srcA[0][r] + 2 * (long)k0);
+                v.va[1][r] = *reinterpret_cast<const u32x4*>(srcA[1][r] + 2 * (long)k0);
+            }
+#pragma unroll
+            for (int r = 0; r < NRB; ++r) {
+                const long ob = (long)min(k0 + rowB[r], zrows - 1) * ldb + colB[r];
+                v.vb[0][r] = *reinterpret_cast<const u32x4*>(Bh + ob);
+                v.vb[1][r] = *reinterpret_cast<const u32x4*>(Bl + ob);
+            }
+        }
+        __device__ __forceinline__ void store(const Vals& v, lds_c* buf) const {
+#pragma unroll
+            for (int r = 0; r < NRA; ++r) {
+                *(lds_u4*)(buf + lofsA[r]) = v.va[0][r];
+                *(lds_u4*)(buf + PARTA + lofsA[r]) = v.va[1][r];
+            }
+#pragma unroll
+            for (int r = 0; r < NRB; ++r) {
+                *(lds_u4*)(buf + 2 * PARTA + lofsB[r]) = v.vb[0][r];
+                *(lds_u4*)(buf + 2 * PARTA + PARTB + lofsB[r]) = v.vb[1][r];
+            }
+        }
+    };
+
+    template <bool SIDE_A>
+    __device__ static __forceinline__ void run_bt(const unsigned short* Ah, const unsigned short* Al, long lda, const unsigned short* Bh,
+                                                  const unsigned short* Bl, long ldb, int zrows, int m0, int n0, int M, int K,
+                                                  char* lds_generic, float* rs_generic, f32x16 (&acc)[MI]) {
+        lds_c* lds = (lds_c*)lds_generic;
+        lds_f* rs_lds = (lds_f*)rs_generic;
+        const int tid = threadIdx.x, lane = tid & 63, wave = tid >> 6;
+        const int wm0 = (wave >> 1) * 32 * MI, wn0 = (wave & 1) * 32;
+        const int fi = lane & 31, fh = lane >> 5;
+        const int g = lane >> 4, li = lane & 15, qq = li >> 2, pp = li & 3;
+        const int chunk = (wn0 >> 3) + 2 * (g & 1) + (pp >> 1);
+        const int offB0 = (8 * (g >> 1) + qq) * 128 + ((chunk ^ (((qq >> 1) & 1) << 2)) << 4) + (pp & 1) * 8;
+        Stage st;
+        st.init(Ah, Al, lda, m0, M, Bh, Bl, ldb, n0, zrows, tid);
+        Vals ring[AHEAD];
+        float rsum[NRA];
+#pragma unroll
+        for (int r = 0; r < NRA; ++r) rsum[r] = 0.f;
+        auto side = [&](const Vals& v) {
+#pragma unroll
+            for (int r = 0; r < NRA; ++r) rsum[r] += v.a_rowpart(r);
+        };
+        const int nk = K / BK;
+        auto load_tile = [&](Vals& v, int t) { st.load(v, min(t, nk - 1) * BK); };
+        load_tile(ring[0], 0);
+        st.store(ring[0], lds);
+        if constexpr (SIDE_A) side(ring[0]);
+#pragma unroll
+        for (int j = 1; j <= AHEAD; ++j) load_tile(ring[j % AHEAD], j);
+        __syncthreads();
+        auto body = [&](int kt, Vals& next, auto more) {
+            const lds_c* buf = lds + (kt & 1) * BUF;
+            const lds_c* pa = buf + (wm0 + fi) * ROWB + fh * 16;
+            const lds_c* pb = buf + 2 * PARTA + offB0;
+            u32x4 ah[KS][MI], al[KS][MI];
+            bf16x8 yh[KS], yl[KS];
+#pragma unroll
+            for (int s = 0; s < KS; ++s) {
+#pragma unroll
+                for (int i = 0; i < MI; ++i) {
+                    ah[s][i] = *(const lds_u4*)(pa + i * 32 * ROWB + s * 32);
+                    al[s][i] = *(const lds_u4*)(pa + PARTA + i * 32 * ROWB + s * 32);
+                }
+                yh[s] = tr_read_k8(pb + s * 2048, 512);
+                yl[s] = tr_read_k8(pb + PARTB + s * 2048, 512);
+            }
+            if constexpr (decltype(more)::value) {
+                st.store(next, lds + ((kt & 1) ^ 1) * BUF);
+                if constexpr (SIDE_A) side(next);
+                load_tile(next, kt + 1 + AHEAD);
+            }
+#pragma unroll
+            for (int s = 0; s < KS; ++s) {
+                bf16x8 xh[MI], xl[MI];
+#pragma unroll
+                for (int i = 0; i < MI; ++i) {
+                    xh[i] = __builtin_bit_cast(bf16x8, ah[s][i]);
+                    xl[i] = __builtin_bit_cast(bf16x8, al[s][i]);
+                }
+#pragma unroll
+                for (int i = 0; i < MI; ++i) acc[i] = __builtin_amdgcn_mfma_f32_32x32x16_bf16(xl[i], yh[s], acc[i], 0, 0, 0);
+#pragma unroll
+                for (int i = 0; i < MI; ++i) acc[i] = __builtin_amdgcn_mfma_f32_32x32x16_bf16(xh[i], yl[s], acc[i], 0, 0, 0);
+#pragma unroll
+                for (int i = 0; i < MI; ++i) acc[i] = __builtin_amdgcn_mfma_f32_32x32x16_bf16(xh[i], yh[s], acc[i], 0, 0, 0);
+            }
+            __builtin_amdgcn_iglp_opt(0);
+            __syncthreads();
+        };
+        using T = std::true_type;
+        using F = std::false_type;
+        for (int kt0 = 0; kt0 < nk - 1; kt0 += AHEAD) {
+#pragma unroll
+            for (int j = 0; j < AHEAD; ++j)
+                if (kt0 + j < nk - 1) body(kt0 + j, ring[(j + 1) % AHEAD], T{});
+        }
+        body(nk - 1, ring[0], F{});
+        if constexpr (SIDE_A) {
+#pragma unroll
+            for (int r = 0; r < NRA; ++r) {
+                float s = rsum[r];
+#pragma unroll
+                for (int o = 1; o < QPR; o <<= 1) s += __shfl_xor(s, o, 64);
+                const int f = tid + NTH * r;
+                if (f % QPR == 0) rs_lds[f / QPR] = s;
+            }
+            __syncthreads();
+        }
+    }
+    __device__ static __forceinline__ int sub_row(int i, int r) {
+        const int lane = threadIdx.x & 63, wave = threadIdx.x >> 6;
+        return (wave >> 1) * 32 * MI + i * 32 + (r & 3) + 8 * (r >> 2) + 4 * (lane >> 5);
+    }
+    __device__ static __forceinline__ int sub_col() {
+        const int lane = threadIdx.x & 63, wave = threadIdx.x >> 6;
+        return (wave & 1) * 32 + (lane & 31);
     }
 };
 
diff --git a/v-gan_amd/csrc/mmd_bf16.hip b/v-gan_amd/csrc/mmd_bf16.hip
--- a/v-gan_amd/csrc/mmd_bf16.hip
+++ b/v-gan_amd/csrc/mmd_bf16.hip
@@ -561,6 +561,94 @@
     }
 }
 
+using TallLoop = GemmBF3Tall<8, 1>;
+
+template <bool REBUILD>
+__global__ __launch_bounds__(TallLoop::NTH, 1) void mmd_backward_bf3_tall_kernel(const unsigned short* __restrict__ Wh, const unsigned short* __restrict__ Wl,
+                                                                         int ldw, const unsigned short* __restrict__ Zh,
+                                                                         const unsigned short* __restrict__ Zl, int kn, int ldb, int brows,
+                                                                         const float* __restrict__ Z, int ldz, int wrow0, int nr, int p,
+                                                                         int ptiles, const float* __restrict__ mul, int ldmul,
+                                                                         const float* __restrict__ mul_shift, float* __restrict__ out, int ldo,
+                                                                         int kchunk, long slab_stride, vgan_finalize_job job, int nfin,
+                                                                         XXJob xx, BwdRebuild rb) {
+    using G = TallLoop;
+    static_assert(G::kLdsBytes >= GemmBF3<64>::kLdsBytes, "an X-X tile rides on the same region");
+    extern __shared__ __attribute__((aligned(16))) char lds[];
+    float* rs = reinterpret_cast<float*>(lds + G::kLdsBytes);
+    const int gx = ptiles, gy = (nr + 127) / 128, total = gx * gy;
+    if ((int)blockIdx.x >= total) {
+        if (blockIdx.y != 0) return;
+        const int extra = (int)blockIdx.x - total;
+        if (extra < nfin)
+            finalize_body(job);
+        else
+            xx_tile_body(xx, extra - nfin, lds, rs);
+        return;
+    }
+    const int xcd = blockIdx.x % 8, kidx = blockIdx.x / 8;
+    const int q = total / 8, r8 = total % 8;
+    const int t = (xcd < r8 ? xcd * (q + 1) : r8 * (q + 1) + (xcd - r8) * q) + kidx;
+    const int band = t / (4 * gx), rem = t - band * 4 * gx;
+    const int rows_in_band = min(4, gy - band * 4);
+    const int m0 = (band * 4 + rem % rows_in_band) * 128, n0 = (rem / rows_in_band) * 64;
+    f32x16 acc[G::MI];
+#pragma unroll
+    for (int i = 0; i < G::MI; ++i)
+#pragma unroll
+        for (int r = 0; r < 16; ++r) acc[i][r] = 0.f;
+    const int k0 = blockIdx.y * kchunk, klen = min(kchunk, kn - k0);
+    out += blockIdx.y * slab_stride;
+    const int col = n0 + G::sub_col(), colc = min(col, p - 1);
+    float z_pre[G::MI][16], m_pre[G::MI][16];
+    float mshift;
+    if constexpr (REBUILD) {
+        mshift = rb.center[colc];
+#pragma unroll
+        for (int i = 0; i < G::MI; ++i)
+#pragma unroll
+            for (int r = 0; r < 16; ++r) {
+                const int rowc = min(m0 + G::sub_row(i, r), nr - 1);
+                z_pre[i][r] = rb.S[(long)rowc * rb.lds + colc];
+                m_pre[i][r] = rb.data[(long)rb.xrow[rowc] * rb.ldd + colc];
+            }
+    } else {
+        mshift = mul_shift != nullptr ? mul_shift[colc] : 0.f;
+#pragma unroll
+        for (int i = 0; i < G::MI; ++i)
+#pragma unroll
+            for (int r = 0; r < 16; ++r) {
+                const int rowc = min(m0 + G::sub_row(i, r), nr - 1);
+                z_pre[i][r] = Z[(long)(wrow0 + rowc) * ldz + colc];
+                m_pre[i][r] = mul != nullptr ? mul[(long)rowc * ldmul + colc] + mshift : 1.f;
+            }
+    }
+    if (klen > 0)
+        G::template run_bt<true>(Wh + k0, Wl + k0, ldw, Zh + (long)k0 * ldb, Zl + (long)k0 * ldb, ldb, brows - k0, m0, n0, nr, klen, lds, rs, acc);
+    if (col >= p) return;
+    if constexpr (REBUILD) {
+        const float tau = 1.0f / (float)p;
+#pragma unroll
+        for (int i = 0; i < G::MI; ++i)
+#pragma unroll
+            for (int r = 0; r < 16; ++r) {
+                const float x = m_pre[i][r];
+                z_pre[i][r] = project_centred(upper_mask(z_pre[i][r], tau), x, mshift);
+                m_pre[i][r] = uncentred_x(centred_x(x, mshift), mshift);
+            }
+    }
+#pragma unroll
+    for (int i = 0; i < G::MI; ++i)
+#pragma unroll
+        for (int r = 0; r < 16; ++r) {
+            const int lrow = G::sub_row(i, r), row = m0 + lrow;
+            if (row < nr) {
+                const float v = klen > 0 ? 2.f * (rs[lrow] * z_pre[i][r] - acc[i][r]) : 0.f;
+                out[(long)row * ldo + col] = v * m_pre[i][r];
+            }
+        }
+}
+
 template <bool RM>
 __global__ __launch_bounds__(512, 2) void mmd_backward_bf3_big_kernel(const unsigned short* __restrict__ Wh, const unsigned short* __restrict__ Wl,
                                                                       int ldw, const unsigned short* __restrict__ ZTh,
@@ -769,11 +857,14 @@
 }
 
 extern "C" int vgan_mmd_backward_bf3_tile(int nr, int p, int splits, int tile) {
-    if (tile == 64 || tile == 128 || tile == 256) return tile;
+    if (tile == 64 || tile == 128 || tile == 256 || tile == VGAN_BWD_TILE_TALL) return tile;
     const int wide_tiles = ((p + 127) / 128) * ((nr + 255) / 256);
     if (nr >= 256 && wide_tiles * splits >= 256) return 256;
     const int big_tiles = ((p + 127) / 128) * ((nr + 127) / 128);
-    return big_tiles * splits >= 512 ? 128 : 64;
+    if (big_tiles * splits >= 512) return 128;
+    const int pt = (p + 63) / 64;
+    const int grid64 = pt * ((nr + 63) / 64) * splits, grid_tall = pt * ((nr + 127) / 128) * splits + 1;
+    return grid64 > 256 && grid_tall <= 256 ? VGAN_BWD_TILE_TALL : 64;
 }
 
 static int launch_backward_bf3(int rm, const uint16_t* Wh, const uint16_t* Wl, int ldw, const uint16_t* Bh, const uint16_t* Bl, int kn, int kp,
@@ -784,15 +875,17 @@
     VGAN_CHECK_ARG(Wh && Wl && Bh && Bl && (Z || rebuild) && out && nr > 0 && p > 0 && kn > 0 && kn % 64 == 0 && kp >= p && kp % 64 == 0);
     VGAN_CHECK_ARG(ldw >= kn && (rebuild || ldz >= p) && ldo >= p && (mul == nullptr || ldmul >= p) && wrow0 >= 0);
     BwdRebuild rb{};
+    int edge = vgan_mmd_backward_bf3_tile(nr, p, splits, tile);
+    const bool tile64 = edge == 64 || edge == VGAN_BWD_TILE_TALL;
     if (rebuild != nullptr) {
         const vgan_bwd_rebuild& q = *rebuild;
-        VGAN_CHECK_ARG(rm && tile == 64 && q.data && q.xrow && q.S && q.center && q.ldd >= p && q.lds >= p && Z == nullptr && mul == nullptr &&
+        VGAN_CHECK_ARG(rm && tile64 && q.data && q.xrow && q.S && q.center && q.ldd >= p && q.lds >= p && Z == nullptr && mul == nullptr &&
                        mul_shift == nullptr);
         rb = BwdRebuild{q.data, q.xrow, q.S, q.center, q.ldd, q.lds};
     }
     VGAN_CHECK_ARG(aligned16(Wh) && aligned16(Wl) && aligned16(Bh) && aligned16(Bl) && ldw % 8 == 0);
     VGAN_CHECK_ARG(splits >= 1 && splits <= 64 && (splits == 1 || slab_stride >= (int64_t)nr * ldo));
-    VGAN_CHECK_ARG((tile == 0 || tile == 64 || tile == 128 || tile == 256) && (mul_shift == nullptr || mul != nullptr) && (!rm || zrows > 0));
+    VGAN_CHECK_ARG((tile == 0 || tile == 64 || tile == 128 || tile == 256 || tile == VGAN_BWD_TILE_TALL) && (mul_shift == nullptr || mul != nullptr) && (!rm || zrows > 0));
     const int kchunk = ((kn / 64 + splits - 1) / splits) * 64;
     const int ldb = rm ? kp : kn;
     vgan_finalize_job job{};
@@ -804,13 +897,33 @@
     XXJob xx{};
     if (xxjob != nullptr) {
         const vgan_xx_job& j = *xxjob;
-        VGAN_CHECK_ARG(rm && tile == 64 && j.Dh && j.Dl && j.dsq && j.tiles && j.bw && j.partial && j.ntiles > 0 && j.ldd % 64 == 0 &&
+        VGAN_CHECK_ARG(rm && tile64 && j.Dh && j.Dl && j.dsq && j.tiles && j.bw && j.partial && j.ntiles > 0 && j.ldd % 64 == 0 &&
                        aligned16(j.Dh) && aligned16(j.Dl) && (reinterpret_cast<uintptr_t>(j.partial) & 15) == 0);
         xx = XXJob{j.Dh, j.Dl, j.dsq, nullptr, nullptr, reinterpret_cast<const TileDesc*>(j.tiles), j.bw, j.partial, j.ldd, 1, 0, j.ntiles, 0};
     }
     const int nfin = finalize != nullptr ? 1 : 0;
-    int edge = vgan_mmd_backward_bf3_tile(nr, p, splits, tile);
     if (edge == 256 && !rm) edge = 128;
+    if (edge == VGAN_BWD_TILE_TALL && !rm) edge = 64;
+    if (edge == VGAN_BWD_TILE_TALL && tile == 0 && ((p + 63) / 64) * ((nr + 127) / 128) * splits + nfin + xx.ntiles > 256) edge = 64;
+    if (edge == VGAN_BWD_TILE_TALL) {
+        using G = TallLoop;
+        constexpr int kDyn = G::kLdsBytes + 128 * (int)sizeof(float);
+        static const hipError_t attr_z = hipFuncSetAttribute(reinterpret_cast<const void*>(&mmd_backward_bf3_tall_kernel<false>),
+                                                             hipFuncAttributeMaxDynamicSharedMemorySize, kDyn);
+        static const hipError_t attr_r = hipFuncSetAttribute(reinterpret_cast<const void*>(&mmd_backward_bf3_tall_kernel<true>),
+                                                             hipFuncAttributeMaxDynamicSharedMemorySize, kDyn);
+        VGAN_CHECK_ARG(attr_z == hipSuccess && attr_r == hipSuccess);
+        const int pt = (p + 63) / 64;
+        dim3 grid(pt * ((nr + 127) / 128) + nfin + xx.ntiles, splits);
+        if (rebuild != nullptr)
+            hipLaunchKernelGGL(mmd_backward_bf3_tall_kernel<true>, grid, dim3(G::NTH), kDyn, st, Wh, Wl, ldw, Bh, Bl, kn, ldb, zrows, Z, ldz, wrow0, nr,
+                               p, pt, mul, ldmul, mul_shift, out, ldo, kchunk, (long)slab_stride, job, nfin, xx, rb);
+        else
+            hipLaunchKernelGGL(mmd_backward_bf3_tall_kernel<false>, grid, dim3(G::NTH), kDyn, st, Wh, Wl, ldw, Bh, Bl, kn, ldb, zrows, Z, ldz, wrow0, nr,
+                               p, pt, mul, ldmul, mul_shift, out, ldo, kchunk, (long)slab_stride, job, nfin, xx, rb);
+        VGAN_CHECK_LAUNCH();
+        return VGAN_OK;
+    }
     if (edge == 256) {
         static const hipError_t attr = hipFuncSetAttribute(reinterpret_cast<const void*>(&mmd_backward_bf3_wide_kernel),
                                                            hipFuncAttributeMaxDynamicSharedMemorySize, GemmBF3Wide::kLdsBytes);
@@ -858,13 +971,21 @@
                                tile, finalize, stream);
 }
 
+extern "C" int vgan_mmd_backward_bf3_rm_xx_tile(const uint16_t* Wh, const uint16_t* Wl, int ldw, int kn, const uint16_t* Zh, const uint16_t* Zl,
+                                                int kp, int zrows, const float* Z, int ldz, int wrow0, int nr, int p, const float* mul, int ldmul,
+                                                const float* mul_shift, float* out, int ldo, int splits, int64_t slab_stride, int tile,
+                                                const vgan_finalize_job* finalize, const vgan_xx_job* xx, vgan_stream_t stream) {
+    VGAN_CHECK_ARG(xx != nullptr);
+    return launch_backward_bf3(1, Wh, Wl, ldw, Zh, Zl, kn, kp, zrows, Z, ldz, wrow0, nr, p, mul, ldmul, mul_shift, out, ldo, splits,
+                               slab_stride, tile, finalize, stream, xx);
+}
+
 extern "C" int vgan_mmd_backward_bf3_rm_xx(const uint16_t* Wh, const uint16_t* Wl, int ldw, int kn, const uint16_t* Zh, const uint16_t* Zl,
                                            int kp, int zrows, const float* Z, int ldz, int wrow0, int nr, int p, const float* mul, int ldmul,
                                            const float* mul_shift, float* out, int ldo, int splits, int64_t slab_stride,
                                            const vgan_finalize_job* finalize, const vgan_xx_job* xx, vgan_stream_t stream) {
-    VGAN_CHECK_ARG(xx != nullptr);
-    return launch_backward_bf3(1, Wh, Wl, ldw, Zh, Zl, kn, kp, zrows, Z, ldz, wrow0, nr, p, mul, ldmul, mul_shift, out, ldo, splits,
-                               slab_stride, 64, finalize, stream, xx);
+    return vgan_mmd_backward_bf3_rm_xx_tile(Wh, Wl, ldw, kn, Zh, Zl, kp, zrows, Z, ldz, wrow0, nr, p, mul, ldmul, mul_shift, out, ldo, splits,
+                                            slab_stride, 64, finalize, xx, stream);
 }
 
 extern "C" int vgan_mmd_backward_bf3_rm(const uint16_t* Wh, const uint16_t* Wl, int ldw, int kn, const uint16_t* Zh, const uint16_t* Zl,
@@ -875,11 +996,19 @@
                                slab_stride, tile, finalize, stream, nullptr, rs_part, ldrs);
 }
 
+extern "C" int vgan_mmd_backward_bf3_rm_rebuild_tile(const uint16_t* Wh, const uint16_t* Wl, int ldw, int kn, const uint16_t* Zh,
+                                                     const uint16_t* Zl, int kp, int zrows, int nr, int p, const vgan_bwd_rebuild* rebuild,
+                                                     float* out, int ldo, int splits, int64_t slab_stride, int tile,
+                                                     const vgan_finalize_job* finalize, const vgan_xx_job* xx, vgan_stream_t stream) {
+    VGAN_CHECK_ARG(rebuild != nullptr);
+    return launch_backward_bf3(1, Wh, Wl, ldw, Zh, Zl, kn, kp, zrows, nullptr, 0, 0, nr, p, nullptr, 0, nullptr, out, ldo, splits, slab_stride, tile,
+                               finalize, stream, xx, nullptr, 0, rebuild);
+}
+
 extern "C" int vgan_mmd_backward_bf3_rm_rebuild(const uint16_t* Wh, const uint16_t* Wl, int ldw, int kn, const uint16_t* Zh, const uint16_t* Zl,
                                                 int kp, int zrows, int nr, int p, const vgan_bwd_rebuild* rebuild, float* out, int ldo,
                                                 int splits, int64_t slab_stride, const vgan_finalize_job* finalize, const vgan_xx_job* xx,
                                                 vgan_stream_t stream) {
-    VGAN_CHECK_ARG(rebuild != nullptr);
-    return launch_backward_bf3(1, Wh, Wl, ldw, Zh, Zl, kn, kp, zrows, nullptr, 0, 0, nr, p, nullptr, 0, nullptr, out, ldo, splits, slab_stride, 64,
-                               finalize, stream, xx, nullptr, 0, rebuild);
-}
+    return vgan_mmd_backward_bf3_rm_rebuild_tile(Wh, Wl, ldw, kn, Zh, Zl, kp, zrows, nr, p, rebuild, out, ldo, splits, slab_stride, 64, finalize,
+                                                 xx, stream);
+}
diff --git a/v-gan_amd/lib.py b/v-gan_amd/lib.py
--- a/v-gan_amd/lib.py
+++ b/v-gan_amd/lib.py
@@ -89,7 +89,9 @@
     "vgan_mmd_backward_bf3_tile": (_i, [_i, _i, _i, _i]),
     "vgan_mmd_backward_bf3_rm": (_i, [_p, _p, _i, _i, _p, _p, _i, _i, _p, _i, _i, _i, _i, _p, _i, _p, _p, _i, _i, _i64, _i, _p, _p, _i, _p]),
     "vgan_mmd_backward_bf3_rm_xx": (_i, [_p, _p, _i, _i, _p, _p, _i, _i, _p, _i, _i, _i, _i, _p, _i, _p, _p, _i, _i, _i64, _p, _p, _p]),
+    "vgan_mmd_backward_bf3_rm_xx_tile": (_i, [_p, _p, _i, _i, _p, _p, _i, _i, _p, _i, _i, _i, _i, _p, _i, _p, _p, _i, _i, _i64, _i, _p, _p, _p]),
     "vgan_mmd_backward_bf3_rm_rebuild": (_i, [_p, _p, _i, _i, _p, _p, _i, _i, _i, _i, _p, _p, _i, _i, _i64, _p, _p, _p]),
+    "vgan_mmd_backward_bf3_rm_rebuild_tile": (_i, [_p, _p, _i, _i, _p, _p, _i, _i, _i, _i, _p, _p, _i, _i, _i64, _i, _p, _p, _p]),
     "vgan_row_sqnorm": (_i, [_p, _i, _p, _i, _i, _p]),
     "vgan_adadelta_step": (_i, [_p, _p, _i, _i64, _p, _p, _i64, _f, _f, _f, _f, _f, _p]),
     "vgan_noise_normal": (_i, [_p, _i, _i, _i, _i, _u64, _p, _u64, _p]),
@@ -159,6 +161,7 @@
 }
 
 ABI_VERSION = 11
+BWD_TILE_TALL = 192
 _lib = None
 
 
diff --git a/v-gan_amd/ops.py b/v-gan_amd/ops.py
--- a/v-gan_amd/ops.py
+++ b/v-gan_amd/ops.py
@@ -3,6 +3,8 @@
 import torch
 
 from . import lib as _lib
+
+BWD_TILE_TALL = _lib.BWD_TILE_TALL
 
 _f32 = torch.float32
 
@@ -354,12 +356,12 @@
         kn = (int(zrows) + 63) // 64 * 64
         assert Wh.stride(0) >= kn and Zh.shape[0] >= zrows
         if xx is not None:
-            assert tile in (0, 64)
-            _lib.check(self.lib.vgan_mmd_backward_bf3_rm_xx(_ptr(Wh), _ptr(Wl), Wh.stride(0), kn, _ptr(Zh), _ptr(Zl), Zh.stride(0), int(zrows),
-                                                            _ptr(Z), Z.stride(0), int(wrow0), int(nr), int(p), _ptr(mul), ldmul, _ptr(mul_shift),
-                                                            _ptr(out), out.stride(0), int(splits), int(slab_stride),
-                                                            ctypes.byref(finalize) if finalize is not None else None, ctypes.byref(xx),
-                                                            self._stream()), "vgan_mmd_backward_bf3_rm_xx")
+            assert tile in (0, 64, BWD_TILE_TALL)
+            _lib.check(self.lib.vgan_mmd_backward_bf3_rm_xx_tile(_ptr(Wh), _ptr(Wl), Wh.stride(0), kn, _ptr(Zh), _ptr(Zl), Zh.stride(0),
+                                                                 int(zrows), _ptr(Z), Z.stride(0), int(wrow0), int(nr), int(p), _ptr(mul), ldmul,
+                                                                 _ptr(mul_shift), _ptr(out), out.stride(0), int(splits), int(slab_stride),
+                                                                 int(tile), ctypes.byref(finalize) if finalize is not None else None,
+                                                                 ctypes.byref(xx), self._stream()), "vgan_mmd_backward_bf3_rm_xx_tile")
             return
         _lib.check(self.lib.vgan_mmd_backward_bf3_rm(_ptr(Wh), _ptr(Wl), Wh.stride(0), kn, _ptr(Zh), _ptr(Zl), Zh.stride(0), int(zrows),
                                                      _ptr(Z), Z.stride(0), int(wrow0), int(nr), int(p), _ptr(mul), ldmul, _ptr(mul_shift),
@@ -368,15 +370,17 @@
                                                      rs_part.stride(0) if rs_part is not None else 0, self._stream()),
                    "vgan_mmd_backward_bf3_rm")
 
-    def mmd_backward_bf3_rm_rebuild(self, Wh, Wl, Zh, Zl, zrows, nr, p, rebuild, out, splits=1, slab_stride=0, finalize=None, xx=None):
+    def mmd_backward_bf3_rm_rebuild(self, Wh, Wl, Zh, Zl, zrows, nr, p, rebuild, out, splits=1, slab_stride=0, finalize=None, xx=None,
+                                    tile=0):
         _mat(out, "out")
         kn = (int(zrows) + 63) // 64 * 64
         assert Wh.stride(0) >= kn and Zh.shape[0] >= zrows
-        _lib.check(self.lib.vgan_mmd_backward_bf3_rm_rebuild(_ptr(Wh), _ptr(Wl), Wh.stride(0), kn, _ptr(Zh), _ptr(Zl), Zh.stride(0), int(zrows),
-                                                             int(nr), int(p), ctypes.byref(rebuild), _ptr(out), out.stride(0), int(splits),
-                                                             int(slab_stride), ctypes.byref(finalize) if finalize is not None else None,
-                                                             ctypes.byref(xx) if xx is not None else None, self._stream()),
-                   "vgan_mmd_backward_bf3_rm_rebuild")
+        _lib.check(self.lib.vgan_mmd_backward_bf3_rm_rebuild_tile(_ptr(Wh), _ptr(Wl), Wh.stride(0), kn, _ptr(Zh), _ptr(Zl), Zh.stride(0),
+                                                                  int(zrows), int(nr), int(p), ctypes.byref(rebuild), _ptr(out), out.stride(0),
+                                                                  int(splits), int(slab_stride), int(tile),
+                                                                  ctypes.byref(finalize) if finalize is not None else None,
+                                                                  ctypes.byref(xx) if xx is not None else None, self._stream()),
+                   "vgan_mmd_backward_bf3_rm_rebuild_tile")
 
     def mmd_backward_bf3_tile(self, nr, p, splits=1, tile=0):
         return int(self.lib.vgan_mmd_backward_bf3_tile(int(nr), int(p), int(splits), int(tile)))
diff --git a/v-gan_amd/trainer.py b/v-gan_amd/trainer.py
--- a/v-gan_amd/trainer.py
+++ b/v-gan_amd/trainer.py
@@ -3,6 +3,8 @@
 import os
 
 import torch
+
+from .lib import BWD_TILE_TALL
 
 ADADELTA_RHO = 0.9
 ADADELTA_EPS = 1e-6
@@ -306,8 +308,10 @@
         self.xx_late_in_backward = False
         if self.xx_in_m4 and self.rm_backward and os.environ.get("VGAN_XX_LATE", "backward") == "backward":
             late = self.tiles.shape[0] - self.n_main
-            bwd_wgs = ((d + 63) // 64) * ((nl + 63) // 64) * self.bsplits + 1
-            self.xx_late_in_backward = (ops.mmd_backward_bf3_tile(nl, d, self.bsplits, self.bwd_tile) == 64 and late <= 512 - bwd_wgs)
+            edge = ops.mmd_backward_bf3_tile(nl, d, self.bsplits, self.bwd_tile)
+            rows, slots = (128, 256) if edge == BWD_TILE_TALL else (64, 512)
+            bwd_wgs = ((d + 63) // 64) * ((nl + rows - 1) // rows) * self.bsplits + 1
+            self.xx_late_in_backward = (edge in (64, BWD_TILE_TALL) and late <= slots - bwd_wgs)
         self.m4_kparts = self.tn_kparts = 1
         self.m4_ws = self.tn_ws = None
         if self.mode == "collapsed" and getattr(ops, "chain_ksplit", False):
@@ -326,7 +330,7 @@
                 self.tn_ws = ops.ksplit_workspace(ops.gemm_grouped_ksplit_ws_bytes(tn, [self.tn_kparts] * 3), self.dev)
         plain_bf3 = (getattr(ops, "bf3_rebuild", False) and self.bf3 and self.fused_prepare and self.gram_tile == 64 and
                      self.rm_backward and world == 1 and not self.overlap and not self.front_sharded and
-                     ops.mmd_backward_bf3_tile(nl, d, self.bsplits, self.bwd_tile) == 64)
+                     ops.mmd_backward_bf3_tile(nl, d, self.bsplits, self.bwd_tile) in (64, BWD_TILE_TALL))
         self.lean = plain_bf3 and os.environ.get("VGAN_Z_FP32", "0") != "1"
         self.xrow = torch.zeros(n, dtype=torch.int32, device=self.dev) if self.lean else None
         self._rebuild = None
@@ -643,7 +647,7 @@
                 if self._rebuild is None:
                     self._rebuild = ops.bwd_rebuild(self.data, self.xrow, self.S, self.center)
                 ops.mmd_backward_bf3_rm_rebuild(self.Wh, self.Wl, self.Zh, self.Zl, 2 * n, nl, d, self._rebuild, self.gU, self.bsplits, gstride,
-                                                fin, xx=self._late_xx_job() if self.xx_late_in_backward else None)
+                                                fin, xx=self._late_xx_job() if self.xx_late_in_backward else None, tile=self.bwd_tile)
             elif self.rm_backward:
                 ops.mmd_backward_bf3_rm(self.Wh, self.Wl, self.Zh, self.Zl, 2 * n, self.Z, n + lo, nl, d, self.Z[lo:lo + nl], self.gU,
                                         self.bsplits, gstride, fin, mul_shift=self.center, tile=self.bwd_tile,
```
